# yang-z-03/scd-resnet

Measured on AMD Instinct MI355X. Metric: 512x512 images/sec training, centerOffsetRes10, at 1/2/4/8 MI355X, higher is better.
Workload: dtype bf16; 1 GPU; centerOffsetRes10 train step (fwd+focal/L1 loss+bwd+Adam, DDP over RCCL), 512x512 synthetic SCD tiles; model=centerOffsetRes10, global_batch=32, step_issue=eager launches, per_gpu_batch=32, parallelism=dp1, image_size=512

## Files before the change

include/scdhip.h:

```cpp
#ifndef SCDHIP_H
#define SCDHIP_H
#include <stddef.h>
#include <stdint.h>

#ifdef __cplusplus
extern "C" {
#endif

#define SCD_DT_F32 0
#define SCD_DT_BF16 1
#define SCD_DT_F16 2

#define SCD_ERR_ARG 9001

#define SCD_MAX_TAPS 16
#define SCD_MAX_PHASES 4
#define SCD_STAT_REPLICAS 64

typedef struct scd_gemm_phase {
    int Qh, Qw, rho_h, rho_w, ntaps;
    int dh[SCD_MAX_TAPS], dw[SCD_MAX_TAPS], wt[SCD_MAX_TAPS];
} scd_gemm_phase;

int scd_conv_gemm(int dtype, const void* x, const void* w, void* y, const float* bias, double* stats,
                  int N, int Hi, int Wi, int Ci, int Ho, int Wo, int Co, int in_stride, int out_stride,
                  int wrow, int relu, int accumulate, int nphase, const scd_gemm_phase* phases,
                  void* stream);

int scd_conv_dgrad_s2(int dtype, const void* dy, const void* w3, void* dx, int N, int Hq, int Wq, int Cg, int Cin,
                      int accumulate, void* stream);
int scd_conv_gemm_bnbwd(int dtype, const void* x, const void* w, void* y, int N, int Hi, int Wi, int Ci, int Ho,
                        int Wo, int Co, int in_stride, int out_stride, int wrow, int nphase,
                        const scd_gemm_phase* phases, const void* bn_y, const float* mean, const float* invstd,
                        const float* relu_scale, const float* relu_shift, double* bn_stats, void* stream);
int scd_conv_gemm_sel(int dtype, int kernel, const void* x, const void* w, void* y, const float* bias, double* stats,
                      int N, int Hi, int Wi, int Ci, int Ho, int Wo, int Co, int in_stride, int out_stride, int wrow,
                      int relu, int accumulate, int nphase, const scd_gemm_phase* phases, const void* bn_y,
                      const float* mean, const float* invstd, const float* relu_scale, const float* relu_shift,
                      void* stream);
int scd_conv_gemm_res(int dtype, const void* x, const void* w, void* y, const float* bias, const void* res, int N,
                      int Hi, int Wi, int Ci, int Ho, int Wo, int Co, int in_stride, int out_stride, int wrow,
                      int relu, int nphase, const scd_gemm_phase* phases, void* stream);
int scd_conv_gemm_heads(int dtype, const void* x, const void* w, void* hid, const float* bias, int N, int H,
                        int W, int Ci, int nh, const int* od, const float* const* w1, const float* const* b1,
                        float* const* outs, void* stream);
int scd_conv_gemm_heads_keep(int dtype, const void* x, const void* w, void* hid, const float* bias, int N, int H,
                             int W, int Ci, int nh, const int* od, const float* const* w1, const float* const* b1,
                             float* const* outs, const unsigned char* keep, int keep_cols, void* stream);

size_t scd_conv_wgrad_workspace(int Cg, int T, int Ci, int nsplit);
int scd_conv_wgrad_nsplit(int dtype, long M, int Cg, int T, int Ci);
int scd_conv_wgrad_nsplit2(int dtype, long M, int Ho, int Wo, int Cg, int T, int Ci);
int scd_conv_wgrad(int dtype, const void* g, const void* x, float* ws, int nsplit,
                   int N, int Ho, int Wo, int Cg, int Hi, int Wi, int Ci, int in_stride,
                   int T, const int* dh, const int* dw, void* stream);
int scd_wgrad_reduce(const float* ws, int nsplit, int Cg, int T, int Ci, int r0, int r1, int cvalid,
                     long ld_n, long ld_c, long ld_t, float* dst, int accumulate, float alpha, void* stream);
int scd_wgrad_reduce_rows(const float* ws, int nsplit, int Cg, int T, int Ci, int nslices, const int* r0,
                          const int* r1, const long* ld_n, const long* ld_c, const long* ld_t, float* const* dst,
                          int cvalid, int accumulate, float alpha, void* stream);

int scd_pack_weight(int dtype, const float* w, void* out, int A, int B, int T, int mode, int ldp,
                    int row_off, void* stream);

int scd_pad_channels(int dtype, const void* src, long rows, int C, int Cp, void* dst, void* stream);

int scd_upsample2x_add(int dtype, const void* up, const void* low, void* out, int N, int h, int w, int C, void* stream);
int scd_upsample2x_add_bwd(int dtype, const void* dout, void* dlow, int N, int h, int w, int C, void* stream);

typedef struct scd_pack_desc {
    const float* w;
    void* out;
    long start;
    int A, B, T, mode, ldp, row_off, a_off, a_tot;
} scd_pack_desc;
int scd_pack_weights_batched(int dtype, const scd_pack_desc* descs, int n, long total, void* stream);

int scd_im2col_stem(int dtype, const float* x, void* cols, int N, int H, int W, int Ho, int Wo, int kh,
                    int kw, int stride, int pad, int Kpad, void* stream);

int scd_stem_conv_fwd(int dtype, const float* x, const void* wpk, void* y, double* stats, int N, int H, int W,
                      int Ho, int Wo, void* stream);
int scd_stem_conv_wgrad_nsplit(long M);
int scd_stem_conv_wgrad(int dtype, const void* dy, const void* ybn, const float* coef, const float* x, float* ws,
                        int nsplit, int N, int H, int W, int Ho, int Wo, void* stream);
int scd_stem_bwd_nsplit(void);
int scd_stem_bwd_fused(int dtype, const void* dout, const uint8_t* argmax, const void* y, const float* scale,
                       const float* shift, const float* mean, const float* invstd, const float* x, double* stats,
                       float* ws, int nsplit, float* tg, int N, int H, int W, int Ho, int Wo, void* stream);
int scd_stem_bwd_combine(int dtype, const float* tg, const void* wpk, const float* coef, float* dst, int accumulate,
                         float alpha, void* stream);

int scd_stats_collapse(double* stats, int nrep, int C, void* stream);
int scd_stats_collapse_to(double* stats, int nrep, int C, double* out, void* stream);
int scd_bn_finalize(double* stats, int nrep, int C, double count, const float* gamma,
                    const float* beta, float* running_mean, float* running_var, int64_t* num_batches,
                    float momentum, float eps, float* mean, float* invstd, float* scale, float* shift,
                    void* stream);
#define SCD_BN_FIN_MAX 4
typedef struct scd_bn_fin_args {
    double* stats;
    int nrep, C;
    double count;
    const float* gamma;
    const float* beta;
    float* running_mean;
    float* running_var;
    int64_t* num_batches;
    float momentum, eps;
    float* mean;
    float* invstd;
    float* scale;
    float* shift;
} scd_bn_fin_args;
int scd_bn_finalize_n(const scd_bn_fin_args* layers, int n, void* stream);
int scd_bn_apply(int dtype, const void* y, void* out, int C, long total, const float* scale,
                 const float* shift, const void* res, const float* rscale, const float* rshift,
                 int relu, void* stream);
int scd_bn_bwd_reduce(int dtype, const void* dout, const void* mask, const void* y, const float* relu_scale,
                      const float* relu_shift, const float* mean, const float* invstd, int C, long total,
                      double* stats, void* stream);
int scd_bn_bwd_finalize(double* stats, int nrep, int C, double count, const float* gamma,
                        const float* mean, const float* invstd, float* dgamma, float* dbeta,
                        float gscale, float* coef, void* stream);
typedef struct scd_bn_bwd_fin_args {
    double* stats;
    int nrep, C;
    double count;
    const float* gamma;
    const float* mean;
    const float* invstd;
    float* dgamma;
    float* dbeta;
    float gscale;
    float* coef;
} scd_bn_bwd_fin_args;
int scd_bn_bwd_finalize_n(const scd_bn_bwd_fin_args* layers, int n, void* stream);
int scd_bn_bwd_apply(int dtype, const void* dout, const void* mask, const void* y, const float* relu_scale,
                     const float* relu_shift, const float* coef, int C, long total, void* dy, void* dz,
                     void* stream);

int scd_bn_bwd_reduce2(int dtype, const void* dout, const void* mask, const void* ya, const void* yb,
                       const float* mean_a, const float* invstd_a, const float* mean_b, const float* invstd_b, int C,
                       long total, double* stats_a, double* stats_b, void* stream);
int scd_bn_bwd_apply2(int dtype, const void* dout, const void* mask, const void* ya, const void* yb,
                      const float* coef_a, const float* coef_b, int C, long total, void* dya, void* dyb, void* stream);


int scd_stem_pool_bwd_bn(int dtype, const void* dout, const uint8_t* argmax, const void* y, const float* scale,
                         const float* shift, const float* mean, const float* invstd, void* dz, double* stats, int N,
                         int H, int W, int C, int Ho, int Wo, void* stream);
int scd_stem_pool_fwd(int dtype, const void* y, const float* scale, const float* shift, void* out,
                      uint8_t* argmax, int N, int H, int W, int C, int Ho, int Wo, void* stream);
int scd_stem_pool_bwd(int dtype, const void* dout, const uint8_t* argmax, const void* y,
                      const float* scale, const float* shift, void* dz, int N, int H, int W, int C,
                      int Ho, int Wo, void* stream);

int scd_heads_fwd(int dtype, const void* hid, int N, int HW, int nh, int Hd, const int* od,
                  const float* const* w1, const float* const* b1, float* const* outs, void* stream);
size_t scd_heads_bwd_accsize(int nh, int Hd, const int* od);
int scd_heads_bwd(int dtype, const void* hid, int N, int HW, int nh, int Hd, const int* od,
                  const float* const* w1, const float* const* douts, void* dhid, double* acc, void* stream);
int scd_heads_bwd_packed(int dtype, const void* hid, int N, int HW, int nh, int Hd, const int* od,
                         const float* const* w1, const float* const* douts, float dscale, float* packed, void* dhid,
                         double* acc, void* stream);
int scd_heads_bwd_weight_finalize(double* acc, int nh, int Hd, const int* od, float* const* dw1,
                                  float* const* db1, float* const* db0, int accumulate, float alpha, void* stream);
int scd_heads_bwd_packed_split(int dtype, const void* hid, int N, int HW, int nh, int Hd, const int* od, int nd,
                               const float* const* w1, const float* const* douts, float dscale, float* packed,
                               void* dhid, double* acc, void* stream);
int scd_heads_sparse_bwd(int dtype, const void* hid, const void* feat, int N, int H, int W, int Cin, int nh, int Hd,
                         const int* od, int nd, const float* const* w1, const float* const* douts, float dscale,
                         const long* inds, int K, void* dhid_s, void* xcol, double* acc, int* slotmap, int* ownermap,
                         void* stream);
int scd_heads_sparse_fixup(int dtype, void* dx, const void* cols, int N, int H, int W, int Cin, const long* inds, int K,
                           int* slotmap, int* ownermap, const void* bn_y, const float* mean, const float* invstd,
                           const float* relu_scale, const float* relu_shift, double* bn_stats, void* stream);

int scd_focal_fwd(const float* logits, const float* gt, long n, float* g, double* acc, void* stream);
int scd_l1_gather_fwd(const float* feat, int N, int C, int HW, const int64_t* inds, const uint8_t* mask,
                      const float* target, int K, int tstride, int toff, float* g, double* acc, void* stream);
int scd_centernet_loss_finalize(double* focal_acc, int nfocal, double* l1_acc, int nl1,
                                const float* l1_weights, float* out, float* factors, void* stream);
int scd_centernet_loss_fwd(const float* heat, const float* gt, long n_heat, const float* regr, int Cr, const float* off,
                           int Co, int N, int HW, const int64_t* inds, const uint8_t* mask, const float* target, int K,
                           int tstride, int toff_r, int toff_o, const float* l1_weights, float* g_heat, float* g_regr,
                           float* g_off, double* focal_acc, float* out, float* factors, void* stream);
int scd_centernet_loss_bwd_scale(float* g_heat, long n_heat, int N, int HW, const int64_t* inds, int K, float* g_regr,
                                 int Cr, float* g_off, int Co, const float* factors, const float* go, void* stream);

int scd_corner_ae_fwd(const float* tl_tag, const float* br_tag, int N, int HW, const int64_t* tl_inds,
                      const int64_t* br_inds, const uint8_t* valid, int K, float w_pull, float w_push,
                      double* focal_acc, int nfocal, double* ae_acc, float* gs_tl, float* gs_br, float* out,
                      float* factors, void* stream);
int scd_corner_ae_bwd(const float* gs_tl, const float* gs_br, int N, int HW, const int64_t* tl_inds,
                      const int64_t* br_inds, const uint8_t* valid, int K, const float* go, float* g_tl, float* g_br,
                      void* stream);

int scd_heads_keep_map(const int64_t* inds, int N, int K, int HW, int64_t* prev, int nprev, uint8_t* keep, void* stream);

int scd_scale_by_device(float* g, long n, const float* factors, int idx, const float* go, void* stream);

int scd_render_center_targets(const float* locs, const int* counts, int B, int K, int H, float threshold,
                              float* heat, uint8_t* mask, float* regr, int64_t* inds, void* stream);
#define SCD_CORNER_SPLIT_THREAD 0
#define SCD_CORNER_SPLIT_GRID 1
#define SCD_CORNER_SPLIT_DEFAULT SCD_CORNER_SPLIT_GRID
int scd_render_corner_targets(const float* locs, const int* counts, int B, int K, int H, float threshold,
                              float* heat, float* tl, float* br, uint8_t* mask, float* regr, int64_t* inds,
                              void* stream);
int scd_render_corner_targets_split(const float* locs, const int* counts, int B, int K, int H, float threshold,
                                    float* heat, float* tl, float* br, uint8_t* mask, float* regr, int64_t* inds,
                                    int split, void* stream);
int scd_corner_tag_inds(const float* locs, const int* counts, int B, int K, int size, int64_t* tl_inds,
                        int64_t* br_inds, uint8_t* valid, void* stream);
size_t scd_augment_workspace(int B);
int scd_augment_tiles(const float* in, float* out, int B, int H, int W, const uint8_t* flips, const float* jitter,
                      const float* noise, float noise_sv, unsigned long long seed, void* workspace, void* stream);
int scd_augment_tiles_indexed(const float* store, long nstore, const int* ids, float* out, int B, int H, int W,
                              const uint8_t* flips, const float* jitter, const float* noise, float noise_sv,
                              unsigned long long seed, void* workspace, void* stream);
int scd_pack_locs(const float* rows, const long* offsets, const int* ids, int B, const uint8_t* flips, const float* cs,
                  int size, int K, int trunc, float* locs, int* counts, void* stream);
#define SCD_ROTATE_MAP_ROW 0
#define SCD_ROTATE_MAP_64X4 1
#define SCD_ROTATE_MAP_32X8 2
#define SCD_ROTATE_MAP_16X16 3
#define SCD_ROTATE_MAP_DEFAULT SCD_ROTATE_MAP_32X8
int scd_rotate_tiles(const float* in, float* out, int B, int H, int W, const double* cs, void* stream);
int scd_rotate_tiles_mapped(const float* in, float* out, int B, int H, int W, const double* cs, int mapping,
                            void* stream);
size_t scd_slide_workspace(int ntiles);
int scd_slide_tiles(const uint8_t* rgb, int H, int W, int C, int tile, int stride, int clipH, int clipV, int padLR,
                    int padTB, int fix, float* out, void* workspace, void* stream);
int scd_slide_detections(const float* decoded, int T, int K, int stride, int padLR, int padTB, int clipV, float thr,
                         int* xy, double* ratio, int* count, void* stream);
#define SCD_SLIDE_SAMPLES_MAX 16384
#define SCD_SLIDE_RADIUS_MAX 1048576
size_t scd_slide_samples_workspace(int T, int K);
int scd_slide_samples(const float* decoded, int T, int K, int stride, int padLR, int padTB, int clipV, float thr,
                      int x0, int y0, int x1, int y1, int radius, double lo, double scale, int nbins, int* xy,
                      double* ratio, float* score, int* index, int* count, int64_t* hist, int64_t* counters,
                      void* workspace, void* stream);
size_t scd_slide_rotate_workspace(int H, int W);
int scd_slide_rotate_clips(const uint8_t* rgb, int H, int W, int C, int left, int top, int right, int bottom,
                           int tile, const double* angles, int R, float* out, void* workspace, void* stream);
size_t scd_decode_workspace(int N, int HW);
int scd_decode_topk(const float* heat, int N, int H, int W, int K, const float* offset, int od_off,
                    const float* regr, int od_regr, float* scores, int64_t* inds, int64_t* ys, int64_t* xs,
                    float* off_out, float* regr_out, void* workspace, void* stream);
int scd_corner_pairs(const float* tl_scores, const int64_t* tl_inds, const int64_t* tl_ys, const int64_t* tl_xs,
                     const float* br_scores, const int64_t* br_inds, const int64_t* br_ys, const int64_t* br_xs,
                     const float* tl_tag, const float* br_tag, int N, int K, int HW, float threshold, int D, float* det,
                     int* nvalid, void* stream);

int scd_ceval_count(const float* scores, const int64_t* cty, const int64_t* ctx, const float* offset, const float* regr,
                    const float* gt_regr, const void* gt_loc, int loc_mode, int loc_w, int N, int K, int L, int H,
                    float thr, int* counts, void* stream);
int scd_ceval_emit(const float* scores, const int64_t* cty, const int64_t* ctx, const float* offset, const float* regr,
                   const float* gt_regr, const void* gt_loc, int loc_mode, int loc_w, int N, int K, int L, int H,
                   float thr, const int* counts, float* const* streams, void* stream);
size_t scd_ceval_summary_workspace(long n);
int scd_ceval_summary(const float* const* streams, const long* lens, long objnum, const float* thr, int nthr,
                      double* out, void* workspace, void* stream);

int scd_adam_step(float* p, const float* g, float* m, float* v, long n, float lr, float beta1, float beta2,
                  float eps, float bc1, float bc2, float gscale, void* stream);
int scd_adam_step_dev(float* p, const float* g, float* m, float* v, long n, double* hyper, float beta1, float beta2,
                      float eps, float gscale, const unsigned long long* skip, void* stream);
int scd_sgd_step_dev(float* p, const float* g, float* buf, long n, double* hyper, float momentum, float dampening,
                     float weight_decay, int nesterov, float gscale,
                     const unsigned long long* skip, void* stream);

int scd_cpool_fwd(int dtype, int dir, const void* x, const void* addend, void* y, int N, int H, int W, int C,
                  void* stream);
int scd_cpool_bwd(int dtype, int dir, const void* x, const void* dy, void* dx, int N, int H, int W, int C,
                  void* stream);

int scd_nms(const float* x, long planes, int H, int W, int k, float* out, void* stream);
int scd_topk(const float* scores, int B, long n, int K, int HW, int W, float* out_scores, int64_t* inds, int* cats,
             float* ys, float* xs, void* stream);
int scd_focal_prob_fwd(const float* p, const float* gt, long n, float* g, double* acc, void* stream);
int scd_masked_l1_fwd(const float* r, const float* t, const uint8_t* mask, long rows, int C, int smooth, float* g,
                      double* acc, void* stream);

size_t scd_peer_mailbox_bytes(int R, int cap);
int scd_peer_alloc(size_t bytes, void** ptr);
int scd_peer_free(void* ptr);
int scd_peer_ipc_handle(void* ptr, void* handle64);
int scd_peer_ipc_open(const void* handle64, void** ptr);
int scd_peer_ipc_close(void* ptr);
int scd_peer_allreduce_f64(double* data, int n, int rank, int R, void* const* boxes, int cap, unsigned long long epoch,
                           unsigned long long* err, unsigned timeout_ms, void* stream);


int scd_event_create(void** ev);
int scd_event_destroy(void* ev);
int scd_event_record(void* ev, void* stream);
int scd_event_elapsed_ms(void* start, void* end, float* ms);

int scd_calib_mfma_peak(const void* src, int grid, int iters, float* out, unsigned long long* stamps, void* stream);
int scd_calib_set_stamps(unsigned long long* stamps);
int scd_calib_stamped_build(void);

const char* scd_version(void);

#ifdef __cplusplus
}
#endif
#endif
```

scd-resnet_amd/csrc/layers.hip:

```cpp
#include <algorithm>

#include "gemm_common.h"
#include "scd_common.h"

namespace {
SCD_KERNEL_NS_BEGIN

__device__ __forceinline__ float s2_phase_weight(const float* w, unsigned A, unsigned B, unsigned r, unsigned k) {
    const unsigned ph = r / B, b = r - ph * B, t = k / A, a = k - t * A;
    const int kr = (int)(ph >> 1) + 1 - 2 * (int)(t >> 1), ks = (int)(ph & 1) + 1 - 2 * (int)(t & 1);
    return (kr >= 0 && kr < 3 && ks >= 0 && ks < 3) ? w[(a * B + b) * 9 + kr * 3 + ks] : 0.f;
}

template <typename T>
__global__ void pack_weight_kernel(const float* w, T* out, int A, int B, int Tt, int mode, int ldp, int row_off) {
    if (mode == 3) {
        const unsigned total = 4u * B * ldp;
        for (unsigned i = blockIdx.x * blockDim.x + threadIdx.x; i < total; i += gridDim.x * blockDim.x) {
            const unsigned r = i / (unsigned)ldp, k = i - r * (unsigned)ldp;
            out[(long)(row_off + r) * ldp + k] = from_f<T>(k < 4u * A ? s2_phase_weight(w, A, B, r, k) : 0.f);
        }
        return;
    }
    const int rows = mode == 0 ? A : mode == 1 ? B : Tt * B;
    const unsigned total = (unsigned)rows * ldp;
    for (unsigned i = blockIdx.x * blockDim.x + threadIdx.x; i < total; i += gridDim.x * blockDim.x) {
        const int r = (int)(i / (unsigned)ldp);
        const int k = (int)(i - (unsigned)r * ldp);
        float v = 0.f;
        if (mode == 0) {
            const int t = k / B, b = k - (k / B) * B;
            if (t < Tt) v = w[((long)r * B + b) * Tt + t];
        } else if (mode == 1) {
            const int t = k / A, a = k - (k / A) * A;
            if (t < Tt) v = w[((long)a * B + r) * Tt + t];
        } else {
            if (k >= A) continue;
            const int t = r / B, b = r - (r / B) * B;
            out[(long)r * ldp + row_off + k] = from_f<T>(w[((long)k * B + b) * Tt + t]);
            continue;
        }
        out[(long)(row_off + r) * ldp + k] = from_f<T>(v);
    }
}

constexpr int PACK_UNIT = 4096;

__global__ __launch_bounds__(256) void pack_weights_batched_kernel(const scd_pack_desc* __restrict__ d, int n, int bf16) {
    const long e0 = (long)blockIdx.x * PACK_UNIT;
    int lo = 0, hi = n - 1;
    while (lo < hi) {
        const int mid = (lo + hi + 1) >> 1;
        if (d[mid].start <= e0) lo = mid; else hi = mid - 1;
    }
    const scd_pack_desc q = d[lo];
    if (q.mode == 1) {
        __shared__ float tile[64 * 65];
        const int T = q.T, BB = max(1, 64 / T);
        const int nbb = (q.B + BB - 1) / BB;
        const int u = (int)((e0 - q.start) / PACK_UNIT);
        const int ta = u / nbb, tb = u - (u / nbb) * nbb;
        const int a0 = ta * 64, b0 = tb * BB;
        if (a0 >= q.A) return;
        const int na = min(64, q.A - a0), nb = min(BB, q.B - b0);
        const int rowl = nb * T, pitch = rowl | 1;
        for (int i = threadIdx.x; i < na * rowl; i += 256) {
            const int a = i / rowl, k = i - a * rowl;
            tile[a * pitch + k] = q.w[((unsigned)(a0 + a) * q.B + b0) * T + k];
        }
        __syncthreads();
        if (bf16 && na % 8 == 0 && q.ldp % 8 == 0 && q.a_tot % 8 == 0 && q.a_off % 8 == 0) {
            const int na8 = na / 8;
            for (int i = threadIdx.x; i < na8 * rowl; i += 256) {
                const int bt = i / na8, a = (i - bt * na8) * 8;
                const int b = bt / T, t = bt - b * T;
                typedef __attribute__((ext_vector_type(8))) h16 bf8;
                bf8 v;
#pragma unroll
                for (int e = 0; e < 8; ++e) v[e] = (h16)tile[(a + e) * pitch + b * T + t];
                const unsigned o = (unsigned)(b0 + b) * q.ldp + t * q.a_tot + q.a_off + a0 + a;
                *(bf8*)((h16*)q.out + o) = v;
            }
            return;
        }
        for (int i = threadIdx.x; i < na * rowl; i += 256) {
            const int bt = i / na, a = i - bt * na;
            const int b = bt / T, t = bt - b * T;
            const float v = tile[a * pitch + b * T + t];
            const unsigned o = (unsigned)(b0 + b) * q.ldp + t * q.a_tot + q.a_off + a0 + a;
            if (bf16) ((h16*)q.out)[o] = (h16)v;
            else ((float*)q.out)[o] = v;
        }
        return;
    }
    if (q.mode == 3) {
        const unsigned count3 = 4u * q.B * q.ldp, base3 = (unsigned)(e0 - q.start);
#pragma unroll 4
        for (int j = 0; j < PACK_UNIT / 256; ++j) {
            const unsigned i = base3 + threadIdx.x + 256 * j;
            if (i >= count3) break;
            const unsigned r = i / (unsigned)q.ldp, k = i - r * (unsigned)q.ldp;
            const float v = s2_phase_weight(q.w, q.A, q.B, r, k);
            const unsigned o = (q.row_off + r) * (unsigned)q.ldp + k;
            if (bf16) ((h16*)q.out)[o] = (h16)v;
            else ((float*)q.out)[o] = v;
        }
        return;
    }
    const unsigned count = q.mode == 0 ? (unsigned)q.A * q.ldp : (unsigned)q.B * q.T * q.A;
    const unsigned base = (unsigned)(e0 - q.start);
    const unsigned ldp = q.ldp, B = q.B, Tt = q.T, A = q.A, TA = Tt * A;
    if (q.mode == 0 && bf16 && ldp % 8 == 0 && B % 8 == 0 && q.row_off >= 0) {
        typedef __attribute__((ext_vector_type(8))) h16 bf8;
#pragma unroll
        for (int j = 0; j < PACK_UNIT / 256 / 8; ++j) {
            const unsigned i = base + 8 * (threadIdx.x + 256 * j);
            if (i >= count) break;
            const unsigned r = i / ldp, k = i - r * ldp;
            const unsigned t = k / B, b = k - t * B;
            bf8 v;
            const float* src = q.w + (r * B + b) * Tt + min(t, Tt - 1);
#pragma unroll
            for (int e = 0; e < 8; ++e) {
                const float x = src[e * Tt];
                v[e] = (h16)(t < Tt ? x : 0.f);
            }
            *(bf8*)((h16*)q.out + (q.row_off + r) * ldp + k) = v;
        }
        return;
    }
#pragma unroll 4
    for (int j = 0; j < PACK_UNIT / 256; ++j) {
        const unsigned i = base + threadIdx.x + 256 * j;
        if (i >= count) break;
        float v;
        unsigned o;
        if (q.mode == 0) {
            const unsigned r = i / ldp, k = i - r * ldp;
            const unsigned t = k / B, b = k - t * B;
            v = t < Tt ? q.w[(r * B + b) * Tt + t] : 0.f;
            o = (q.row_off + r) * ldp + k;
        } else if (q.mode == 1) {
            const unsigned r = i / TA, rem = i - r * TA;
            const unsigned t = rem / A, a = rem - t * A;
            v = q.w[(a * B + r) * Tt + t];
            o = r * ldp + t * q.a_tot + q.a_off + a;
        } else {
            const unsigned BA = B * A;
            const unsigned t = i / BA, rem = i - t * BA;
            const unsigned b = rem / A, a = rem - b * A;
            v = q.w[(a * B + b) * Tt + t];
            o = (t * B + b) * ldp + q.a_off + a;
        }
        if (bf16) ((h16*)q.out)[o] = (h16)v;
        else ((float*)q.out)[o] = v;
    }
}

struct HeadsDesc {
    int nh, Hd, od[4], orow[4], nout;
    int nd;
    int hstride, dstride;
    const float* w1[4];
    const float* b1[4];
    const float* dout[4];
    float* out[4];
    const float* pk;
};

__global__ void heads_pack_kernel(int N, int HW, HeadsDesc d, float scale, float* pk) {
    const long P = (long)N * HW;
    for (long px = blockIdx.x * (long)blockDim.x + threadIdx.x; px < P; px += (long)gridDim.x * blockDim.x) {
        const long n = px / HW, q = px - n * HW;
        for (int h = 0; h < d.nd; ++h) {
            float v[4];
#pragma unroll
            for (int o = 0; o < 4; ++o) v[o] = o < d.od[h] ? d.dout[h][(n * d.od[h] + o) * HW + q] * scale : 0.f;
            *(float4*)(pk + (px * d.nd + h) * 4) = make_float4(v[0], v[1], v[2], v[3]);
        }
    }
}

template <typename T>
__global__ void heads_fwd_kernel(const T* hid, int N, int HW, HeadsDesc d) {
    constexpr int E = Vec16<T>::N;
    const int cph = d.Hd / E;
    const unsigned cpp = (unsigned)(d.nh * cph);
    const unsigned total = (unsigned)N * HW * cpp;
    for (unsigned base = blockIdx.x * blockDim.x; base < total; base += gridDim.x * blockDim.x) {
        const unsigned i = base + threadIdx.x;
        const bool ok = i < total;
        const unsigned px = ok ? i / cpp : 0;
        const int ch = ok ? (int)(i - px * cpp) : 0;
        const int h = ch / cph;
        const int cl = (ch - h * cph) * E;
        float v[E];
        if (ok) Vec16<T>::load(hid + (size_t)i * E, v);
        else
#pragma unroll
            for (int e = 0; e < E; ++e) v[e] = 0.f;
        float acc[4];
#pragma unroll
        for (int o = 0; o < 4; ++o) {
            float a = 0.f;
            if (ok && o < d.od[h]) {
                const float* w = d.w1[h] + o * d.Hd + cl;
#pragma unroll
                for (int e = 0; e < E; ++e) a += v[e] * w[e];
            }
            for (int m = cph >> 1; m > 0; m >>= 1) a += __shfl_xor(a, m, 64);
            acc[o] = a;
        }
        if (ok && (ch - h * cph) == 0) {
            const int n = (int)(px / (unsigned)HW);
            const int q = (int)(px - (unsigned)n * HW);
            for (int o = 0; o < d.od[h]; ++o)
                d.out[h][((size_t)n * d.od[h] + o) * HW + q] = acc[o] + d.b1[h][o];
        }
    }
}

template <typename T, int U, bool PK = false>
__global__ __launch_bounds__(512) void heads_bwd_kernel(const T* hid, int N, int HW, HeadsDesc d, T* dhid,
                                                        double* acc, int accsz, int PXB) {
    constexpr int E = Vec16<T>::N;
    constexpr int NA = 4 * E + E + 4;
    const int cph = d.Hd / E;
    const int cpp = d.nd * cph;
    const int G = blockDim.x / cpp;
    const int tid = threadIdx.x;
    const int c = tid % cpp;
    const int g = tid / cpp;
    const int h = c / cph;
    const int cl = (c - h * cph) * E;
    const int ct = h * d.Hd + cl;
    const int od = d.od[h];
    const float* dout = d.dout[h];
    float w[4][E];
#pragma unroll
    for (int o = 0; o < 4; ++o)
#pragma unroll
        for (int e = 0; e < E; ++e) w[o][e] = o < od ? d.w1[h][o * d.Hd + cl + e] : 0.f;
    float a[NA];
#pragma unroll
    for (int k = 0; k < NA; ++k) a[k] = 0.f;
    const unsigned P = (unsigned)N * HW;
    const unsigned p0 = blockIdx.x * (unsigned)PXB;
    const unsigned p1 = min(P, p0 + PXB);
    const unsigned Ctot = d.hstride, Dtot = d.dstride;
    auto body = [&](unsigned px, const float* gd, float* v) {
        float r[E];
#pragma unroll
        for (int e = 0; e < E; ++e) {
            const float s = gd[0] * w[0][e] + gd[1] * w[1][e] + gd[2] * w[2][e] + gd[3] * w[3][e];
            r[e] = v[e] > 0.f ? s : 0.f;
#pragma unroll
            for (int o = 0; o < 4; ++o) a[o * E + e] += gd[o] * v[e];
            a[4 * E + e] += r[e];
        }
#pragma unroll
        for (int o = 0; o < 4; ++o) a[5 * E + o] += gd[o];
        Vec16<T>::store(dhid + px * Dtot + ct, r);
    };
    auto load_gd = [&](unsigned px, float* gd) {
        if constexpr (PK) {
            const float4 v = *(const float4*)(d.pk + ((size_t)px * d.nd + h) * 4);
            gd[0] = v.x; gd[1] = v.y; gd[2] = v.z; gd[3] = v.w;
        } else {
            const unsigned n = px / (unsigned)HW;
            const unsigned q = px - n * HW;
#pragma unroll
            for (int o = 0; o < 4; ++o) gd[o] = o < od ? dout[(n * od + o) * (unsigned)HW + q] : 0.f;
        }
    };
    if (g < G) {
        unsigned px = p0 + g;
        for (; px + (U - 1) * G < p1; px += U * G) {
            float gd[U][4], v[U][E];
#pragma unroll
            for (int u = 0; u < U; ++u) {
                load_gd(px + u * G, gd[u]);
                Vec16<T>::load(hid + (px + u * G) * Ctot + ct, v[u]);
            }
#pragma unroll
            for (int u = 0; u < U; ++u) body(px + u * G, gd[u], v[u]);
        }
        for (; px < p1; px += G) {
            float gd[4], v[E];
            load_gd(px, gd);
            Vec16<T>::load(hid + px * Ctot + ct, v);
            body(px, gd, v);
        }
    }
    constexpr int KR = (NA + 3) / 4;
    __shared__ float red[KR * 512];
    double* dst = acc + (size_t)(blockIdx.x % SCD_STAT_REPLICAS) * accsz;
#pragma unroll
    for (int k0 = 0; k0 < NA; k0 += KR) {
        if (k0) __syncthreads();
        if (g < G)
#pragma unroll
            for (int k = 0; k < KR; ++k)
                if (k0 + k < NA) red[(k * G + g) * cpp + c] = a[k0 + k];
        __syncthreads();
        for (int i = tid; i < KR * cpp; i += blockDim.x) {
            const int kk = i / cpp, cc = i - (i / cpp) * cpp;
            const int k = k0 + kk;
            if (k >= NA) continue;
            float s = 0.f;
            for (int j = 0; j < G; ++j) s += red[(kk * G + j) * cpp + cc];
            const int hh = cc / cph;
            const int cll = (cc - hh * cph) * E;
            const int odh = d.od[hh];
            if (k < 4 * E) {
                const int o = k / E, e = k - (k / E) * E;
                if (o < odh) atomic_add_f64(dst + (d.orow[hh] + o) * d.Hd + cll + e, (double)s);
            } else if (k < 5 * E) {
                atomic_add_f64(dst + d.nout * d.Hd + d.nout + hh * d.Hd + cll + (k - 4 * E), (double)s);
            } else {
                const int o = k - 5 * E;
                if (o < odh && cll == 0) atomic_add_f64(dst + d.nout * d.Hd + d.orow[hh] + o, (double)s);
            }
        }
    }
}

bool make_desc(HeadsDesc& d, int nh, int Hd, const int* od) {
    if (nh < 1 || nh > 4 || Hd % 8 != 0) return false;
    d.nh = nh; d.Hd = Hd; d.nout = 0;
    d.nd = nh; d.hstride = d.dstride = nh * Hd;
    for (int h = 0; h < 4; ++h) {
        d.od[h] = h < nh ? od[h] : 0;
        if (d.od[h] > 4) return false;
        d.orow[h] = d.nout;
        d.nout += d.od[h];
        d.w1[h] = nullptr; d.b1[h] = nullptr; d.dout[h] = nullptr; d.out[h] = nullptr;
        d.pk = nullptr;
    }
    return d.nout * Hd <= 8 * 512;
}

inline int ew_blocks(long n) { return (int)std::min<long>(8192, std::max<long>(1, (n + 255) / 256)); }

SCD_KERNEL_NS_END
}

extern "C" int scd_pack_weights_batched(int dtype, const scd_pack_desc* descs, int n, long total, void* stream) {
    SCD_F16_FWD(scd_pack_weights_batched, descs, n, total, stream);
    if (n < 1 || total < 1 || total >= (1L << 31) || total % PACK_UNIT || (dtype != SCD_DT_BF16 && dtype != SCD_DT_F32)) return SCD_ERR_ARG;
    hipLaunchKernelGGL(pack_weights_batched_kernel, dim3((unsigned)(total / PACK_UNIT)), dim3(256), 0, (hipStream_t)stream,
                       descs, n, dtype == SCD_DT_BF16 ? 1 : 0);
    SCD_RETURN_LAUNCH();
}

extern "C" int scd_pack_weight(int dtype, const float* w, void* out, int A, int B, int T, int mode, int ldp, int row_off,
                               void* stream) {
    SCD_F16_FWD(scd_pack_weight, w, out, A, B, T, mode, ldp, row_off, stream);
    if (mode == 3 && (T != 9 || ldp < 4 * A)) return SCD_ERR_ARG;
    const long total = (long)(mode == 0 ? A : mode == 3 ? 4 * B : B) * ldp;
    return scd_dispatch_dtype(dtype, [&](auto tag) {
        using E = typename decltype(tag)::type;
        hipLaunchKernelGGL((pack_weight_kernel<E>), dim3(ew_blocks(total)), dim3(256), 0, (hipStream_t)stream, w,
                           (E*)out, A, B, T, mode, ldp, row_off);
        SCD_RETURN_LAUNCH();
    });
}

extern "C" int scd_heads_fwd(int dtype, const void* hid, int N, int HW, int nh, int Hd, const int* od,
                             const float* const* w1, const float* const* b1, float* const* outs, void* stream) {
    SCD_F16_FWD(scd_heads_fwd, hid, N, HW, nh, Hd, od, w1, b1, outs, stream);
    HeadsDesc d;
    if (!make_desc(d, nh, Hd, od)) return SCD_ERR_ARG;
    return scd_dispatch_dtype(dtype, [&](auto tag) {
        using T = typename decltype(tag)::type;
        constexpr int E = 16 / sizeof(T);
        const int cph = Hd / E;
        if (cph > 64 || (cph & (cph - 1))) return SCD_ERR_ARG;
        for (int h = 0; h < nh; ++h) { d.w1[h] = w1[h]; d.b1[h] = b1[h]; d.out[h] = outs[h]; }
        const long total = (long)N * HW * nh * cph;
        const int blocks = (int)std::min<long>(16384, (total + 255) / 256);
        hipLaunchKernelGGL((heads_fwd_kernel<T>), dim3(blocks), dim3(256), 0, (hipStream_t)stream, (const T*)hid, N,
                           HW, d);
        SCD_RETURN_LAUNCH();
    });
}

template <bool PK>
static int launch_heads_bwd(int dtype, const void* hid, int N, int HW, int nh, int Hd, const int* od, int nd,
                            const float* const* w1, const float* const* douts, float dscale, float* packed, void* dhid,
                            double* acc, void* stream) {
    HeadsDesc d;
    if (!make_desc(d, nh, Hd, od) || (PK && !packed) || nd < 1 || nd > nh) return SCD_ERR_ARG;
    d.nd = nd;
    d.dstride = nd * Hd;
    return scd_dispatch_dtype(dtype, [&](auto tag) {
        using T = typename decltype(tag)::type;
        constexpr int E = 16 / sizeof(T);
        const int cpp = nd * Hd / E;
        if (cpp > 256 || (Hd % E)) return SCD_ERR_ARG;
        for (int h = 0; h < nh; ++h) { d.w1[h] = w1[h]; d.dout[h] = douts[h]; }
        const int accsz = d.nout * Hd + d.nout + nh * Hd;
        const long P = (long)N * HW;
        if (P * nh * Hd >= (1L << 31)) return SCD_ERR_ARG;
        hipStream_t st = (hipStream_t)stream;
        if constexpr (PK) {
            hipLaunchKernelGGL(heads_pack_kernel, dim3(ew_blocks(P)), dim3(256), 0, st, N, HW, d, dscale, packed);
            hipError_t e = hipGetLastError();
            if (e != hipSuccess) return (int)e;
            d.pk = packed;
        }
        const int G = 512 / cpp;
        const int threads = G * cpp;
        const int PXB = 2048;
        const int blocks = cdiv(P, PXB);
        hipLaunchKernelGGL((heads_bwd_kernel<T, E, PK>), dim3(blocks), dim3(threads), 0, st, (const T*)hid, N, HW, d,
                           (T*)dhid, acc, accsz, PXB);
        SCD_RETURN_LAUNCH();
    });
}

extern "C" int scd_heads_bwd(int dtype, const void* hid, int N, int HW, int nh, int Hd, const int* od,
                             const float* const* w1, const float* const* douts, void* dhid, double* acc,
                             void* stream) {
    SCD_F16_FWD(scd_heads_bwd, hid, N, HW, nh, Hd, od, w1, douts, dhid, acc, stream);
    return launch_heads_bwd<false>(dtype, hid, N, HW, nh, Hd, od, nh, w1, douts, 1.f, nullptr, dhid, acc, stream);
}

extern "C" int scd_heads_bwd_packed(int dtype, const void* hid, int N, int HW, int nh, int Hd, const int* od,
                                    const float* const* w1, const float* const* douts, float dscale, float* packed,
                                    void* dhid, double* acc, void* stream) {
    SCD_F16_FWD(scd_heads_bwd_packed, hid, N, HW, nh, Hd, od, w1, douts, dscale, packed, dhid, acc, stream);
    return scd_heads_bwd_packed_split(dtype, hid, N, HW, nh, Hd, od, nh, w1, douts, dscale, packed, dhid, acc, stream);
}

extern "C" int scd_heads_bwd_packed_split(int dtype, const void* hid, int N, int HW, int nh, int Hd, const int* od,
                                          int nd, const float* const* w1, const float* const* douts, float dscale,
                                          float* packed, void* dhid, double* acc, void* stream) {
    SCD_F16_FWD(scd_heads_bwd_packed_split, hid, N, HW, nh, Hd, od, nd, w1, douts, dscale, packed, dhid, acc, stream);
    return launch_heads_bwd<true>(dtype, hid, N, HW, nh, Hd, od, nd, w1, douts, dscale, packed, dhid, acc, stream);
}

namespace {
SCD_KERNEL_NS_BEGIN
constexpr int SP_SPB = 2;

template <typename T>
__global__ __launch_bounds__(256) void heads_sparse_bwd_kernel(const T* hid, const T* feat, int N, int H, int W, int Cin,
                                                               HeadsDesc d, float dscale, const long* inds, int K,
                                                               T* dhid_s, T* xcol, double* acc, int accsz,
                                                               int* slotmap, int* ownermap) {
    const int HW = H * W;
    const int Cs = (d.nh - d.nd) * d.Hd;
    const int tid = threadIdx.x;
    const int c = tid;
    const bool cok = c < Cs;
    const int h = cok ? d.nd + c / d.Hd : d.nd;
    const int j = cok ? c - (h - d.nd) * d.Hd : 0;
    const int od = d.od[h];
    float w[4];
#pragma unroll
    for (int o = 0; o < 4; ++o) w[o] = (cok && o < od) ? d.w1[h][o * d.Hd + j] : 0.f;
    float a_dw1[4] = {0.f, 0.f, 0.f, 0.f}, a_db1[4] = {0.f, 0.f, 0.f, 0.f}, a_db0 = 0.f;
    const int S = N * K;
    const int s0 = blockIdx.x * SP_SPB;
    const int ns = min(S, s0 + SP_SPB) - s0;
    __shared__ int dup[SP_SPB];
    if (tid < SP_SPB) dup[tid] = 0;
    __syncthreads();
    for (int i = tid; i < ns * K; i += blockDim.x) {
        const int jj = i / K, k2 = i - (i / K) * K;
        const int s = s0 + jj, k = s - (s / K) * K;
        if (k2 < k && inds[s - k + k2] == inds[s]) dup[jj] = 1;
    }
    __syncthreads();
    for (int jj = 0; jj < ns; ++jj) {
        const int s = s0 + jj;
        const int b = s / K;
        const long ind = inds[s];
        const bool active = ind >= 0 && ind < HW && !dup[jj];
        const int q0 = active ? (int)ind : 0;
        const int y = q0 / W, x = q0 - (q0 / W) * W;
        const long p = (long)b * HW + q0;
        float r = 0.f;
        if (active && cok) {
            const float hv = to_f<T>(hid[p * d.hstride + d.nd * d.Hd + c]);
            float g[4];
#pragma unroll
            for (int o = 0; o < 4; ++o) g[o] = o < od ? d.dout[h][((long)b * od + o) * HW + q0] * dscale : 0.f;
            const float sacc = g[0] * w[0] + g[1] * w[1] + g[2] * w[2] + g[3] * w[3];
            r = hv > 0.f ? sacc : 0.f;
#pragma unroll
            for (int o = 0; o < 4; ++o) { a_dw1[o] += g[o] * hv; a_db1[o] += g[o]; }
            a_db0 += r;
        }
        if (cok) dhid_s[(long)s * Cs + c] = from_f<T>(r);
        if (active && tid < 9) {
            if (tid == 0) slotmap[p] = s;
            const int qy = y + tid / 3 - 1, qx = x + tid % 3 - 1;
            if ((unsigned)qy < (unsigned)H && (unsigned)qx < (unsigned)W)
                atomicMin(ownermap + (long)b * HW + qy * W + qx, s * 9 + tid);
        }
        for (int ci = tid; ci < Cin; ci += blockDim.x) {
            T v[9];
#pragma unroll
            for (int t = 0; t < 9; ++t) {
                const int iy = y + t / 3 - 1, ix = x + t % 3 - 1;
                const bool in = (unsigned)iy < (unsigned)H && (unsigned)ix < (unsigned)W;
                v[t] = in ? feat[(((long)b * H + iy) * W + ix) * Cin + ci] : from_f<T>(0.f);
            }
#pragma unroll
            for (int t = 0; t < 9; ++t) xcol[(long)s * 9 * Cin + t * Cin + ci] = v[t];
        }
    }
    if (cok) {
        double* dst = acc + (size_t)(blockIdx.x % SCD_STAT_REPLICAS) * accsz;
#pragma unroll
        for (int o = 0; o < 4; ++o)
            if (o < od) atomic_add_f64(dst + (d.orow[h] + o) * d.Hd + j, (double)a_dw1[o]);
        atomic_add_f64(dst + d.nout * d.Hd + d.nout + h * d.Hd + j, (double)a_db0);
        if (j == 0)
#pragma unroll
            for (int o = 0; o < 4; ++o)
                if (o < od) atomic_add_f64(dst + d.nout * d.Hd + d.orow[h] + o, (double)a_db1[o]);
    }
}

template <typename T>
__global__ __launch_bounds__(256) void heads_sparse_fixup_kernel(T* dx, const T* cols, int N, int H, int W, int Cin,
                                                                 const long* inds, int K, const int* slotmap,
                                                                 int* ownermap, const T* bny, const float* mean,
                                                                 const float* invstd, const float* rsc,
                                                                 const float* rsh, double* stats) {
    const int HW = H * W;
    const int s = blockIdx.x;
    const int b = s / K;
    const long ind = inds[s];
    if (ind < 0 || ind >= HW) return;
    const long p = (long)b * HW + ind;
    if (slotmap[p] != s) return;
    const int y = (int)ind / W, x = (int)ind - ((int)ind / W) * W;
    const int tid = threadIdx.x;
    __shared__ int nb[25], own[9];
    if (tid < 25) {
        const int py = y + tid / 5 - 2, px = x + tid % 5 - 2;
        nb[tid] = ((unsigned)py < (unsigned)H && (unsigned)px < (unsigned)W) ? slotmap[(long)b * HW + py * W + px] : -1;
    } else if (tid >= 32 && tid < 41) {
        const int t = tid - 32;
        const int qy = y + t / 3 - 1, qx = x + t % 3 - 1;
        own[t] = ((unsigned)qy < (unsigned)H && (unsigned)qx < (unsigned)W) ? ownermap[(long)b * HW + qy * W + qx] : -1;
    }
    __syncthreads();
    if (tid < 9 && own[tid] == s * 9 + tid)
        ownermap[(long)b * HW + (y + tid / 3 - 1) * W + x + tid % 3 - 1] = 0x7fffffff;
    const long KC = 9L * Cin;
    for (int ci = tid; ci < Cin; ci += blockDim.x) {
        float bm = 0.f, bi = 0.f, bs = 0.f, bh = 0.f;
        if (bny) { bm = mean[ci]; bi = invstd[ci]; bs = rsc[ci]; bh = rsh[ci]; }
        float dsum = 0.f, dsq = 0.f;
        for (int t = 0; t < 9; ++t) {
            if (own[t] != s * 9 + t) continue;
            const int oy = t / 3 - 1, ox = t % 3 - 1;
            float corr = 0.f;
#pragma unroll
            for (int t2 = 0; t2 < 9; ++t2) {
                const int s2 = nb[(oy - (t2 / 3 - 1) + 2) * 5 + ox - (t2 % 3 - 1) + 2];
                if (s2 >= 0) corr += to_f<T>(cols[(long)s2 * KC + t2 * Cin + ci]);
            }
            const long qi = p + oy * W + ox;
            T* dp = dx + qi * Cin + ci;
            const T old = *dp;
            const T nv = from_f<T>(to_f<T>(old) + corr);
            *dp = nv;
            if (bny) {
                const float yv = to_f<T>(bny[qi * Cin + ci]);
                const float dd = yv * bs + bh > 0.f ? to_f<T>(nv) - to_f<T>(old) : 0.f;
                dsum += dd;
                dsq += dd * (yv - bm) * bi;
            }
        }
        if (bny) {
            const int rep = stat_replica(s);
            atomic_add_f64(stat_slot(stats, rep, 0, Cin, ci), (double)dsum);
            atomic_add_f64(stat_slot(stats, rep, 1, Cin, ci), (double)dsq);
        }
    }
}

__global__ void heads_sparse_reset_kernel(const long* inds, int S, int K, int HW, int* slotmap) {
    const int s = blockIdx.x * blockDim.x + threadIdx.x;
    if (s >= S) return;
    const long ind = inds[s];
    if (ind < 0 || ind >= HW) return;
    const long p = (long)(s / K) * HW + ind;
    if (slotmap[p] == s) slotmap[p] = -1;
}

SCD_KERNEL_NS_END
}

extern "C" int scd_heads_sparse_bwd(int dtype, const void* hid, const void* feat, int N, int H, int W, int Cin, int nh,
                                    int Hd, const int* od, int nd, const float* const* w1, const float* const* douts,
                                    float dscale, const long* inds, int K, void* dhid_s, void* xcol, double* acc,
                                    int* slotmap, int* ownermap, void* stream) {
    SCD_F16_FWD(scd_heads_sparse_bwd, hid, feat, N, H, W, Cin, nh, Hd, od, nd, w1, douts, dscale, inds, K, dhid_s, xcol,
                acc, slotmap, ownermap, stream);
    HeadsDesc d;
    if (!make_desc(d, nh, Hd, od) || nd < 0 || nd >= nh || K < 1 || (nh - nd) * Hd > 256) return SCD_ERR_ARG;
    if ((long)N * K * 9 * 9 >= (1L << 31) || (long)N * H * W * nh * Hd >= (1L << 31)) return SCD_ERR_ARG;
    d.nd = nd;
    for (int h = 0; h < nh; ++h) { d.w1[h] = w1[h]; d.dout[h] = douts[h]; }
    const int accsz = d.nout * Hd + d.nout + nh * Hd;
    const int blocks = cdiv((long)N * K, SP_SPB);
    return scd_dispatch_dtype(dtype, [&](auto tag) {
        using T = typename decltype(tag)::type;
        hipLaunchKernelGGL(heads_sparse_bwd_kernel<T>, dim3(blocks), dim3(256), 0, (hipStream_t)stream, (const T*)hid,
                           (const T*)feat, N, H, W, Cin, d, dscale, inds, K, (T*)dhid_s, (T*)xcol, acc, accsz, slotmap,
                           ownermap);
        SCD_RETURN_LAUNCH();
    });
}

extern "C" int scd_heads_sparse_fixup(int dtype, void* dx, const void* cols, int N, int H, int W, int Cin,
                                      const long* inds, int K, int* slotmap, int* ownermap, const void* bn_y,
                                      const float* mean, const float* invstd, const float* relu_scale,
                                      const float* relu_shift, double* bn_stats, void* stream) {
    SCD_F16_FWD(scd_heads_sparse_fixup, dx, cols, N, H, W, Cin, inds, K, slotmap, ownermap, bn_y, mean, invstd,
                relu_scale, relu_shift, bn_stats, stream);
    if (Cin < 1 || K < 1) return SCD_ERR_ARG;
    if (bn_y && !(mean && invstd && relu_scale && relu_shift && bn_stats)) return SCD_ERR_ARG;
    const int S = N * K;
    hipStream_t st = (hipStream_t)stream;
    return scd_dispatch_dtype(dtype, [&](auto tag) {
        using T = typename decltype(tag)::type;
        hipLaunchKernelGGL(heads_sparse_fixup_kernel<T>, dim3(S), dim3(256), 0, st, (T*)dx, (const T*)cols, N, H, W,
                           Cin, inds, K, slotmap, ownermap, (const T*)bn_y, mean, invstd, relu_scale, relu_shift,
                           bn_stats);
        hipError_t e = hipGetLastError();
        if (e != hipSuccess) return (int)e;
        hipLaunchKernelGGL(heads_sparse_reset_kernel, dim3(cdiv(S, 256)), dim3(256), 0, st, inds, S, K, H * W, slotmap);
        SCD_RETURN_LAUNCH();
    });
}

#ifndef SCD_F16_BUILD
namespace {

struct HeadsGrad {
    float* dw1[4];
    float* db1[4];
    float* db0[4];
};

__global__ void heads_bwd_weight_finalize_kernel(double* acc, int accsz, HeadsDesc d, HeadsGrad g, int accumulate,
                                                 double alpha) {
    for (int i = blockIdx.x * blockDim.x + threadIdx.x; i < accsz; i += gridDim.x * blockDim.x) {
        double s = 0.0;
        for (int r = 0; r < SCD_STAT_REPLICAS; ++r) {
            s += acc[(long)r * accsz + i];
            acc[(long)r * accsz + i] = 0.0;
        }
        float* dst;
        if (i < d.nout * d.Hd) {
            const int row = i / d.Hd, cl = i - (i / d.Hd) * d.Hd;
            int h = 0;
            while (h + 1 < d.nh && row >= d.orow[h + 1]) ++h;
            dst = g.dw1[h] + (row - d.orow[h]) * d.Hd + cl;
        } else if (i < d.nout * d.Hd + d.nout) {
            const int row = i - d.nout * d.Hd;
            int h = 0;
            while (h + 1 < d.nh && row >= d.orow[h + 1]) ++h;
            dst = g.db1[h] + (row - d.orow[h]);
        } else {
            const int c = i - d.nout * d.Hd - d.nout;
            const int h = c / d.Hd;
            dst = g.db0[h] + (c - h * d.Hd);
        }
        s *= alpha;
        *dst = accumulate ? (*dst + (float)s) : (float)s;
    }
}

__global__ void adam_kernel(float* p, const float* g, float* m, float* v, long n, float lr, float b1, float b2,
                            float eps, float bc1, float bc2_sqrt, float gscale) {
    const float step = lr / bc1;
    for (long i = blockIdx.x * (long)blockDim.x + threadIdx.x; i < n; i += (long)gridDim.x * blockDim.x) {
        const float gi = g[i] * gscale;
        float mi = m[i];
        mi = mi + (1.f - b1) * (gi - mi);
        float vi = v[i] * b2 + (1.f - b2) * gi * gi;
        const float denom = sqrtf(vi) / bc2_sqrt + eps;
        p[i] = p[i] - step * (mi / denom);
        m[i] = mi;
        v[i] = vi;
    }
}

__global__ void adam_tick_kernel(double* hyper, const unsigned long long* skip) {
    if (skip && *skip) return;
    if (threadIdx.x == 0) hyper[1] = hyper[1] + 1.0;
}

__global__ void adam_dev_kernel(float* p, const float* g, float* m, float* v, long n, const double* hyper, float b1,
                                float b2, float eps, float gscale, const unsigned long long* skip) {
    if (skip && *skip) return;
    const double s = hyper[1];
    const float lr = (float)hyper[0];
    const float bc1 = (float)(1.0 - pow((double)b1, s));
    const float bc2 = (float)(1.0 - pow((double)b2, s));
    const float step = lr / bc1;
    const float bc2_sqrt = sqrtf(bc2);
    for (long i = blockIdx.x * (long)blockDim.x + threadIdx.x; i < n; i += (long)gridDim.x * blockDim.x) {
        const float gi = g[i] * gscale;
        float mi = m[i];
        mi = mi + (1.f - b1) * (gi - mi);
        float vi = v[i] * b2 + (1.f - b2) * gi * gi;
        const float denom = sqrtf(vi) / bc2_sqrt + eps;
        p[i] = p[i] - step * (mi / denom);
        m[i] = mi;
        v[i] = vi;
    }
}

__global__ void sgd_tick_kernel(double* hyper, const unsigned long long* skip) {
    if (skip && *skip) return;
    if (threadIdx.x == 0) {
        hyper[1] = hyper[1] + 1.0;
        hyper[3] = hyper[2];
        hyper[2] = 1.0;
    }
}

__global__ void sgd_dev_kernel(float* p, const float* g, float* buf, long n, const double* hyper, float mom, float damp,
                               float wd, int nesterov, float gscale, const unsigned long long* skip) {
    if (skip && *skip) return;
    const float lr = (float)hyper[0];
    const bool first = hyper[3] == 0.0;
    for (long i = blockIdx.x * (long)blockDim.x + threadIdx.x; i < n; i += (long)gridDim.x * blockDim.x) {
        const float pi = p[i];
        float d = g[i] * gscale;
        if (wd != 0.f) d = d + wd * pi;
        if (mom != 0.f) {
            const float b = first ? d : buf[i] * mom + (1.f - damp) * d;
            buf[i] = b;
            d = nesterov ? d + mom * b : b;
        }
        p[i] = pi - lr * d;
    }
}
}

extern "C" size_t scd_heads_bwd_accsize(int nh, int Hd, const int* od) {
    int nout = 0;
    for (int h = 0; h < nh; ++h) nout += od[h];
    return (size_t)SCD_STAT_REPLICAS * (nout * Hd + nout + nh * Hd) * sizeof(double);
}

extern "C" int scd_heads_bwd_weight_finalize(double* acc, int nh, int Hd, const int* od, float* const* dw1,
                                             float* const* db1, float* const* db0, int accumulate, float alpha, void* stream) {
    HeadsDesc d;
    if (!make_desc(d, nh, Hd, od)) return SCD_ERR_ARG;
    HeadsGrad g;
    for (int h = 0; h < 4; ++h) {
        g.dw1[h] = h < nh ? dw1[h] : nullptr;
        g.db1[h] = h < nh ? db1[h] : nullptr;
        g.db0[h] = h < nh ? db0[h] : nullptr;
    }
    const int accsz = d.nout * Hd + d.nout + nh * Hd;
    hipLaunchKernelGGL(heads_bwd_weight_finalize_kernel, dim3(cdiv(accsz, 256)), dim3(256), 0, (hipStream_t)stream, acc,
                       accsz, d, g, accumulate, (double)alpha);
    SCD_RETURN_LAUNCH();
}

extern "C" int scd_adam_step(float* p, const float* g, float* m, float* v, long n, float lr, float beta1, float beta2,
                             float eps, float bc1, float bc2, float gscale, void* stream) {
    hipLaunchKernelGGL(adam_kernel, dim3(ew_blocks(n)), dim3(256), 0, (hipStream_t)stream, p, g, m, v, n, lr, beta1,
                       beta2, eps, bc1, sqrtf(bc2), gscale);
    SCD_RETURN_LAUNCH();
}

extern "C" int scd_adam_step_dev(float* p, const float* g, float* m, float* v, long n, double* hyper, float beta1,
                                 float beta2, float eps, float gscale, const unsigned long long* skip, void* stream) {
    if (!hyper) return SCD_ERR_ARG;
    hipLaunchKernelGGL(adam_tick_kernel, dim3(1), dim3(64), 0, (hipStream_t)stream, hyper, skip);
    hipLaunchKernelGGL(adam_dev_kernel, dim3(ew_blocks(n)), dim3(256), 0, (hipStream_t)stream, p, g, m, v, n,
                       (const double*)hyper, beta1, beta2, eps, gscale, skip);
    SCD_RETURN_LAUNCH();
}

extern "C" int scd_sgd_step_dev(float* p, const float* g, float* buf, long n, double* hyper, float momentum,
                                float dampening, float weight_decay, int nesterov, float gscale,
                                const unsigned long long* skip, void* stream) {
    if (!hyper || (momentum != 0.f && !buf)) return SCD_ERR_ARG;
    hipLaunchKernelGGL(sgd_tick_kernel, dim3(1), dim3(64), 0, (hipStream_t)stream, hyper, skip);
    hipLaunchKernelGGL(sgd_dev_kernel, dim3(ew_blocks(n)), dim3(256), 0, (hipStream_t)stream, p, g, buf, n,
                       (const double*)hyper, momentum, dampening, weight_decay, nesterov, gscale, skip);
    SCD_RETURN_LAUNCH();
}
#endif
```

scd-resnet_amd/csrc/loss_decode.hip:

```cpp
#define BLOCK_OPS_FP
#include "block_ops.h"

namespace {

__global__ void focal_fwd_kernel(const float* x, const float* gt, long n, float* g, double* acc) {
    float posl = 0.f, negl = 0.f, npos = 0.f;
    for (long i = blockIdx.x * (long)blockDim.x + threadIdx.x; i < n; i += (long)gridDim.x * blockDim.x)
        g[i] = focal_logit_term(x[i], gt[i], posl, negl, npos);
    focal_accumulate(posl, negl, npos, acc);
}

__global__ void l1_gather_kernel(const float* feat, int N, int C, int HW, const int64_t* inds, const uint8_t* mask,
                                 const float* target, int K, int tstride, int toff, float* g, double* acc) {
    float s = 0.f, cnt = 0.f;
    for (int i = blockIdx.x * blockDim.x + threadIdx.x; i < N * K; i += gridDim.x * blockDim.x) {
        const int n = i / K;
        if (!mask[i]) continue;
        cnt += 1.f;
        const long ind = inds[i];
        for (int c = 0; c < C; ++c) {
            const long fi = ((long)n * C + c) * HW + ind;
            const float d = feat[fi] - target[(long)i * tstride + toff + c];
            s += fabsf(d);
            const float sg = d > 0.f ? 1.f : (d < 0.f ? -1.f : 0.f);
            if (sg != 0.f) atomic_add_f32(g + fi, sg);
        }
    }
    double a = (double)s, b = (double)cnt;
    if (block_sums_d<4>(a, b, blockDim.x / 64)) {
        atomic_add_f64(acc + 0, a);
        atomic_add_f64(acc + 1, b);
    }
}

struct LossFin {
    float l1w[8];
};

__device__ __forceinline__ float focal_finalize(const double* facc, int f, float* factor) {
    double pl = 0, nl = 0, np = 0;
    for (int r = 0; r < SCD_STAT_REPLICAS; ++r) {
        const double* a = facc + ((long)f * SCD_STAT_REPLICAS + r) * FOCAL_ACC;
        pl += a[0]; nl += a[1]; np += a[2];
    }
    const float posl = (float)pl, negl = (float)nl, npos = (float)np;
    *factor = np == 0.0 ? -1.f : -1.f / npos;
    return np == 0.0 ? -negl : -(posl + negl) / npos;
}

__global__ void loss_finalize_kernel(double* facc, int nfocal, double* lacc, int nl1, LossFin w, float* out,
                                     float* factors) {
    if (blockIdx.x != 0) return;
    if (threadIdx.x == 0) {
        double total = 0.0;
        for (int f = 0; f < nfocal; ++f) {
            const float v = focal_finalize(facc, f, factors + f);
            out[1 + f] = v;
            total += v;
        }
        for (int l = 0; l < nl1; ++l) {
            const double s = lacc[2 * l], cnt = lacc[2 * l + 1];
            const float v = w.l1w[l] * ((float)s / ((float)cnt + 1e-4f));
            out[1 + nfocal + l] = v;
            factors[nfocal + l] = w.l1w[l] / ((float)cnt + 1e-4f);
            total += v;
        }
        out[0] = (float)total;
    }
    __syncthreads();
    for (int i = threadIdx.x; i < nfocal * SCD_STAT_REPLICAS * FOCAL_ACC; i += blockDim.x) facc[i] = 0.0;
    if (lacc)
        for (int i = threadIdx.x; i < 2 * nl1; i += blockDim.x) lacc[i] = 0.0;
}

__global__ void scale_by_device_kernel(float* g, long n, const float* factors, int idx, const float* go) {
    const float f = factors[idx] * (go ? go[0] : 1.f);
    for (long i = blockIdx.x * (long)blockDim.x + threadIdx.x; i < n; i += (long)gridDim.x * blockDim.x) g[i] *= f;
}

__global__ void centernet_loss_a_kernel(const float* x, const float* gt, long n, float* g, double* acc, float* gz,
                                        long nz) {
    float posl = 0.f, negl = 0.f, npos = 0.f;
    const long stride = (long)gridDim.x * blockDim.x;
    for (long i = blockIdx.x * (long)blockDim.x + threadIdx.x; i < n; i += stride)
        g[i] = focal_logit_term(x[i], gt[i], posl, negl, npos);
    for (long i = blockIdx.x * (long)blockDim.x + threadIdx.x; i < nz; i += stride) gz[i] = 0.f;
    focal_accumulate(posl, negl, npos, acc);
}

static_assert(SCD_STAT_REPLICAS == 64, "centernet_loss_b_kernel sums the focal replicas with one wave");

struct L1Term {
    const float* feat;
    float* g;
    int C, toff;
};

__global__ __launch_bounds__(1024) void centernet_loss_b_kernel(int N, int HW, const int64_t* inds, const uint8_t* mask,
                                                               const float* target, int K, int tstride, L1Term t0,
                                                               L1Term t1, double* facc, LossFin w, float* out,
                                                               float* factors) {
    float s[2] = {0.f, 0.f}, cnt = 0.f;
    for (int i = threadIdx.x; i < N * K; i += blockDim.x) {
        if (!mask[i]) continue;
        cnt += 1.f;
        const int n = i / K;
        const long ind = inds[i];
#pragma unroll
        for (int l = 0; l < 2; ++l) {
            const L1Term& t = l ? t1 : t0;
            for (int c = 0; c < t.C; ++c) {
                const long fi = ((long)n * t.C + c) * HW + ind;
                const float d = t.feat[fi] - target[(long)i * tstride + t.toff + c];
                s[l] += fabsf(d);
                const float sg = d > 0.f ? 1.f : (d < 0.f ? -1.f : 0.f);
                if (sg != 0.f) atomic_add_f32(t.g + fi, sg);
            }
        }
    }
    __shared__ double red[3][16], frd[3];
    const double a = wave_sum_d((double)s[0]), b = wave_sum_d((double)s[1]), c = wave_sum_d((double)cnt);
    const int lane = threadIdx.x & 63, wv = threadIdx.x >> 6;
    if (lane == 0) { red[0][wv] = a; red[1][wv] = b; red[2][wv] = c; }
    if (wv == 0) {
        const double* q = facc + (long)lane * FOCAL_ACC;
        const double pl = wave_sum_d(q[0]), nl = wave_sum_d(q[1]), np = wave_sum_d(q[2]);
        if (lane == 0) { frd[0] = pl; frd[1] = nl; frd[2] = np; }
    }
    __syncthreads();
    if (threadIdx.x == 0) {
        double ls[2] = {0.0, 0.0}, lc = 0.0;
        for (int k = 0; k < (int)(blockDim.x / 64); ++k) { ls[0] += red[0][k]; ls[1] += red[1][k]; lc += red[2][k]; }
        const double pl = frd[0], nl = frd[1], np = frd[2];
        const float posl = (float)pl, negl = (float)nl, npos = (float)np;
        const float v = np == 0.0 ? -negl : -(posl + negl) / npos;
        out[1] = v;
        factors[0] = np == 0.0 ? -1.f : -1.f / npos;
        double total = v;
        for (int l = 0; l < 2; ++l) {
            const float vl = w.l1w[l] * ((float)ls[l] / ((float)lc + 1e-4f));
            out[2 + l] = vl;
            factors[1 + l] = w.l1w[l] / ((float)lc + 1e-4f);
            total += vl;
        }
        out[0] = (float)total;
    }
    __syncthreads();
    for (int i = threadIdx.x; i < SCD_STAT_REPLICAS * FOCAL_ACC; i += blockDim.x) facc[i] = 0.0;
}

__global__ void centernet_loss_scale_kernel(float* gh, long nh, int N, int HW, const int64_t* inds, int K, float* g0,
                                            int C0, float* g1, int C1, const float* factors, const float* go) {
    const float gs = go ? go[0] : 1.f;
    const float f0 = factors[0] * gs;
    const long stride = (long)gridDim.x * blockDim.x;
    const long t0 = blockIdx.x * (long)blockDim.x + threadIdx.x;
    for (long i = t0; i < nh; i += stride) gh[i] *= f0;
    const float f1 = factors[1] * gs, f2 = factors[2] * gs;
    for (long s = t0; s < (long)N * K; s += stride) {
        const int n = (int)(s / K), k = (int)(s - (long)n * K);
        const int64_t ind = inds[s];
        if (ind < 0 || ind >= HW) continue;
        bool first = true;
        for (int k2 = 0; k2 < k; ++k2) first &= inds[(long)n * K + k2] != ind;
        if (!first) continue;
        for (int c = 0; c < C0; ++c) g0[((long)n * C0 + c) * HW + ind] *= f1;
        for (int c = 0; c < C1; ++c) g1[((long)n * C1 + c) * HW + ind] *= f2;
    }
}

template <typename Cand>
__device__ __forceinline__ void select_sorted_keys(Cand cand, int n, int K, unsigned long long* keys) {
    __shared__ unsigned hist[256];
    __shared__ unsigned s_prefix, s_krem, s_count, s_eqtaken;
    const int tid = threadIdx.x;
    unsigned prefix = 0, pmask = 0, krem = (unsigned)K;
    for (int pass = 0; pass < 4; ++pass) {
        const int shift = 24 - 8 * pass;
        for (int i = tid; i < 256; i += blockDim.x) hist[i] = 0;
        __syncthreads();
        for (int i = tid; i < n; i += blockDim.x) {
            unsigned b;
            if (cand(i, b) && (b & pmask) == prefix) atomicAdd(&hist[(b >> shift) & 255], 1u);
        }
        __syncthreads();
        if (tid == 0) {
            unsigned cum = 0, d = 0;
            for (int b = 255; b >= 0; --b) {
                if (cum + hist[b] >= krem) { d = (unsigned)b; break; }
                cum += hist[b];
            }
            s_prefix = prefix | (d << shift);
            s_krem = krem - cum;
        }
        __syncthreads();
        prefix = s_prefix;
        krem = s_krem;
        pmask |= 255u << shift;
        __syncthreads();
    }
    if (tid == 0) { s_count = 0; s_eqtaken = 0; }
    for (int i = tid; i < 1024; i += blockDim.x) keys[i] = 0ull;
    __syncthreads();
    const unsigned thr = prefix;
    for (int i = tid; i < n; i += blockDim.x) {
        unsigned b;
        if (cand(i, b) && b > thr) {
            const unsigned slot = atomicAdd(&s_count, 1u);
            keys[slot] = ((unsigned long long)b << 32) | (unsigned)(0xFFFFFFFFu - (unsigned)i);
        }
    }
    __syncthreads();
    for (int base = 0; base < n; base += blockDim.x) {
        __syncthreads();
        const unsigned taken = s_eqtaken;
        if (taken >= krem) break;
        const int i = base + tid;
        unsigned b = 0;
        const bool eq = i < n && cand(i, b) && b == thr;
        const unsigned long long bal = __ballot(eq);
        const int lane = tid & 63, wv = tid >> 6;
        __shared__ unsigned wcount[16];
        if (lane == 0) wcount[wv] = __popcll(bal);
        __syncthreads();
        unsigned before = 0;
        for (int k = 0; k < wv; ++k) before += wcount[k];
        before += __popcll(bal & ((1ull << lane) - 1ull));
        if (eq && taken + before < krem) {
            const unsigned slot = (unsigned)K - krem + taken + before;
            keys[slot] = ((unsigned long long)thr << 32) | (unsigned)(0xFFFFFFFFu - (unsigned)i);
        }
        __syncthreads();
        if (tid == 0) {
            unsigned tot = 0;
            for (int k = 0; k < (int)(blockDim.x / 64); ++k) tot += wcount[k];
            s_eqtaken = taken + tot;
        }
    }
    __syncthreads();
    int P = 1;
    while (P < K) P <<= 1;
    for (int size = 2; size <= P; size <<= 1) {
        for (int stride = size >> 1; stride > 0; stride >>= 1) {
            for (int i = tid; i < P; i += blockDim.x) {
                const int j = i ^ stride;
                if (j > i) {
                    const bool desc = (i & size) == 0;
                    const unsigned long long a = keys[i], b = keys[j];
                    if (desc ? (a < b) : (a > b)) { keys[i] = b; keys[j] = a; }
                }
            }
            __syncthreads();
        }
    }
}

// ... 74 lines not shown
        }
        *(float4*)(out + r * 8) = make_float4(row[0], row[1], row[2], row[3]);
        *(float4*)(out + r * 8 + 4) = make_float4(row[4], row[5], row[6], row[7]);
    }
    if (tid == 0) nvalid[n] = nsel;
}

constexpr int AE_MAXK = 64;
constexpr int AE_THREADS = 256;

__global__ __launch_bounds__(AE_THREADS) void corner_ae_fwd_kernel(const float* tl_tag, const float* br_tag, int HW,
                                                                   const int64_t* tl_inds, const int64_t* br_inds,
                                                                   const uint8_t* valid, int K, float w_pull,
                                                                   float w_push, double* acc, float* gs_tl,
                                                                   float* gs_br) {
    __shared__ double et[AE_MAXK], eb[AE_MAXK], mm[AE_MAXK];
    __shared__ int vd[AE_MAXK];
    const int b = blockIdx.x, tid = threadIdx.x;
    if (tid < K) {
        const long o = (long)b * K + tid;
        const int64_t it = tl_inds[o], ib = br_inds[o];
        const int v = valid[o] && it >= 0 && it < HW && ib >= 0 && ib < HW;
        vd[tid] = v;
        et[tid] = v ? (double)tl_tag[(long)b * HW + it] : 0.0;
        eb[tid] = v ? (double)br_tag[(long)b * HW + ib] : 0.0;
        mm[tid] = (et[tid] + eb[tid]) / 2;
    }
    __syncthreads();
    int n = 0;
    for (int k = 0; k < K; ++k) n += vd[k];
    const float fn = (float)n;
    const float dpull_f = fn + 1e-4f, dpush_f = (fn - 1.f) * fn + 1e-4f;
    const double dpull = (double)dpull_f, dpush = (double)dpush_f, inv = (double)(1.f / dpull_f);
    double pull = 0.0, push = 0.0;
    if (tid < K && vd[tid]) {
        const double a = et[tid] - mm[tid], c = eb[tid] - mm[tid];
        pull = a * a / dpull + c * c / dpull;
    }
    for (int f = tid; f < K * K; f += blockDim.x) {
        const int i = f / K, j = f - i * K;
        if (!(vd[i] && vd[j])) continue;
        push += (fmax(1.0 - fabs(mm[j] - mm[i]), 0.0) - inv) / dpush;
    }
    if (block_sums_d<AE_THREADS / 64>(pull, push, AE_THREADS / 64)) {
        acc[2 * b] = pull;
        acc[2 * b + 1] = push;
    }
    if (tid < K) {
        double gt = 0.0, gb = 0.0;
        if (vd[tid]) {
            const double gp = ((et[tid] - mm[tid]) - (eb[tid] - mm[tid])) / dpull;
            double cnt = 0.0;
            for (int j = 0; j < K; ++j) {
                if (!vd[j]) continue;
                const double d = mm[tid] - mm[j];
                if (1.0 - fabs(d) > 0.0) cnt += d > 0.0 ? -1.0 : (d < 0.0 ? 1.0 : 0.0);
            }
            const double gm = 2.0 * cnt / dpush * 0.5;
            gt = (double)w_pull * gp + (double)w_push * gm;
            gb = -(double)w_pull * gp + (double)w_push * gm;
        }
        gs_tl[(long)b * K + tid] = (float)gt;
        gs_br[(long)b * K + tid] = (float)gb;
    }
}

__global__ void corner_ae_finalize_kernel(double* facc, int nfocal, const double* acc, int N, float w_pull, float w_push,
                                          float* out, float* factors) {
    if (threadIdx.x == 0) {
        double total = 0.0;
        for (int f = 0; f < nfocal; ++f) {
            const float v = focal_finalize(facc, f, factors + f);
            out[1 + f] = v;
            total += v;
        }
        double pull = 0.0, push = 0.0;
        for (int b = 0; b < N; ++b) { pull += acc[2 * b]; push += acc[2 * b + 1]; }
        const float vp = w_pull * (float)pull, vq = w_push * (float)push;
        out[1 + nfocal] = vp;
        out[2 + nfocal] = vq;
        out[0] = (float)(total + vp + vq);
    }
    __syncthreads();
    for (int i = threadIdx.x; i < nfocal * SCD_STAT_REPLICAS * FOCAL_ACC; i += blockDim.x) facc[i] = 0.0;
}

__global__ __launch_bounds__(256) void corner_ae_bwd_kernel(const float* gs_tl, const float* gs_br,
                                                            const int64_t* tl_inds, const int64_t* br_inds,
                                                            const uint8_t* valid, int K, int HW, const float* go,
                                                            float* g_tl, float* g_br) {
    __shared__ float gs[2][AE_MAXK];
    __shared__ int ix[2][AE_MAXK];
    const int b = blockIdx.y, tid = threadIdx.x;
    if (tid < 2 * K) {
        const int c = tid >= K, k = tid - c * K;
        const long o = (long)b * K + k;
        gs[c][k] = (c ? gs_br : gs_tl)[o];
        const int64_t ind = (c ? br_inds : tl_inds)[o];
        ix[c][k] = (valid[o] && ind >= 0 && ind < HW) ? (int)ind : -1;
    }
    __syncthreads();
    const float s = go ? go[0] : 1.f;
    for (int p = blockIdx.x * blockDim.x + tid; p < HW; p += gridDim.x * blockDim.x) {
        float a = 0.f, c = 0.f;
        for (int k = 0; k < K; ++k) {
            if (ix[0][k] == p) a += gs[0][k];
            if (ix[1][k] == p) c += gs[1][k];
        }
        g_tl[(long)b * HW + p] = a * s;
        g_br[(long)b * HW + p] = c * s;
    }
}

}

extern "C" int scd_focal_fwd(const float* logits, const float* gt, long n, float* g, double* acc, void* stream) {
    hipLaunchKernelGGL(focal_fwd_kernel, dim3(ew_blocks(n)), dim3(256), 0, (hipStream_t)stream, logits, gt, n, g, acc);
    SCD_RETURN_LAUNCH();
}

extern "C" int scd_l1_gather_fwd(const float* feat, int N, int C, int HW, const int64_t* inds, const uint8_t* mask,
                                 const float* target, int K, int tstride, int toff, float* g, double* acc, void* stream) {
    const int blocks = std::max(1, std::min(64, cdiv((long)N * K, 256)));
    hipLaunchKernelGGL(l1_gather_kernel, dim3(blocks), dim3(256), 0, (hipStream_t)stream, feat, N, C, HW, inds, mask,
                       target, K, tstride, toff, g, acc);
    SCD_RETURN_LAUNCH();
}

extern "C" int scd_centernet_loss_finalize(double* focal_acc, int nfocal, double* l1_acc, int nl1,
                                           const float* l1_weights, float* out, float* factors, void* stream) {
    if (nl1 > 8) return SCD_ERR_ARG;
    LossFin w;
    for (int i = 0; i < 8; ++i) w.l1w[i] = i < nl1 ? l1_weights[i] : 0.f;
    hipLaunchKernelGGL(loss_finalize_kernel, dim3(1), dim3(64), 0, (hipStream_t)stream, focal_acc, nfocal, l1_acc, nl1, w,
                       out, factors);
    SCD_RETURN_LAUNCH();
}

extern "C" int scd_centernet_loss_fwd(const float* heat, const float* gt, long n_heat, const float* regr, int Cr,
                                      const float* off, int Co, int N, int HW, const int64_t* inds, const uint8_t* mask,
                                      const float* target, int K, int tstride, int toff_r, int toff_o,
                                      const float* l1_weights, float* g_heat, float* g_regr, float* g_off,
                                      double* focal_acc, float* out, float* factors, void* stream) {
    if (n_heat < 1 || K < 1 || N < 1 || g_off != g_regr + (long)N * Cr * HW) return SCD_ERR_ARG;
    hipStream_t st = (hipStream_t)stream;
    const long nz = (long)N * (Cr + Co) * HW;
    hipLaunchKernelGGL(centernet_loss_a_kernel, dim3(ew_blocks(std::max(n_heat, nz))), dim3(256), 0, st, heat, gt, n_heat,
                       g_heat, focal_acc, g_regr, nz);
    hipError_t e = hipGetLastError();
    if (e != hipSuccess) return (int)e;
    LossFin w;
    for (int i = 0; i < 8; ++i) w.l1w[i] = i < 2 ? l1_weights[i] : 0.f;
    L1Term t0{regr, g_regr, Cr, toff_r}, t1{off, g_off, Co, toff_o};
    hipLaunchKernelGGL(centernet_loss_b_kernel, dim3(1), dim3(1024), 0, st, N, HW, inds, mask, target, K, tstride, t0, t1,
                       focal_acc, w, out, factors);
    SCD_RETURN_LAUNCH();
}

extern "C" int scd_centernet_loss_bwd_scale(float* g_heat, long n_heat, int N, int HW, const int64_t* inds, int K,
                                            float* g_regr, int Cr, float* g_off, int Co, const float* factors,
                                            const float* go, void* stream) {
    hipLaunchKernelGGL(centernet_loss_scale_kernel, dim3(ew_blocks(n_heat)), dim3(256), 0, (hipStream_t)stream, g_heat,
                       n_heat, N, HW, inds, K, g_regr, Cr, g_off, Co, factors, go);
    SCD_RETURN_LAUNCH();
}

__global__ __launch_bounds__(1024) void heads_keep_map_kernel(const int64_t* inds, int N, int K, int HW, int64_t* prev,
                                                              int nprev, uint8_t* keep) {
    for (int i = threadIdx.x; i < nprev; i += blockDim.x) {
        const int64_t q = prev[i];
        if (q >= 0) keep[q] = 0;
    }
    __syncthreads();
    for (int i = threadIdx.x; i < N * K; i += blockDim.x) {
        const int n = i / K;
        const int64_t v = inds[i];
        const int64_t q = (v >= 0 && v < HW) ? (int64_t)n * HW + v : -1;
        if (q >= 0) keep[q] = 1;
        prev[i] = q;
    }
    for (int i = N * K + threadIdx.x; i < nprev; i += blockDim.x) prev[i] = -1;
}

extern "C" int scd_heads_keep_map(const int64_t* inds, int N, int K, int HW, int64_t* prev, int nprev, uint8_t* keep,
                                  void* stream) {
    if (N < 1 || K < 1 || HW < 1 || nprev < N * K) return SCD_ERR_ARG;
    hipLaunchKernelGGL(heads_keep_map_kernel, dim3(1), dim3(1024), 0, (hipStream_t)stream, inds, N, K, HW, prev, nprev,
                       keep);
    SCD_RETURN_LAUNCH();
}

extern "C" int scd_scale_by_device(float* g, long n, const float* factors, int idx, const float* go, void* stream) {
    hipLaunchKernelGGL(scale_by_device_kernel, dim3(ew_blocks(n)), dim3(256), 0, (hipStream_t)stream, g, n, factors, idx,
                       go);
    SCD_RETURN_LAUNCH();
}

extern "C" size_t scd_decode_workspace(int N, int HW) { return (size_t)N * HW * sizeof(float); }

extern "C" int scd_decode_topk(const float* heat, int N, int H, int W, int K, const float* offset, int od_off,
                               const float* regr, int od_regr, float* scores, int64_t* inds, int64_t* ys, int64_t* xs,
                               float* off_out, float* regr_out, void* workspace, void* stream) {
    if (K < 1 || K > 1024 || K > H * W) return SCD_ERR_ARG;
    hipStream_t st = (hipStream_t)stream;
    float* t = (float*)workspace;
    hipLaunchKernelGGL(nms_kernel<NmsSigmoid>, dim3(ew_blocks((long)N * H * W)), dim3(256), 0, st, heat, (long)N, H, W, 3,
                       t);
    hipError_t e = hipGetLastError();
    if (e != hipSuccess) return (int)e;
    hipLaunchKernelGGL(decode_select_kernel, dim3(N), dim3(1024), 0, st, t, H * W, W, K, offset, od_off, regr, od_regr,
                       scores, inds, ys, xs, off_out, regr_out);
    SCD_RETURN_LAUNCH();
}

extern "C" int scd_corner_pairs(const float* tl_scores, const int64_t* tl_inds, const int64_t* tl_ys,
                                const int64_t* tl_xs, const float* br_scores, const int64_t* br_inds,
                                const int64_t* br_ys, const int64_t* br_xs, const float* tl_tag, const float* br_tag,
                                int N, int K, int HW, float threshold, int D, float* det, int* nvalid, void* stream) {
    if (!tl_scores || !tl_inds || !tl_ys || !tl_xs || !br_scores || !br_inds || !br_ys || !br_xs || !tl_tag || !br_tag ||
        !det || !nvalid)
        return SCD_ERR_ARG;
    if (N < 1 || K < 1 || K > PAIR_MAXK || HW < 1 || D < 1 || D > 1024 || D > K * K) return SCD_ERR_ARG;
    hipLaunchKernelGGL(corner_pairs_kernel, dim3(N), dim3(1024), 0, (hipStream_t)stream, tl_scores, tl_inds, tl_ys, tl_xs,
                       br_scores, br_inds, br_ys, br_xs, tl_tag, br_tag, K, HW, threshold, D, det, nvalid);
    SCD_RETURN_LAUNCH();
}

extern "C" int scd_corner_ae_fwd(const float* tl_tag, const float* br_tag, int N, int HW, const int64_t* tl_inds,
                                 const int64_t* br_inds, const uint8_t* valid, int K, float w_pull, float w_push,
                                 double* focal_acc, int nfocal, double* ae_acc, float* gs_tl, float* gs_br, float* out,
                                 float* factors, void* stream) {
    if (!tl_tag || !br_tag || !tl_inds || !br_inds || !valid || !focal_acc || !ae_acc || !gs_tl || !gs_br || !out ||
        !factors)
        return SCD_ERR_ARG;
    if (N < 1 || HW < 1 || (long)N * HW >= (1L << 31) || K < 1 || K > AE_MAXK || nfocal < 0) return SCD_ERR_ARG;
    hipStream_t st = (hipStream_t)stream;
    hipLaunchKernelGGL(corner_ae_fwd_kernel, dim3(N), dim3(AE_THREADS), 0, st, tl_tag, br_tag, HW, tl_inds, br_inds,
                       valid, K, w_pull, w_push, ae_acc, gs_tl, gs_br);
    hipError_t e = hipGetLastError();
    if (e != hipSuccess) return (int)e;
    hipLaunchKernelGGL(corner_ae_finalize_kernel, dim3(1), dim3(64), 0, st, focal_acc, nfocal, ae_acc, N, w_pull, w_push,
                       out, factors);
    SCD_RETURN_LAUNCH();
}

extern "C" int scd_corner_ae_bwd(const float* gs_tl, const float* gs_br, int N, int HW, const int64_t* tl_inds,
                                 const int64_t* br_inds, const uint8_t* valid, int K, const float* go, float* g_tl,
                                 float* g_br, void* stream) {
    if (!gs_tl || !gs_br || !tl_inds || !br_inds || !valid || !g_tl || !g_br) return SCD_ERR_ARG;
    if (N < 1 || N > 65535 || HW < 1 || (long)N * HW >= (1L << 31) || K < 1 || K > AE_MAXK) return SCD_ERR_ARG;
    const int slices = std::max(1, std::min(64, cdiv(HW, 256)));
    hipLaunchKernelGGL(corner_ae_bwd_kernel, dim3(slices, N), dim3(256), 0, (hipStream_t)stream, gs_tl, gs_br, tl_inds,
                       br_inds, valid, K, HW, go, g_tl, g_br);
    SCD_RETURN_LAUNCH();
}
```

scd-resnet_amd/csrc/scd_common.h:

```cpp
#pragma once
#include <hip/hip_runtime.h>
#include <stdint.h>
#include <string.h>

#include "../../include/scdhip.h"

#define SCD_F16_ENTRY_POINTS(X) \
    X(scd_conv_gemm) \
    X(scd_conv_gemm_sel) \
    X(scd_conv_gemm_bnbwd) \
    X(scd_conv_gemm_res) \
    X(scd_conv_gemm_heads) \
    X(scd_conv_gemm_heads_keep) \
    X(scd_conv_wgrad_nsplit2) \
    X(scd_conv_wgrad_nsplit) \
    X(scd_conv_wgrad) \
    X(scd_bn_apply) \
    X(scd_bn_bwd_reduce) \
    X(scd_bn_bwd_apply) \
    X(scd_bn_bwd_reduce2) \
    X(scd_bn_bwd_apply2) \
    X(scd_pack_weights_batched) \
    X(scd_pack_weight) \
    X(scd_im2col_stem) \
    X(scd_stem_pool_fwd) \
    X(scd_stem_pool_bwd) \
    X(scd_stem_pool_bwd_bn) \
    X(scd_heads_fwd) \
    X(scd_heads_bwd) \
    X(scd_heads_bwd_packed) \
    X(scd_heads_bwd_packed_split) \
    X(scd_heads_sparse_bwd) \
    X(scd_heads_sparse_fixup) \
    X(scd_stem_conv_fwd) \
    X(scd_stem_conv_wgrad) \
    X(scd_stem_bwd_fused) \
    X(scd_conv_dgrad_s2) \
    X(scd_stem_bwd_combine) \
    X(scd_pad_channels) \
    X(scd_upsample2x_add) \
    X(scd_upsample2x_add_bwd)
#ifdef SCD_F16_BUILD
#define SCD_F16_RENAME(fn) extern "C" decltype(fn) fn __asm__(#fn "__f16");
SCD_F16_ENTRY_POINTS(SCD_F16_RENAME)
#define SCD_F16_FWD(fn, ...) ((void)0)
#else
#define SCD_F16_DECL(fn) extern "C" decltype(fn) fn##__f16;
SCD_F16_ENTRY_POINTS(SCD_F16_DECL)
#define SCD_F16_FWD(fn, ...) \
    do { if (dtype == SCD_DT_F16) return fn##__f16(SCD_DT_BF16, __VA_ARGS__); } while (0)
#endif

#ifdef SCD_F16_BUILD
#define SCD_KERNEL_NS_BEGIN inline namespace f16 {
#define SCD_KERNEL_NS_END }
#else
#define SCD_KERNEL_NS_BEGIN
#define SCD_KERNEL_NS_END
#endif

__device__ __forceinline__ float h16_word_half(unsigned w, int hi) {
#ifdef SCD_F16_BUILD
    return (float)__builtin_bit_cast(_Float16, (unsigned short)(hi ? w >> 16 : w & 0xffffu));
#else
    return __uint_as_float(hi ? (w & 0xffff0000u) : (w << 16));
#endif
}

typedef __attribute__((ext_vector_type(4))) float f32x4;
typedef __attribute__((ext_vector_type(8))) __bf16 bf16x8;
#ifdef SCD_F16_BUILD
typedef _Float16 h16;
#else
typedef __bf16 h16;
#endif
typedef __attribute__((ext_vector_type(8))) h16 h16x8;
typedef __attribute__((ext_vector_type(4))) h16 h16x4;
__device__ __forceinline__ f32x4 mfma_16x16x32_h16(h16x8 a, h16x8 b, f32x4 c) {
#ifdef SCD_F16_BUILD
    return __builtin_amdgcn_mfma_f32_16x16x32_f16(a, b, c, 0, 0, 0);
#else
    return __builtin_amdgcn_mfma_f32_16x16x32_bf16(a, b, c, 0, 0, 0);
#endif
}
typedef __attribute__((ext_vector_type(4))) short s16x4;
typedef __attribute__((address_space(3))) s16x4 lds_s16x4;

template <typename T> struct scd_type { using type = T; };
template <typename F>
static inline int scd_dispatch_dtype(int dtype, F&& f) {
    if (dtype == SCD_DT_BF16) return f(scd_type<h16>{});
#ifndef SCD_F16_BUILD
    if (dtype == SCD_DT_F32) return f(scd_type<float>{});
#endif
    return SCD_ERR_ARG;
}

#define SCD_RETURN_LAUNCH() return (int)hipGetLastError()

template <typename T> __device__ __forceinline__ float to_f(T v);
template <> __device__ __forceinline__ float to_f<float>(float v) { return v; }
template <> __device__ __forceinline__ float to_f<h16>(h16 v) { return (float)v; }

template <typename T> __device__ __forceinline__ T from_f(float v);
template <> __device__ __forceinline__ float from_f<float>(float v) { return v; }
template <> __device__ __forceinline__ h16 from_f<h16>(float v) { return (h16)v; }

template <typename T> struct Vec16;
template <> struct Vec16<float> {
    static constexpr int N = 4;
    __device__ static void load(const void* p, float* f) {
        float4 v = *(const float4*)p;
        f[0] = v.x; f[1] = v.y; f[2] = v.z; f[3] = v.w;
    }
    __device__ static void store(void* p, const float* f) {
        *(float4*)p = make_float4(f[0], f[1], f[2], f[3]);
    }
};
template <> struct Vec16<h16> {
    static constexpr int N = 8;
    __device__ static void load(const void* p, float* f) {
        h16x8 v = *(const h16x8*)p;
#pragma unroll
        for (int i = 0; i < 8; ++i) f[i] = (float)v[i];
    }
    __device__ static void store(void* p, const float* f) {
        h16x8 v;
#pragma unroll
        for (int i = 0; i < 8; ++i) v[i] = (h16)f[i];
        *(h16x8*)p = v;
    }
};

__device__ __forceinline__ float wave_sum(float v) {
#pragma unroll
    for (int o = 32; o > 0; o >>= 1) v += __shfl_xor(v, o, 64);
    return v;
}
__device__ __forceinline__ double wave_sum_d(double v) {
#pragma unroll
    for (int o = 32; o > 0; o >>= 1) v += __shfl_xor(v, o, 64);
    return v;
}

__device__ __forceinline__ void atomic_add_f64(double* p, double v) { unsafeAtomicAdd(p, v); }
__device__ __forceinline__ void atomic_add_f32(float* p, float v) { unsafeAtomicAdd(p, v); }

static inline int cdiv(long a, long b) { return (int)((a + b - 1) / b); }

static inline int num_cus() {
    static int n = 0;
    if (n == 0) {
        int dev = 0;
        if (hipGetDevice(&dev) != hipSuccess ||
            hipDeviceGetAttribute(&n, hipDeviceAttributeMultiprocessorCount, dev) != hipSuccess || n <= 0)
            n = 256;
    }
    return n;
}

static inline int resident_grid(const void* kernel, int threads, size_t dyn_lds = 0) {
    int per = 1;
    if (hipOccupancyMaxActiveBlocksPerMultiprocessor(&per, kernel, threads, dyn_lds) != hipSuccess || per < 1) per = 1;
    return per * num_cus();
}
```

scd-resnet_amd/scdhip/blocks.py:

```python
import os

import torch

from . import ops
from .flat import grads_ready


def _c(t):
    return t if t is None or t.is_contiguous() else t.contiguous()


_STEM_FUSED_BWD = os.environ.get("SCD_STEM_FUSED_BWD", "1") != "0"


def _conv_ld(w):
    T = w.shape[2] * w.shape[3]
    return (w.shape[1] * T, T, 1)


def _conv_stats(x, conv, bn, stride, pad, training, timer=None):
    C = conv.weight.shape[0]
    kh, kw = conv.weight.shape[2], conv.weight.shape[3]
    wp = ops.pack_weight(conv.weight, x.dtype, 0)
    stats = ops.bn_stats(bn, "fwd") if training else None
# ... 97 lines not shown
    def forward(ctx, up, low):
        return ops.upsample_add(up, low)

    @staticmethod
    def backward(ctx, dout):
        dout = _c(dout)
        return dout, ops.upsample_add_bwd(dout)


def _block_layers(blk):
    mods = [(blk.conv1, blk.bn1), (blk.conv2, blk.bn2)]
    if "conv3" in blk._modules:
        mods.append((blk.conv3, blk.bn3))
    return [(c, bn, c.weight, (c.kernel_size[0], c.kernel_size[1], c.stride[0], c.padding[0])) for c, bn in mods]


class ResidualFn(torch.autograd.Function):

    @staticmethod
    def forward(ctx, x, w1, blk):
        tr = blk.training
        layers = _block_layers(blk)
        dconv, dbn = blk.downsample if blk.downsample is not None else (None, None)
        yd = std = None
        saved, sts, a = [], [], x
        for i, (conv, bn, _, (_, _, s, p)) in enumerate(layers):
            if i == 0 and tr and dconv is not None:
                y, st, yd, std = _conv1_and_downsample(x, dconv, dbn, conv, bn, s, p, dconv.stride[0])
            else:
                y, st = _train_bn_conv(a, conv, bn, s, p, tr)
            saved += [a, y]
            sts.append(st)
            if i + 1 < len(layers):
                a = ops.bn_apply(y, st, True)
        if dconv is not None:
            if yd is None:
                yd, std = _train_bn_conv(x, dconv, dbn, dconv.stride[0], 0, tr)
            out = ops.bn_apply(y, st, True, res=yd, rst=std)
        else:
            out = ops.bn_apply(y, st, True, res=x)
        ctx.save_for_backward(*saved, yd, out)
        ctx.sts = (sts, std)
        ctx.blk, ctx.layers, ctx.down = blk, layers, (dconv, dbn)
        return out

    @staticmethod
    def backward(ctx, dout):
        *saved, yd, out = ctx.saved_tensors
        sts, std = ctx.sts
        layers, (dconv, dbn) = ctx.layers, ctx.down
        ins, ys = saved[0::2], saved[1::2]
        x = ins[0]
        _, H, W, Cin = x.shape
        dx = dyd = None

        def wgrad(i, dy, dst):
            ops.conv_wgrad(dy, ins[i], *layers[i][3], dst, _conv_ld(layers[i][2]))

        n = len(layers) - 1
        _, bnn, wn, _ = layers[n]
        if dconv is not None:
            dy, dyd = ops.bn_backward_pair(bnn, sts[n], ys[n], dbn, std, yd, _c(dout), out)
            wd = dconv.weight
            gd, gn = ops.grad_of(wd), ops.grad_of(wn)
            with ops.side_batch():
                ops.conv_wgrad(dyd, x, 1, 1, dconv.stride[0], 0, gd, _conv_ld(wd))
                wgrad(n, dy, gn)
        else:
            dx = torch.empty_like(x)
            dy = ops.bn_backward(bnn, sts[n], _c(dout), ys[n], mask=out, dz_out=dx)
            wgrad(n, dy, ops.grad_of(wn))
        for i in range(n, 0, -1):
            _, _, w, geom = layers[i]
            dy = _dgrad_bn_relu_bwd(dy, ops.pack_weight(w, x.dtype, 1), w.shape[1], ins[i].shape[1], ins[i].shape[2],
                                    *geom, layers[i - 1][1], sts[i - 1], ys[i - 1])
            wgrad(i - 1, dy, ops.grad_of(layers[i - 1][2]))
        _, _, w1, (_, _, s1, p1) = layers[0]
        dx = ops.conv_dgrad_w(dy, w1, H, W, s1, p1, out=dx, accumulate=dx is not None)
        if dyd is not None:
            ops.conv_dgrad(dyd, ops.pack_weight(wd, x.dtype, 1), Cin, H, W, 1, 1, dconv.stride[0], 0, out=dx,
                           accumulate=True)
        grads_ready(ctx.blk)
        return dx, None, None


class DeconvBNFn(torch.autograd.Function):

    @staticmethod
    def forward(ctx, x, w, deconv, bn):
        k = w.shape[2]
        s, p = deconv.stride[0], deconv.padding[0]
        Cout = w.shape[1]
        stats = ops.bn_stats(bn, "fwd") if bn.training else None
        y = ops.deconv_fwd(x, ops.pack_weight(w, x.dtype, 1), Cout, k, s, p, stats=stats)
        st = ops.bn_finalize(bn, stats, Cout, y.numel() // Cout, bn.training)
        out = ops.bn_apply(y, st, True)
        ctx.save_for_backward(x, y, out)
        ctx.st, ctx.deconv, ctx.bn = st, deconv, bn
        ctx.prod = ops.bn_producer(x)
        ops.set_bn_producer(out, bn, st, y)
        return out

    @staticmethod
    def backward(ctx, dout):
        x, y, out = ctx.saved_tensors
        deconv, bn, st = ctx.deconv, ctx.bn, ctx.st
        w = deconv.weight
        k = w.shape[2]
        s, p = deconv.stride[0], deconv.padding[0]
        dout = _c(dout)
        dy = ops.bn_backward(bn, st, dout, y, relu=True, stats=ops.take_bn_bwd_fused(bn, dout))
        T = k * k
        ops.conv_wgrad(x, dy, k, k, s, p, ops.grad_of(w), (w.shape[1] * T, T, 1))
        fuse = ctx.prod is not None and x.dtype in ops.HALF
        dx = ops.deconv_dgrad(dy, ops.pack_weight(w, x.dtype, 0), w.shape[0], k, s, p,
                              bn_bwd=ops.fused_bn_bwd_args(ctx.prod) if fuse else None)
        if fuse:
            ops.mark_bn_bwd_fused(ctx.prod[0], dx)
        grads_ready(deconv, bn)
        return dx, None, None, None


class ConvBNFn(torch.autograd.Function):

    @staticmethod
    def forward(ctx, x, w, conv, bn, relu):
        s, p = conv.stride[0], conv.padding[0]
        y, st = _train_bn_conv(x, conv, bn, s, p, bn.training)
        out = ops.bn_apply(y, st, relu)
        ctx.save_for_backward(x, y, out)
        ctx.st, ctx.conv, ctx.bn, ctx.relu = st, conv, bn, relu
        return out

    @staticmethod
    def backward(ctx, dout):
        x, y, out = ctx.saved_tensors
        conv, bn, st = ctx.conv, ctx.bn, ctx.st
        w = conv.weight
        kh, kw = w.shape[2], w.shape[3]
        s, p = conv.stride[0], conv.padding[0]
        dy = ops.bn_backward(bn, st, _c(dout), y, relu=ctx.relu)
        ops.conv_wgrad(dy, x, kh, kw, s, p, ops.grad_of(w), _conv_ld(w))
        dx = ops.conv_dgrad(dy, ops.pack_weight(w, x.dtype, 1), x.shape[3], x.shape[1], x.shape[2], kh, kw, s, p)
        grads_ready(conv, bn)
        return dx, None, None, None, None


class HeadsFn(torch.autograd.Function):

    @staticmethod
    def forward(ctx, feat, w0_first, heads):
        N, H, W, Cin = feat.shape
        w0s = [h[0].weight for h in heads]
        b0 = torch.cat([h[0].bias for h in heads], 0)
        hd = ops.HeadsDesc([h[2].weight for h in heads], [h[2].bias for h in heads])
        wp = ops.pack_concat(w0s, feat.dtype, 0)
        hint = ops.take_sparse_hint()
        keep = ctx.keep = ctx.refill = None
        if (hd.fused and hint is not None and hd.nh >= 2 and Cin <= 256 and (hd.nh - 1) * hd.Hd <= 256
                and hint.dim() == 2 and hint.shape[0] == N):
            keep = ops.heads_keep_map(hint, N, H * W)
            ctx.keep = (hint, hint._version)
            ctx.refill = (wp, b0)
        hid, outs = ops.heads_fwd(feat, wp, b0, hd, keep)
        ctx.save_for_backward(feat, hid)
        ctx.w0s = w0s
        ctx.heads, ctx.hd = heads, hd
        ctx.prod = ops.bn_producer(feat)
        return tuple(outs)

    @staticmethod
    def backward(ctx, *douts):
        feat, hid = ctx.saved_tensors
        w0s = ctx.w0s
        heads, hd = ctx.heads, ctx.hd
        Hd, nh = hd.Hd, hd.nh
        N, H, W, Cin = feat.shape
        douts = [(_c(d) if d is not None else torch.zeros(N, o, H, W, device=feat.device))
                 for d, o in zip(douts, hd.od)]
        S = ops.begin_loss_scale(feat.dtype)
        dptrs = ops.tensor_ptrs(douts)
        nd = HeadsFn._dense_prefix(douts, Hd, Cin)
        if ctx.keep is not None:
            inds = ops.sparse_grad_inds(douts[-1]) if nd == 1 else None
            if inds is None or inds is not ctx.keep[0] or inds._version != ctx.keep[1]:
                ops.heads_refill(feat, *ctx.refill, hd, hid)
            ctx.refill = None
        if nd < nh:
            return HeadsFn._backward_sparse(ctx, douts, dptrs, hd.odarr, nd, S)
        dhid = ops.heads_bwd_packed(hid, hd, dptrs, S)
        ops.heads_bwd_weight_finalize(hd, [h[0].bias for h in heads], S)
        ld = (Cin * 9, 9, 1)
        rows = [(i * Hd, (i + 1) * Hd, ops.grad_of(h[0].weight), ld) for i, h in enumerate(heads)]
        ops.conv_wgrad(dhid, feat, 3, 3, 1, 1, None, None, rows=rows)
        slot = ops.shared_grad_slot(feat)
        prev = slot[1] if slot is not None else None
        fuse = slot is None and ctx.prod is not None and feat.dtype in ops.HALF
        dfeat = ops.conv_dgrad(dhid, ops.pack_concat(w0s, feat.dtype, 1), Cin, H, W, 3, 3, 1, 1, out=prev,
                               accumulate=prev is not None, bn_bwd=ops.fused_bn_bwd_args(ctx.prod) if fuse else None)
        if fuse:
            ops.mark_bn_bwd_fused(ctx.prod[0], dfeat)
        grads_ready(*[m for h in heads for m in h if isinstance(m, torch.nn.Module)])
        if slot is not None:
            return ops.shared_grad_out(feat, slot, dfeat if prev is None else None), None, None
        return dfeat, None, None

    @staticmethod
    def _dense_prefix(douts, Hd, Cin):
        nh = len(douts)
        if nh < 2 or Cin > 256:
            return nh
        certs = [ops.sparse_grad_inds(d) for d in douts]
        nd = nh
        while nd > 1 and certs[nd - 1] is not None and certs[nd - 1] is certs[-1]:
            nd -= 1
        return nd if (nh - nd) * Hd <= 256 else nh

    @staticmethod
    def _backward_sparse(ctx, douts, dptrs, odarr, nd, S):
        feat, hid = ctx.saved_tensors
        w0s, heads, hd = ctx.w0s, ctx.heads, ctx.hd
        Hd, nh = hd.Hd, hd.nh
        N, H, W, Cin = feat.shape
        dt = feat.dtype
        inds = ops.sparse_grad_inds(douts[-1])
        Sl = N * inds.shape[1]
        Cs = (nh - nd) * Hd
        dh_dense = ops.heads_bwd_packed(hid, hd, dptrs, S, nd)
        dhid_s, xcol, slotmap, ownermap = ops.heads_sparse_bwd(hid, feat, hd, nd, dptrs, S, inds)
        ops.heads_bwd_weight_finalize(hd, [h[0].bias for h in heads], S)
        ld = (Cin * 9, 9, 1)

        def wgrads():
            rd = [(i * Hd, (i + 1) * Hd, ops.grad_of(heads[i][0].weight), ld) for i in range(nd)]
            rs = [((i - nd) * Hd, (i - nd + 1) * Hd, ops.grad_of(heads[i][0].weight), ld) for i in range(nd, nh)]
            with ops.side_batch():
                ops.conv_wgrad(dh_dense, feat, 3, 3, 1, 1, None, None, rows=rd)
                ops.conv_wgrad(dhid_s.view(1, 1, Sl, Cs), xcol.view(1, 1, Sl, 9 * Cin), 1, 1, 1, 0, None, None,
                               rows=rs, red_taps=9)
        fuse = ctx.prod is not None and dt in ops.HALF
        bn_args = ops.fused_bn_bwd_args(ctx.prod) if fuse else None
        dfeat = ops.conv_dgrad(dh_dense, ops.pack_concat(w0s[:nd], dt, 1), Cin, H, W, 3, 3, 1, 1, bn_bwd=bn_args)
        wt_s = ops.pack_concat(w0s[nd:], dt, 2)
        cols = ops.conv_fwd(dhid_s.view(1, 1, Sl, Cs), wt_s, 9 * Cin, 1, 1, 1, 0)
        ops.heads_sparse_fixup(dfeat, cols, inds, slotmap, ownermap, bn_args)
        mods = [m for h in heads for m in h if isinstance(m, torch.nn.Module)]
        if fuse:
            ops.mark_bn_bwd_fused(ctx.prod[0], dfeat)
        wgrads()
        grads_ready(*mods)
        return dfeat, None, None


class CornerPoolFn(torch.autograd.Function):

    @staticmethod
    def forward(ctx, x, w_anchor, mod, dirs):
        tr = mod.branchMergeBn.training
        b1, b2, lc = mod.branch1, mod.branch2, mod.lastConv
        if tr:
            y1, s1 = _conv_stats(x, b1.conv, b1.bn, 1, 1, tr)
            y2, s2 = _conv_stats(x, b2.conv, b2.bn, 1, 1, tr)
            C1, C2 = b1.conv.weight.shape[0], b2.conv.weight.shape[0]
            st1, st2 = ops.bn_finalize_pair(b1.bn, s1, C1, y1.numel() // C1, b2.bn, s2, C2, y2.numel() // C2)
        else:
            y1, st1 = _train_bn_conv(x, b1.conv, b1.bn, 1, 1, tr)
            y2, st2 = _train_bn_conv(x, b2.conv, b2.bn, 1, 1, tr)
        a1 = ops.bn_apply(y1, st1, True)
        a2 = ops.bn_apply(y2, st2, True)
        p1 = ops.cpool_fwd(a1, dirs[0])
        t0 = ops.LaunchTimer.record("cpool_fwd_add")
        s = ops.cpool_fwd(a2, dirs[1], addend=p1)
        ops.LaunchTimer.close("cpool_fwd_add", t0)
        del p1
        if tr:
            ym, sm = _conv_stats(s, mod.branchMerge, mod.branchMergeBn, 1, 1, tr)
            ysc, ss = _conv_stats(x, mod.shortcutConv, mod.shortcutBn, 1, 0, tr)
            Cm, Cs = mod.branchMerge.weight.shape[0], mod.shortcutConv.weight.shape[0]
            stm, sts = ops.bn_finalize_pair(mod.branchMergeBn, sm, Cm, ym.numel() // Cm, mod.shortcutBn, ss, Cs,
                                            ysc.numel() // Cs)
        else:
            ym, stm = _train_bn_conv(s, mod.branchMerge, mod.branchMergeBn, 1, 1, tr)
            ysc, sts = _train_bn_conv(x, mod.shortcutConv, mod.shortcutBn, 1, 0, tr)
        r = ops.bn_apply(ym, stm, True, res=ysc, rst=sts)
        yl, stl = _train_bn_conv(r, lc.conv, lc.bn, 1, 1, tr, timer="cpool_lastconv")
        out = ops.bn_apply(yl, stl, True)
        ctx.save_for_backward(x, y1, a1, y2, a2, s, ym, ysc, r, yl, out)
        ctx.sts = (st1, st2, stm, sts, stl)
        ctx.mod, ctx.dirs = mod, dirs
        return out

    @staticmethod
    def backward(ctx, dout):
        x, y1, a1, y2, a2, s, ym, ysc, r, yl, out = ctx.saved_tensors
        st1, st2, stm, sts, stl = ctx.sts
        mod, dirs = ctx.mod, ctx.dirs
        N, H, W, C = x.shape
        lc = mod.lastConv
        dyl = ops.bn_backward(lc.bn, stl, _c(dout), yl, relu=True)
        ops.conv_wgrad(dyl, r, 3, 3, 1, 1, ops.grad_of(lc.conv.weight), _conv_ld(lc.conv.weight))
        dr = ops.conv_dgrad(dyl, ops.pack_weight(lc.conv.weight, x.dtype, 1), C, H, W, 3, 3, 1, 1)
        dym, dys = ops.bn_backward_pair(mod.branchMergeBn, stm, ym, mod.shortcutBn, sts, ysc, dr, r)
        wsc = mod.shortcutConv.weight
        ops.conv_wgrad(dys, x, 1, 1, 1, 0, ops.grad_of(wsc), _conv_ld(wsc))
        slot = ops.shared_grad_slot(x)
        prev = slot[1] if slot is not None else None
        dx = ops.conv_dgrad(dys, ops.pack_weight(wsc, x.dtype, 1), C, H, W, 1, 1, 1, 0, out=prev,
                            accumulate=prev is not None)
        wm = mod.branchMerge.weight
        ops.conv_wgrad(dym, s, 3, 3, 1, 1, ops.grad_of(wm), _conv_ld(wm))
        Cb = wm.shape[1]
        ds = ops.conv_dgrad(dym, ops.pack_weight(wm, x.dtype, 1), Cb, H, W, 3, 3, 1, 1)
        for (a, y, st, br), d in zip(((a1, y1, st1, mod.branch1), (a2, y2, st2, mod.branch2)), dirs):
            da = ops.cpool_bwd(a, ds, d)
            dy = ops.bn_backward(br.bn, st, da, y, relu=True)
            ops.conv_wgrad(dy, x, 3, 3, 1, 1, ops.grad_of(br.conv.weight), _conv_ld(br.conv.weight))
            ops.conv_dgrad(dy, ops.pack_weight(br.conv.weight, x.dtype, 1), C, H, W, 3, 3, 1, 1, out=dx,
                           accumulate=True)
        grads_ready(mod)
        if slot is not None:
            return ops.shared_grad_out(x, slot, dx if prev is None else None), None, None, None
        return dx, None, None, None


class CPoolFn(torch.autograd.Function):

    @staticmethod
    def forward(ctx, x, direction):
        ctx.save_for_backward(x)
        ctx.direction = direction
        return ops.cpool_fwd(x, direction)


    @staticmethod
    def backward(ctx, dy):
        (x,) = ctx.saved_tensors
        return ops.cpool_bwd(x, _c(dy), ctx.direction), None


class NCHWToNHWC(torch.autograd.Function):

    @staticmethod
    def forward(ctx, x, dtype):
        ctx.dtype_in = x.dtype
        return x.permute(0, 2, 3, 1).to(dtype).contiguous()

    @staticmethod
    def backward(ctx, g):
        return g.permute(0, 3, 1, 2).to(ctx.dtype_in).contiguous(), None
```

scd-resnet_amd/scdhip/lib.py:

```python
import ctypes
import os

import torch

HERE = os.path.dirname(os.path.abspath(__file__))
LIB_PATH = os.environ.get("SCDHIP_LIB", os.path.join(HERE, "libscdhip.so"))

DT_F32 = 0
DT_BF16 = 1
DT_F16 = 2
MAX_TAPS = 16
MAX_PHASES = 4
STAT_REPLICAS = 64

c_int, c_long, c_float, c_double, c_size_t, c_void_p = (ctypes.c_int, ctypes.c_long, ctypes.c_float,
                                                        ctypes.c_double, ctypes.c_size_t, ctypes.c_void_p)


class GemmPhase(ctypes.Structure):
    _fields_ = [("Qh", c_int), ("Qw", c_int), ("rho_h", c_int), ("rho_w", c_int), ("ntaps", c_int),
                ("dh", c_int * MAX_TAPS), ("dw", c_int * MAX_TAPS), ("wt", c_int * MAX_TAPS)]


class BnFinArgs(ctypes.Structure):
    _fields_ = [("stats", c_void_p), ("nrep", c_int), ("C", c_int), ("count", c_double), ("gamma", c_void_p),
                ("beta", c_void_p), ("running_mean", c_void_p), ("running_var", c_void_p), ("num_batches", c_void_p),
                ("momentum", c_float), ("eps", c_float), ("mean", c_void_p), ("invstd", c_void_p), ("scale", c_void_p),
                ("shift", c_void_p)]


class BnBwdFinArgs(ctypes.Structure):
    _fields_ = [("stats", c_void_p), ("nrep", c_int), ("C", c_int), ("count", c_double), ("gamma", c_void_p),
                ("mean", c_void_p), ("invstd", c_void_p), ("dgamma", c_void_p), ("dbeta", c_void_p),
                ("gscale", c_float), ("coef", c_void_p)]


class PackDesc(ctypes.Structure):
    _fields_ = [("w", c_void_p), ("out", c_void_p), ("start", c_long), ("A", c_int), ("B", c_int), ("T", c_int),
                ("mode", c_int), ("ldp", c_int), ("row_off", c_int), ("a_off", c_int), ("a_tot", c_int)]


P = c_void_p
I = c_int
L = c_long
F = c_float
D = c_double
PP = ctypes.POINTER(c_void_p)
IP = ctypes.POINTER(c_int)
LP = ctypes.POINTER(c_long)

SIGNATURES = {
    "scd_conv_gemm": (I, [I, P, P, P, P, P, I, I, I, I, I, I, I, I, I, I, I, I, I, ctypes.POINTER(GemmPhase), P]),
    "scd_conv_gemm_sel": (I, [I, I, P, P, P, P, P, I, I, I, I, I, I, I, I, I, I, I, I, I, ctypes.POINTER(GemmPhase), P, P,
                              P, P, P, P]),
    "scd_conv_gemm_res": (I, [I, P, P, P, P, P, I, I, I, I, I, I, I, I, I, I, I, I, ctypes.POINTER(GemmPhase), P]),
    "scd_conv_gemm_heads": (I, [I, P, P, P, P, I, I, I, I, I, IP, PP, PP, PP, P]),
    "scd_conv_gemm_heads_keep": (I, [I, P, P, P, P, I, I, I, I, I, IP, PP, PP, PP, P, I, P]),
    "scd_conv_gemm_bnbwd": (I, [I, P, P, P, I, I, I, I, I, I, I, I, I, I, I, ctypes.POINTER(GemmPhase), P, P, P, P,
                                P, P, P]),
    "scd_conv_wgrad_workspace": (c_size_t, [I, I, I, I]),
    "scd_conv_wgrad_nsplit": (I, [I, L, I, I, I]),
    "scd_conv_wgrad_nsplit2": (I, [I, L, I, I, I, I, I]),
    "scd_conv_wgrad": (I, [I, P, P, P, I, I, I, I, I, I, I, I, I, I, IP, IP, P]),
    "scd_wgrad_reduce": (I, [P, I, I, I, I, I, I, I, L, L, L, P, I, F, P]),
    "scd_wgrad_reduce_rows": (I, [P, I, I, I, I, I, IP, IP, LP, LP, LP, PP, I, I, F, P]),
    "scd_pack_weight": (I, [I, P, P, I, I, I, I, I, I, P]),
    "scd_pack_weights_batched": (I, [I, P, I, L, P]),
    "scd_pad_channels": (I, [I, P, L, I, I, P, P]),
    "scd_upsample2x_add": (I, [I, P, P, P, I, I, I, I, P]),
    "scd_upsample2x_add_bwd": (I, [I, P, P, I, I, I, I, P]),
    "scd_im2col_stem": (I, [I, P, P, I, I, I, I, I, I, I, I, I, I, P]),
    "scd_stem_conv_fwd": (I, [I, P, P, P, P, I, I, I, I, I, P]),
    "scd_stem_conv_wgrad_nsplit": (I, [L]),
    "scd_stem_conv_wgrad": (I, [I, P, P, P, P, P, I, I, I, I, I, I, P]),
    "scd_stem_bwd_nsplit": (I, []),
    "scd_conv_dgrad_s2": (I, [I, P, P, P, I, I, I, I, I, I, P]),
    "scd_stem_bwd_fused": (I, [I, P, P, P, P, P, P, P, P, P, P, I, P, I, I, I, I, I, P]),
    "scd_stem_bwd_combine": (I, [I, P, P, P, P, I, F, P]),
    "scd_stem_pool_bwd_bn": (I, [I, P, P, P, P, P, P, P, P, P, I, I, I, I, I, I, P]),
    "scd_stats_collapse": (I, [P, I, I, P]),
    "scd_stats_collapse_to": (I, [P, I, I, P, P]),
    "scd_bn_finalize": (I, [P, I, I, D, P, P, P, P, P, F, F, P, P, P, P, P]),
    "scd_bn_apply": (I, [I, P, P, I, L, P, P, P, P, P, I, P]),
    "scd_bn_bwd_reduce": (I, [I, P, P, P, P, P, P, P, I, L, P, P]),
    "scd_bn_bwd_finalize": (I, [P, I, I, D, P, P, P, P, P, F, P, P]),
    "scd_bn_finalize_n": (I, [ctypes.POINTER(BnFinArgs), I, P]),
    "scd_bn_bwd_finalize_n": (I, [ctypes.POINTER(BnBwdFinArgs), I, P]),
    "scd_bn_bwd_apply": (I, [I, P, P, P, P, P, P, I, L, P, P, P]),
    "scd_bn_bwd_reduce2": (I, [I, P, P, P, P, P, P, P, P, I, L, P, P, P]),
    "scd_bn_bwd_apply2": (I, [I, P, P, P, P, P, P, I, L, P, P, P]),
    "scd_stem_pool_fwd": (I, [I, P, P, P, P, P, I, I, I, I, I, I, P]),
    "scd_stem_pool_bwd": (I, [I, P, P, P, P, P, P, I, I, I, I, I, I, P]),
    "scd_heads_fwd": (I, [I, P, I, I, I, I, IP, PP, PP, PP, P]),
    "scd_heads_bwd_accsize": (c_size_t, [I, I, IP]),
    "scd_heads_bwd": (I, [I, P, I, I, I, I, IP, PP, PP, P, P, P]),
    "scd_heads_bwd_packed": (I, [I, P, I, I, I, I, IP, PP, PP, F, P, P, P, P]),
    "scd_heads_bwd_weight_finalize": (I, [P, I, I, IP, PP, PP, PP, I, F, P]),
    "scd_heads_bwd_packed_split": (I, [I, P, I, I, I, I, IP, I, PP, PP, F, P, P, P, P]),
    "scd_heads_sparse_bwd": (I, [I, P, P, I, I, I, I, I, I, IP, I, PP, PP, F, P, I, P, P, P, P, P, P]),
    "scd_heads_sparse_fixup": (I, [I, P, P, I, I, I, I, P, I, P, P, P, P, P, P, P, P, P]),
    "scd_focal_fwd": (I, [P, P, L, P, P, P]),
    "scd_l1_gather_fwd": (I, [P, I, I, I, P, P, P, I, I, I, P, P, P]),
    "scd_centernet_loss_finalize": (I, [P, I, P, I, P, P, P, P]),
    "scd_scale_by_device": (I, [P, L, P, I, P, P]),
    "scd_heads_keep_map": (I, [P, I, I, I, P, I, P, P]),
    "scd_centernet_loss_fwd": (I, [P, P, L, P, I, P, I, I, I, P, P, P, I, I, I, I, P, P, P, P, P, P, P, P]),
    "scd_centernet_loss_bwd_scale": (I, [P, L, I, I, P, I, P, I, P, I, P, P, P]),
    "scd_corner_ae_fwd": (I, [P, P, I, I, P, P, P, I, F, F, P, I, P, P, P, P, P, P]),
    "scd_corner_ae_bwd": (I, [P, P, I, I, P, P, P, I, P, P, P, P]),
    "scd_corner_pairs": (I, [P, P, P, P, P, P, P, P, P, P, I, I, I, F, I, P, P, P]),
    "scd_decode_workspace": (c_size_t, [I, I]),
    "scd_decode_topk": (I, [P, I, I, I, I, P, I, P, I, P, P, P, P, P, P, P, P]),
    "scd_augment_workspace": (c_size_t, [I]),
    "scd_augment_tiles": (I, [P, P, I, I, I, P, P, P, F, ctypes.c_ulonglong, P, P]),
    "scd_augment_tiles_indexed": (I, [P, L, P, P, I, I, I, P, P, P, F, ctypes.c_ulonglong, P, P]),
    "scd_pack_locs": (I, [P, P, P, I, P, P, I, I, I, P, P, P]),
    "scd_rotate_tiles": (I, [P, P, I, I, I, P, P]),
    "scd_rotate_tiles_mapped": (I, [P, P, I, I, I, P, I, P]),
    "scd_slide_workspace": (c_size_t, [I]),
    "scd_slide_tiles": (I, [P, I, I, I, I, I, I, I, I, I, I, P, P, P]),
    "scd_slide_detections": (I, [P, I, I, I, I, I, I, F, P, P, P, P]),
    "scd_slide_samples_workspace": (c_size_t, [I, I]),
    "scd_slide_samples": (I, [P, I, I, I, I, I, I, F, I, I, I, I, I, D, D, I, P, P, P, P, P, P, P, P, P]),
    "scd_slide_rotate_workspace": (c_size_t, [I, I]),
    "scd_slide_rotate_clips": (I, [P, I, I, I, I, I, I, I, I, ctypes.POINTER(c_double), I, P, P, P]),
    "scd_ceval_count": (I, [P, P, P, P, P, P, P, I, I, I, I, I, I, F, P, P]),
    "scd_ceval_emit": (I, [P, P, P, P, P, P, P, I, I, I, I, I, I, F, P, PP, P]),
    "scd_ceval_summary_workspace": (c_size_t, [L]),
    "scd_ceval_summary": (I, [PP, ctypes.POINTER(c_long), L, P, I, P, P, P]),
    "scd_adam_step": (I, [P, P, P, P, L, F, F, F, F, F, F, F, P]),
    "scd_adam_step_dev": (I, [P, P, P, P, L, P, F, F, F, F, P, P]),
    "scd_sgd_step_dev": (I, [P, P, P, L, P, F, F, F, I, F, P, P]),
    "scd_render_center_targets": (I, [P, P, I, I, I, F, P, P, P, P, P]),
    "scd_render_corner_targets": (I, [P, P, I, I, I, F, P, P, P, P, P, P, P]),
    "scd_render_corner_targets_split": (I, [P, P, I, I, I, F, P, P, P, P, P, P, I, P]),
    "scd_corner_tag_inds": (I, [P, P, I, I, I, P, P, P, P]),
    "scd_cpool_fwd": (I, [I, I, P, P, P, I, I, I, I, P]),
    "scd_cpool_bwd": (I, [I, I, P, P, P, I, I, I, I, P]),
    "scd_nms": (I, [P, L, I, I, I, P, P]),
    "scd_topk": (I, [P, I, L, I, I, I, P, P, P, P, P, P]),
    "scd_focal_prob_fwd": (I, [P, P, L, P, P, P]),
    "scd_masked_l1_fwd": (I, [P, P, P, L, I, I, P, P, P]),
    "scd_peer_mailbox_bytes": (c_size_t, [I, I]),
    "scd_peer_alloc": (I, [c_size_t, PP]),
    "scd_peer_free": (I, [P]),
    "scd_peer_ipc_handle": (I, [P, P]),
    "scd_peer_ipc_open": (I, [P, PP]),
    "scd_peer_ipc_close": (I, [P]),
    "scd_peer_allreduce_f64": (I, [P, I, I, I, PP, I, ctypes.c_ulonglong, P, ctypes.c_uint, P]),
    "scd_event_create": (I, [PP]),
    "scd_event_destroy": (I, [P]),
    "scd_event_record": (I, [P, P]),
    "scd_event_elapsed_ms": (I, [P, P, ctypes.POINTER(c_float)]),
    "scd_calib_mfma_peak": (I, [P, I, I, P, P, P]),
    "scd_calib_set_stamps": (I, [P]),
    "scd_calib_stamped_build": (I, []),
    "scd_version": (ctypes.c_char_p, []),
}


class _Lib:
    def __init__(self, path):
        if not os.path.exists(path):
            raise RuntimeError("libscdhip.so not found at %s -- build it with `python -c 'import __graft_entry__ as g; "
                               "g.build()'` (make -C scd-resnet_amd/csrc).  There is no CPU fallback." % path)
        self.path = path
        self.dll = ctypes.CDLL(path)
        for name, (res, args) in SIGNATURES.items():
            fn = getattr(self.dll, name)
            fn.restype = res
            fn.argtypes = args
            setattr(self, name, fn)


_LIB = None


def lib():
    global _LIB
    if _LIB is None:
        _LIB = _Lib(LIB_PATH)
    return _LIB


def check(rc, name):
    if rc != 0:
        raise RuntimeError("libscdhip: %s failed with status %d%s" % (
            name, rc, " (invalid argument / unsupported shape)" if rc == 9001 else " (hipError)"))


def call(name, *args):
    rc = getattr(_LIB or lib(), name)(*args)
    if rc:
        check(rc, name)


def ptr_array(ptrs):
    arr = (c_void_p * max(1, len(ptrs)))()
    for i, p in enumerate(ptrs):
        arr[i] = p
    return arr


def int_array(vals):
    arr = (c_int * max(1, len(vals)))()
    for i, v in enumerate(vals):
        arr[i] = int(v)
    return arr


def long_array(vals):
    arr = (c_long * max(1, len(vals)))()
    for i, v in enumerate(vals):
        arr[i] = int(v)
    return arr


def exported_symbols():
    return list(SIGNATURES)
```

scd-resnet_amd/scdhip/ops.py:

```python
import contextlib
import ctypes
import math
import os

import torch
import torch.distributed as dist

from . import lib as L

_DT = {torch.float32: L.DT_F32, torch.bfloat16: L.DT_BF16, torch.float16: L.DT_F16}
HALF = (torch.bfloat16, torch.float16)


class LossScale:
    f16 = float(os.environ.get("SCD_F16_LOSS_SCALE", "1024"))
    scaled_task = None


def loss_scale(dtype):
    return LossScale.f16 if dtype == torch.float16 else 1.0


def begin_loss_scale(dtype):
    S = loss_scale(dtype)
# ... 166 lines not shown
def new_bn_group():
    return dist.new_group(ranks=list(range(dist.get_world_size())))


def syncbn_group():
    if os.environ.get("SCD_SYNCBN_OWN_GROUP", "0") == "1":
        return new_bn_group()
    return dist.group.WORLD


def bn_sync_shares_group(group):
    g = _BNSync.group
    if g is None or _BNSync.peer is not None:
        return False
    world = dist.group.WORLD
    return (g or world) is (group or world)


def set_bn_sync(group, peer=None):
    if _BNSync.peer is not None:
        _BNSync.peer.close()
        _BNSync.peer = None
    _BNSync.group = group
    _BNSync.world = dist.get_world_size(group) if group is not None else 1
    if peer is None:
        peer = os.environ.get("SCD_SYNCBN_PEER", "0") == "1"
    if group is not None and peer and _BNSync.world > 1:
        from .peer import PeerAllReduce
        _BNSync.peer = PeerAllReduce(group)


def setup_syncbn(log=None):
    want = os.environ.get("SCD_SYNCBN_PEER", "0").lower()
    if _BNSync.peer is not None:
        _BNSync.peer.close()
        _BNSync.peer = None
    _BNSync.why = None
    if want in ("1", "auto", "on") and torch.cuda.is_available() and dist.get_world_size() > 1:
        from .peer import PeerAllReduce
        peer, why = PeerAllReduce.try_create(dist.group.WORLD)
        if peer is None and want == "1":
            raise RuntimeError("SCD_SYNCBN_PEER=1: the peer-memory SyncBN path could not be set up: %s" % why)
        if peer is not None:
            _BNSync.group, _BNSync.world, _BNSync.peer = dist.group.WORLD, dist.get_world_size(), peer
        else:
            _BNSync.why = why
    elif want not in ("1", "auto", "on"):
        _BNSync.why = "opt-in (SCD_SYNCBN_PEER=auto)"
    else:
        _BNSync.why = "no GPU" if not torch.cuda.is_available() else "world 1"
    if _BNSync.peer is None:
        set_bn_sync(syncbn_group(), peer=False)
        _BNSync.why = _BNSync.why or "fallback"
    mode = bn_sync_mode()
    if log is not None:
        log("SyncBN statistics: %s%s; gradient buckets %s" % (
            mode, "" if _BNSync.peer is not None else " (peer memory not used: %s)" % _BNSync.why,
            "all-reduced on WORLD from inside the backward" if mode != "rccl-world" else
            "all-reduced at the end of the backward (SyncBN shares their RCCL communicator)"))
    return mode


def bn_sync_mode():
    if _BNSync.group is None:
        return "off"
    if _BNSync.peer is not None:
        return "peer"
    return "rccl-world" if _BNSync.group is dist.group.WORLD else "rccl-own"


def bn_sync_peer():
    return _BNSync.peer


@contextlib.contextmanager
def bn_sync_suspended():
    saved = (_BNSync.group, _BNSync.world, _BNSync.peer)
    _BNSync.group, _BNSync.world, _BNSync.peer = None, 1, None
    try:
        yield
    finally:
        _BNSync.group, _BNSync.world, _BNSync.peer = saved


def bn_sync_group():
    return _BNSync.group


def bn_sync_poll():
    if _BNSync.peer is not None:
        _BNSync.peer.poll()


def bn_sync_world():
    return _BNSync.world if _BNSync.group is not None else 1


class SyncCounter:
    calls = 0
    per_step = None


def _allreduce_stats(stats, C):
    if _BNSync.group is None:
        return L.STAT_REPLICAS
    SyncCounter.calls += 1
    L.call("scd_stats_collapse", ptr(stats), L.STAT_REPLICAS, C, stream())
    if _BNSync.peer is not None:
        _BNSync.peer.all_reduce(stats[:2 * C])
    else:
        dist.all_reduce(stats[:2 * C], group=_BNSync.group)
    return 1


def _allreduce_stats_pair(sa, Ca, sb, Cb):
    if _BNSync.group is None:
        return sa, sb, L.STAT_REPLICAS
    n = 2 * (Ca + Cb)
    if _BNSync.peer is not None and n > _BNSync.peer.cap:
        _allreduce_stats(sa, Ca)
        _allreduce_stats(sb, Cb)
        return sa, sb, 1
    SyncCounter.calls += 1
    stage = torch.empty(n, dtype=torch.float64, device=sa.device)
    L.call("scd_stats_collapse_to", ptr(sa), L.STAT_REPLICAS, Ca, ptr(stage), stream())
    L.call("scd_stats_collapse_to", ptr(sb), L.STAT_REPLICAS, Cb, ptr(stage[2 * Ca:]), stream())
    if _BNSync.peer is not None:
        _BNSync.peer.all_reduce(stage)
    else:
        dist.all_reduce(stage, group=_BNSync.group)
    return stage[:2 * Ca], stage[2 * Ca:], 1


def new_stats(C, device):
    return torch.zeros(L.STAT_REPLICAS * 2 * C, dtype=torch.float64, device=device)


def persistent_zeros(owner, attr, numel, dtype):
    buf = getattr(owner, attr, None)
    dev = owner.device if torch.is_tensor(owner) else owner.weight.device
    if buf is None or buf.numel() != numel or buf.device != dev or buf.dtype != dtype:
        buf = torch.zeros(numel, dtype=dtype, device=dev)
        setattr(owner, attr, buf)
    return buf


def bn_stats(bn, which):
    return persistent_zeros(bn, "_scd_stats_" + which, L.STAT_REPLICAS * 2 * bn.num_features, torch.float64)



class PackPlan:

    def __init__(self):
        self.entries = {}
        self._sig = None
        self._dev = {}
        self.frozen = False
        self._retired = []

    def lookup(self, key):
        e = self.entries.get(key)
        if e is None:
            return None
        e[3] = True
        return e[0]

    def add(self, key, out, parts, dtype):
        self.entries[key] = [out, parts, dtype, True]

    def refresh(self):
        if capturing():
            self.frozen = True
        if not self.frozen:
            self.entries = {k: e for k, e in self.entries.items() if e[3]}
        if not self.entries:
            return
        sig = tuple((k, e[0].data_ptr(), tuple(p[0].data_ptr() for p in e[1])) for k, e in self.entries.items())
        if sig != self._sig:
            if capturing():
                raise RuntimeError("PackPlan: the operand set changed inside a step-graph capture (run an eager "
                                   "step first)")
            self._sig = sig
            if self.frozen:
                self._retired.append(self._dev)
            self._dev = {}
            per = {}
            for e in self.entries.values():
                per.setdefault(e[2], []).append(e)
            for dtype, es in per.items():
                descs, start = [], 0
                for out, parts, _, _ in es:
                    for (w, mode, ldp, row_off, a_off, a_tot) in parts:
                        A, B, T = w.shape[0], w.shape[1], w.shape[2] * w.shape[3]
                        d = L.PackDesc(w.data_ptr(), out.data_ptr(), start, A, B, T, mode, ldp, row_off, a_off, a_tot)
                        descs.append(d)
                        if mode == 0:
                            start += (A * ldp + 4095) // 4096 * 4096
                        elif mode == 3:
                            start += (4 * B * ldp + 4095) // 4096 * 4096
                        elif mode == 2:
                            start += (A * B * T + 4095) // 4096 * 4096
                        else:
                            bb = max(1, 64 // T)
                            start += ((A + 63) // 64) * ((B + bb - 1) // bb) * 4096
                arr = (L.PackDesc * len(descs))(*descs)
                host = torch.frombuffer(bytearray(bytes(arr)), dtype=torch.uint8)
                self._dev[dtype] = (host.to(es[0][0].device), len(descs), start)
        for dtype, (dev, n, total) in self._dev.items():
            L.call("scd_pack_weights_batched", _DT[dtype], dev.data_ptr(), n, total, stream())
        for e in self.entries.values():
            e[3] = False


_ACTIVE_PLAN = None


def pack_begin(plan):
    global _ACTIVE_PLAN
    clear_bn_fusion()
    _ACTIVE_PLAN = None
    plan.refresh()
    _ACTIVE_PLAN = plan


def pack_end():
    global _ACTIVE_PLAN
    _ACTIVE_PLAN = None


def pack_concat(ws, dtype, mode):
    A_tot = sum(w.shape[0] for w in ws)
    B, T = ws[0].shape[1], ws[0].shape[2] * ws[0].shape[3]
    plan = _ACTIVE_PLAN
    key = (tuple(id(w) for w in ws), dtype, mode)
    if plan is not None and all(isinstance(w, torch.nn.Parameter) for w in ws):
        hit = plan.lookup(key)
        if hit is not None:
            return hit
    if mode == 0:
        out = torch.empty(A_tot, T * B, dtype=dtype, device=ws[0].device)
        parts, off = [], 0
        for w in ws:
            parts.append((w, 0, T * B, off, 0, 0))
            pack_weight(w, dtype, 0, out=out, row_off=off, _cache=False)
            off += w.shape[0]
    elif mode == 2:
        out = torch.empty(T * B, A_tot, dtype=dtype, device=ws[0].device)
        parts, off = [], 0
        for w in ws:
            parts.append((w, 2, A_tot, 0, off, A_tot))
            L.call("scd_pack_weight", _DT[dtype], ptr(w), ptr(out), w.shape[0], B, T, 2, A_tot, off, stream())
            off += w.shape[0]
    else:
        cat = torch.cat(list(ws), 0)
        out = pack_weight(cat, dtype, 1, _cache=False)
        parts, off = [], 0
        for w in ws:
            parts.append((w, 1, T * A_tot, 0, off, A_tot))
            off += w.shape[0]
    if plan is not None and all(isinstance(w, torch.nn.Parameter) for w in ws):
        plan.add(key, out, parts, dtype)
    return out


def pack_weight(w, dtype, mode, ldp=None, out=None, row_off=0, _cache=True):
    plan = _ACTIVE_PLAN
    if _cache and out is None and row_off == 0 and plan is not None and isinstance(w, torch.nn.Parameter):
        key = (id(w), dtype, mode, ldp)
        hit = plan.lookup(key)
        if hit is not None:
            return hit
        res = pack_weight(w, dtype, mode, ldp, _cache=False)
        T = w.shape[2] * w.shape[3]
        plan.add(key, res, [(w, mode, res.shape[1], 0, 0, w.shape[0])], dtype)
        return res
    A, B = w.shape[0], w.shape[1]
    T = w.shape[2] * w.shape[3]
    if mode == 3:
        rows, ldp = 4 * B, ldp or 4 * A
    else:
        rows = A if mode == 0 else B
        ldp = ldp or T * (B if mode == 0 else A)
    if out is None:
        out = torch.empty(rows, ldp, dtype=dtype, device=w.device)
    L.call("scd_pack_weight", _DT[dtype], ptr(w), ptr(out), A, B, T, mode, ldp, row_off, stream())
    return out



class _Phases:
    __slots__ = ("arr", "n", "list")

    def __init__(self, phases):
        self.list = phases
        self.n = len(phases)
        self.arr = (L.GemmPhase * max(1, self.n))(*phases)

    def __len__(self):
        return self.n

    def __iter__(self):
        return iter(self.list)


_PHASES = {}


def _fwd_phase(kh, kw, pad, Ho, Wo):
    key = ("f", kh, kw, pad, Ho, Wo)
    ps = _PHASES.get(key)
    if ps is None:
        ph = L.GemmPhase()
        ph.Qh, ph.Qw, ph.rho_h, ph.rho_w = Ho, Wo, 0, 0
        ph.ntaps = kh * kw
        for r in range(kh):
            for s in range(kw):
                t = r * kw + s
                ph.dh[t], ph.dw[t], ph.wt[t] = r - pad, s - pad, t
        ps = _PHASES[key] = _Phases([ph])
    return ps


def _dgrad_phases(kh, kw, stride, pad, Hc, Wc, nonempty=False):
    key = ("d", kh, kw, stride, pad, Hc, Wc, nonempty)
    ps = _PHASES.get(key)
    if ps is not None:
        return ps
    phases = []
    for rh in range(stride):
        for rw in range(stride):
            Qh = -(-(Hc - rh) // stride)
            Qw = -(-(Wc - rw) // stride)
            if Qh <= 0 or Qw <= 0:
                continue
            ph = L.GemmPhase()
            ph.Qh, ph.Qw, ph.rho_h, ph.rho_w = Qh, Qw, rh, rw
            taps = [(r, s) for r in range(kh) if (r - rh - pad) % stride == 0
                    for s in range(kw) if (s - rw - pad) % stride == 0]
            ph.ntaps = len(taps)
            for t, (r, s) in enumerate(taps):
                ph.dh[t] = (rh + pad - r) // stride
                ph.dw[t] = (rw + pad - s) // stride
                ph.wt[t] = r * kw + s
            if ph.ntaps > 0 or not nonempty:
                phases.append(ph)
    ps = _PHASES[key] = _Phases(phases)
    return ps


def _c(t):
    return t if t.is_contiguous() else t.contiguous()


def pad_channels(t, C, Cp, rows):
    out = torch.empty(rows, Cp, dtype=t.dtype, device=t.device)
    L.call("scd_pad_channels", dt(t), ptr(t), rows, C, Cp, ptr(out), stream())
    return out


def _gemm(x, wpack, y, Co, Ho, Wo, in_stride, out_stride, phases, bias=None, stats=None, relu=False,
          accumulate=False, bn_bwd=None):
    N, Hi, Wi, Ci = x.shape
    bk = 64 if x.dtype in HALF else 32
    if Ci % bk:
        Cp = -(-Ci // bk) * bk
        T = wpack.shape[1] // Ci
        if T * Ci != wpack.shape[1]:
            raise RuntimeError("narrow-layer padding needs an unpadded [rows][taps*Ci] operand")
        x = pad_channels(_c(x), Ci, Cp, N * Hi * Wi).view(N, Hi, Wi, Cp)
        wpack = pad_channels(wpack, Ci, Cp, wpack.shape[0] * T).view(wpack.shape[0], T * Cp)
        Ci = Cp
    arr, nph = phases.arr, phases.n
    t0 = ClassTimer.begin()
    if bn_bwd is not None:
        st, ybn, bstats = bn_bwd
        assert bias is None and stats is None and not relu and not accumulate
        L.call("scd_conv_gemm_bnbwd", dt(x), ptr(x), ptr(wpack), ptr(y), N, Hi, Wi, Ci, Ho, Wo, Co, in_stride,
               out_stride, wpack.shape[1], nph, arr, ptr(ybn), ptr(st.mean), ptr(st.invstd), ptr(st.scale),
               ptr(st.shift), ptr(bstats), stream())
    else:
        L.call("scd_conv_gemm", dt(x), ptr(x), ptr(wpack), ptr(y), ptr(bias), ptr(stats), N, Hi, Wi, Ci, Ho, Wo, Co,
               in_stride, out_stride, wpack.shape[1], int(relu), int(accumulate), nph, arr, stream())
    if t0 is not None:
        ClassTimer.end("gemm", t0, _gemm_flops(Ci, Co, N, phases))
    return y


def conv_fwd(x, wpack, Co, kh, kw, stride, pad, bias=None, stats=None, relu=False, out=None):
    _need_gpu(x)
    N, H, W, _ = x.shape
    Ho = (H + 2 * pad - kh) // stride + 1
    Wo = (W + 2 * pad - kw) // stride + 1
    if out is None:
        out = torch.empty(N, Ho, Wo, Co, dtype=x.dtype, device=x.device)
    return _gemm(x, wpack, out, Co, Ho, Wo, stride, 1, _fwd_phase(kh, kw, pad, Ho, Wo), bias, stats, relu)


def gemm_res(x, wpack, y, Co, Ho, Wo, in_stride, out_stride, phases, bias=None, res=None, relu=False):
    _need_gpu(x)
    N, Hi, Wi, Ci = x.shape
    if Ci % (64 if x.dtype in HALF else 32):
        raise RuntimeError("scd_conv_gemm_res: %d input channels (a multiple of the K stage is required)" % Ci)
    if res is not None and (res.shape != y.shape or res.dtype != y.dtype or not res.is_contiguous()):
        raise RuntimeError("scd_conv_gemm_res: the residual must be a contiguous NHWC tensor of the output's shape "
                           "and dtype")
    t0 = ClassTimer.begin()
    L.call("scd_conv_gemm_res", dt(x), ptr(x), ptr(wpack), ptr(y), ptr(bias), ptr(res), N, Hi, Wi, Ci, Ho, Wo, Co,
           in_stride, out_stride, wpack.shape[1], int(relu), phases.n, phases.arr, stream())
    if t0 is not None:
        ClassTimer.end("gemm", t0, _gemm_flops(Ci, Co, N, phases))
    return y


def conv_fwd_res(x, wpack, Co, kh, kw, stride, pad, bias=None, res=None, relu=False, out=None):
    N, H, W, _ = x.shape
    Ho = (H + 2 * pad - kh) // stride + 1
    Wo = (W + 2 * pad - kw) // stride + 1
# ... 87 lines not shown
    return (st, y, bn_stats(bn, "bwdf"))



class SharedGrad:
    enabled = os.environ.get("SCD_SHARED_GRAD", "1") != "0"


_SHARED_GRAD = {}


def share_grad(t, n):
    if SharedGrad.enabled and n > 1 and torch.is_grad_enabled() and t.requires_grad:
        _SHARED_GRAD.clear()
        _SHARED_GRAD[_tkey(t)] = [n, None]


def shared_grad_slot(t):
    return _SHARED_GRAD.get(_tkey(t)) if _SHARED_GRAD else None


def _shared_grad_check(key, slot):
    if slot[0] > 0 and _SHARED_GRAD.get(key) is slot:
        _SHARED_GRAD.pop(key, None)
        raise RuntimeError("scdhip: %d consumer(s) of a shared feature gradient never ran backward; the partial sum "
                           "was not handed to autograd (ops.share_grad)" % slot[0])


def shared_grad_out(t, slot, grad):
    key = _tkey(t)
    if slot[1] is None:
        slot[1] = grad
        torch.autograd.Variable._execution_engine.queue_callback(lambda: _shared_grad_check(key, slot))
    slot[0] -= 1
    if slot[0] <= 0:
        _SHARED_GRAD.pop(key, None)
        return slot[1]
    return None


def mark_bn_bwd_fused(bn, grad):
    _BN_FUSED[id(bn)] = _tkey(grad)


def take_bn_bwd_fused(bn, dout):
    k = _BN_FUSED.pop(id(bn), None)
    if k is None:
        return None
    buf = bn_stats(bn, "bwdf")
    if k != _tkey(dout):
        buf.zero_()
        return None
    return buf


def clear_bn_fusion():
    _BN_PRODUCER.clear()



class SparseHeads:
    enabled = os.environ.get("SCD_SPARSE_HEADS", "1") != "0"


_SPARSE_GRAD = {}


def certify_sparse_grad(buf, inds):
    if SparseHeads.enabled:
        _SPARSE_GRAD[buf.untyped_storage().data_ptr()] = (buf, buf._version, inds)


def clear_sparse_grads():
    _SPARSE_GRAD.clear()


def sparse_grad_inds(g):
    if g is None or not _SPARSE_GRAD:
        return None
    e = _SPARSE_GRAD.get(g.untyped_storage().data_ptr())
    if e is None:
        return None
    buf, ver, inds = e
    if buf._version != ver or g._version != ver:
        return None
    return inds


_HEADS_HINT = [None]
_KEEP_MAPS = {}


def hint_sparse_support(inds):
    if SparseHeads.enabled and inds is not None:
        conv = inds.to(torch.int64).contiguous()
        _HEADS_HINT[0] = (inds, inds._version, conv)


def take_sparse_hint():
    h = _HEADS_HINT[0]
    _HEADS_HINT[0] = None
    _LAST_HINT[0] = h
    return h[2] if h is not None else None


def hinted_inds(inds):
    h = _HEADS_HINT[0] if _HEADS_HINT[0] is not None else _LAST_HINT[0]
    if h is not None and h[0] is inds and h[1] == inds._version:
        return h[2]
    return inds.to(torch.int64).contiguous()


_LAST_HINT = [None]


def heads_keep_map(inds, N, HW):
    K = inds.shape[1]
    key = (str(inds.device), N * HW, K)
    e = _KEEP_MAPS.get(key)
    if e is None:
        e = (torch.zeros(N * HW, dtype=torch.uint8, device=inds.device),
             torch.full((N * K,), -1, dtype=torch.int64, device=inds.device))
        _KEEP_MAPS[key] = e
    keep, prev = e
    L.call("scd_heads_keep_map", ptr(inds), N, K, HW, ptr(prev), prev.numel(), ptr(keep), stream())
    return keep


_SPARSE_MAPS = {}


def sparse_maps(dev, npix):
    key = (str(dev), npix)
    m = _SPARSE_MAPS.get(key)
    if m is None:
        m = (torch.full((npix,), -1, dtype=torch.int32, device=dev),
             torch.full((npix,), 0x7fffffff, dtype=torch.int32, device=dev))
        _SPARSE_MAPS[key] = m
    return m


def tensor_ptrs(ts):
    return L.ptr_array([t.data_ptr() for t in ts])


class HeadsDesc:

    def __init__(self, w1, b1):
        self.w1, self.b1, self.nh, self.od, self.Hd = w1, b1, len(w1), [w.shape[0] for w in w1], w1[0].shape[1]
        self.odarr, self.w1s, self.b1s = L.int_array(self.od), tensor_ptrs(w1), tensor_ptrs(b1)
        self.fused = self.Hd == 128 and self.nh <= 4 and max(self.od) <= 4
        self._acc = None

    def acc(self):
        if self._acc is None:
            n = L.lib().scd_heads_bwd_accsize(self.nh, self.Hd, self.odarr) // 8
            self._acc = persistent_zeros(self.w1[0], "_scd_heads_acc", n, torch.float64)
        return self._acc


def _heads_gemm(feat, wp, b0, hd, hid, outs, keep, keep_cols):
    N, H, W, Cin = feat.shape
    L.call("scd_conv_gemm_heads_keep", dt(feat), ptr(feat), ptr(wp), ptr(hid), ptr(b0), N, H, W, Cin, hd.nh, hd.odarr,
           hd.w1s, hd.b1s, tensor_ptrs(outs), ptr(keep) if keep is not None else None, keep_cols, stream())


def heads_fwd(feat, wp, b0, hd, keep=None):
    N, H, W, _ = feat.shape
    Ct = hd.nh * hd.Hd
    outs = [torch.empty(N, o, H, W, device=feat.device, dtype=torch.float32) for o in hd.od]
    if hd.fused:
        hid = torch.empty(N, H, W, Ct, device=feat.device, dtype=feat.dtype)
        t0 = LaunchTimer.record("heads_gemm")
        _heads_gemm(feat, wp, b0, hd, hid, outs, keep, hd.Hd)
        LaunchTimer.close("heads_gemm", t0)
    else:
        hid = conv_fwd(feat, wp, Ct, 3, 3, 1, 1, bias=b0, relu=True)
        L.call("scd_heads_fwd", dt(hid), ptr(hid), N, H * W, hd.nh, hd.Hd, hd.odarr, hd.w1s, hd.b1s, tensor_ptrs(outs),
               stream())
    return hid, outs


def heads_refill(feat, wp, b0, hd, hid):
    N, H, W, _ = feat.shape
    _heads_gemm(feat, wp, b0, hd, hid, [torch.empty(N, o, H, W, device=feat.device) for o in hd.od], None, 0)


def heads_bwd_packed(hid, hd, dptrs, S, nd=None):
    N, H, W, _ = hid.shape
    n = hd.nh if nd is None else nd
    dhid = torch.empty(N, H, W, n * hd.Hd, device=hid.device, dtype=hid.dtype)
    packed = torch.empty(N * H * W * n * 4, device=hid.device)
    name, split = ("scd_heads_bwd_packed", ()) if nd is None else ("scd_heads_bwd_packed_split", (nd,))
    L.call(name, dt(hid), ptr(hid), N, H * W, hd.nh, hd.Hd, hd.odarr, *split, hd.w1s, dptrs, float(S), ptr(packed),
           ptr(dhid), ptr(hd.acc()), stream())
    return dhid


def heads_sparse_bwd(hid, feat, hd, nd, dptrs, S, inds):
    N, H, W, Cin = feat.shape
    K = inds.shape[1]
    dhid_s = torch.empty(N * K, (hd.nh - nd) * hd.Hd, device=feat.device, dtype=feat.dtype)
    xcol = torch.empty(N * K, Cin * 9, device=feat.device, dtype=feat.dtype)
    slotmap, ownermap = sparse_maps(feat.device, N * H * W)
    L.call("scd_heads_sparse_bwd", dt(hid), ptr(hid), ptr(feat), N, H, W, Cin, hd.nh, hd.Hd, hd.odarr, nd, hd.w1s,
           dptrs, float(S), ptr(inds), K, ptr(dhid_s), ptr(xcol), ptr(hd.acc()), ptr(slotmap), ptr(ownermap), stream())
    return dhid_s, xcol, slotmap, ownermap


def heads_sparse_fixup(dfeat, cols, inds, slotmap, ownermap, bn_bwd=None):
    N, H, W, Cin = dfeat.shape
    bn_ptrs = (None,) * 6
    if bn_bwd is not None:
        st, ybn, bstats = bn_bwd
        bn_ptrs = (ptr(ybn), ptr(st.mean), ptr(st.invstd), ptr(st.scale), ptr(st.shift), ptr(bstats))
    L.call("scd_heads_sparse_fixup", dt(dfeat), ptr(dfeat), ptr(cols), N, H, W, Cin, ptr(inds), inds.shape[1],
           ptr(slotmap), ptr(ownermap), *bn_ptrs, stream())


def heads_bwd_weight_finalize(hd, b0s, S):
    L.call("scd_heads_bwd_weight_finalize", ptr(hd.acc()), hd.nh, hd.Hd, hd.odarr,
           tensor_ptrs([grad_of(w) for w in hd.w1]), tensor_ptrs([grad_of(b) for b in hd.b1]),
           tensor_ptrs([grad_of(b) for b in b0s]), 1, 1.0 / S, stream())



class _Side:
    enabled = os.environ.get("SCD_WGRAD_STREAM", "1") != "0"
    batch = None
    priority = 10
    streams = {}
    joined_task = {}


def _graph_task():
    try:
        return torch._C._current_graph_task_id()
    except Exception:
        return -1


def side_stream(dev):
    task = _graph_task()
    if not _Side.enabled or task == -1:
        return None
    idx = dev.index if dev.index is not None else torch.cuda.current_device()
    s = _Side.streams.get(idx)
    if s is None:
        s = _new_side_stream(idx)
        _Side.streams[idx] = s
    if _Side.batch is None or idx not in _Side.batch:
        s.wait_stream(torch.cuda.current_stream(idx))
        if _Side.batch is not None:
            _Side.batch.add(idx)
    if _Side.joined_task.get(idx) != task:
        _Side.joined_task[idx] = task
        torch.autograd.Variable._execution_engine.queue_callback(join_side_streams)
    return s


def _new_side_stream(idx):
    return torch.cuda.Stream(device=idx, priority=_Side.priority)


@contextlib.contextmanager
def side_batch():
    outer = _Side.batch
    _Side.batch = set() if outer is None else outer
    try:
        yield
    finally:
        _Side.batch = outer


def join_side_streams():
    for idx, s in _Side.streams.items():
        torch.cuda.current_stream(idx).wait_stream(s)
    _Side.joined_task.clear()


def side_stream_for_comm(dev):
    idx = dev.index if dev.index is not None else torch.cuda.current_device()
    s = _Side.streams.get(idx)
    if s is None or _graph_task() == -1:
        return None
    s.wait_stream(torch.cuda.current_stream(idx))
    return s


def conv_wgrad(g, x, kh, kw, stride, pad, dst, ld, cvalid=None, accumulate=True, rows=None, red_taps=1):
    side = side_stream(g.device) if g.is_cuda else None
    if side is None:
        return _conv_wgrad(g, x, kh, kw, stride, pad, dst, ld, cvalid, accumulate, rows, red_taps)
    with torch.cuda.stream(side):
        _conv_wgrad(g, x, kh, kw, stride, pad, dst, ld, cvalid, accumulate, rows, red_taps)
    g.record_stream(side)
    x.record_stream(side)


def _conv_wgrad(g, x, kh, kw, stride, pad, dst, ld, cvalid=None, accumulate=True, rows=None, red_taps=1):
    N, Ho, Wo, Cg = g.shape
    _, Hi, Wi, Ci = x.shape
    T = kh * kw
    d = dt(g)
    key = (d, N, Ho, Wo, Cg, Ci, kh, kw, pad)
    plan = _WGRAD_PLANS.get(key)
    if plan is None:
        dh = L.int_array([r - pad for r in range(kh) for s in range(kw)])
        dw = L.int_array([s - pad for r in range(kh) for s in range(kw)])
        ns = L.lib().scd_conv_wgrad_nsplit2(d, N * Ho * Wo, Ho, Wo, Cg, T, Ci)
        plan = _WGRAD_PLANS[key] = (dh, dw, ns, L.lib().scd_conv_wgrad_workspace(Cg, T, Ci, ns) // 4)
    dh, dw, ns, wsn = plan
    ws = torch.empty(wsn, dtype=torch.float32, device=g.device)
    t0 = ClassTimer.begin()
    L.call("scd_conv_wgrad", d, ptr(g), ptr(x), ptr(ws), ns, N, Ho, Wo, Cg, Hi, Wi, Ci, stride, T, dh, dw, stream())
    if rows is None:
        rows = [(0, Cg, dst, ld)]
    Tr, Cr = T * red_taps, Ci // red_taps
    cv = Cr if cvalid is None else cvalid
    for i in range(0, len(rows), 4):
        part = rows[i:i + 4]
        rkey = tuple((r[0], r[1], ptr(r[2]), tuple(r[3])) for r in part)
        arrs = _WGRAD_ROWS.get(rkey)
        if arrs is None:
            if len(_WGRAD_ROWS) > 4096:
                _WGRAD_ROWS.clear()
            arrs = _WGRAD_ROWS[rkey] = (
                L.int_array([r[0] for r in part]), L.int_array([r[1] for r in part]),
                L.long_array([r[3][0] for r in part]), L.long_array([r[3][1] for r in part]),
                L.long_array([r[3][2] for r in part]), L.ptr_array([ptr(r[2]) for r in part]))
        L.call("scd_wgrad_reduce_rows", ptr(ws), ns, Cg, Tr, Cr, len(part), *arrs, cv, int(accumulate), grad_alpha(g),
               stream())
    if t0 is not None:
        ClassTimer.end("wgrad", t0, 2.0 * N * Ho * Wo * Cg * T * Ci)


_WGRAD_PLANS = {}
_WGRAD_ROWS = {}



class BNState:
    __slots__ = ("mean", "invstd", "scale", "shift", "count")


def bn_finalize(bn, stats, C, count, training=True):
    st = _bn_state(C, bn.weight.device)
    if training:
        return _bn_finalize_launch(bn, st, stats, _allreduce_stats(stats, C), C, count)
    st.count = count
    L.call("scd_bn_finalize", *_bn_fin_args(bn, st, None, 0, C), stream())
    return st


def _bn_fin_args(bn, st, stats, nrep, C):
    ev = stats is None
    return (ptr(stats), nrep, C, 1.0 if ev else float(st.count), ptr(bn.weight), ptr(bn.bias), ptr(bn.running_mean),
            ptr(bn.running_var), 0 if ev else ptr(bn.num_batches_tracked), 0.0 if ev else float(bn.momentum),
            float(bn.eps), ptr(st.mean), ptr(st.invstd), ptr(st.scale), ptr(st.shift))


def _bn_finalize_launch(bn, st, stats, nrep, C, count):
    st.count = count * bn_sync_world()
    L.call("scd_bn_finalize", *_bn_fin_args(bn, st, stats, nrep, C), stream())
    return st


def _bn_state(C, dev):
    st = BNState()
    st.mean, st.invstd, st.scale, st.shift = torch.empty(4, C, device=dev).unbind(0)
# ... 613 lines not shown
```

Measured before the change: 6162 images/s.

## Fuse dense and sparse head backward kernels and cache concatenated biases

Merges the dense heads backward and the sparse heads backward into one launch, with block ranges split between the two paths. Single-output heads now read dout directly, which skips the pack kernel. The slotmap reset moves to a side stream with event synchronisation, and bias concatenation goes through the batched pack plan cache. The aim is fewer launches and less packing traffic in the heads backward, at the cost of added cross-stream ordering complexity and a fused kernel whose two halves may be unevenly balanced.

```diff
diff --git a/include/scdhip.h b/include/scdhip.h
--- a/include/scdhip.h
+++ b/include/scdhip.h
@@ -176,6 +176,18 @@
 int scd_heads_sparse_fixup(int dtype, void* dx, const void* cols, int N, int H, int W, int Cin, const long* inds, int K,
                            int* slotmap, int* ownermap, const void* bn_y, const float* mean, const float* invstd,
                            const float* relu_scale, const float* relu_shift, double* bn_stats, void* stream);
+int scd_heads_bwd_split(int dtype, const void* hid, int N, int HW, int nh, int Hd, const int* od, int nd,
+                        const float* const* w1, const float* const* douts, float dscale, void* dhid, double* acc,
+                        void* stream);
+int scd_heads_bwd_dense_sparse(int dtype, const void* hid, const void* feat, int N, int H, int W, int Cin, int nh,
+                               int Hd, const int* od, int nd, const float* const* w1, const float* const* douts,
+                               float dscale, float* packed, const long* inds, int K, void* dhid, void* dhid_s,
+                               void* xcol, double* acc, int* slotmap, int* ownermap, void* stream);
+int scd_heads_sparse_fixup_keep(int dtype, void* dx, const void* cols, int N, int H, int W, int Cin, const long* inds,
+                                int K, int* slotmap, int* ownermap, const void* bn_y, const float* mean,
+                                const float* invstd, const float* relu_scale, const float* relu_shift, double* bn_stats,
+                                void* stream);
+int scd_heads_sparse_reset(const long* inds, int N, int K, int HW, int* slotmap, void* stream);
 
 int scd_focal_fwd(const float* logits, const float* gt, long n, float* g, double* acc, void* stream);
 int scd_l1_gather_fwd(const float* feat, int N, int C, int HW, const int64_t* inds, const uint8_t* mask,
diff --git a/scd-resnet_amd/csrc/layers.hip b/scd-resnet_amd/csrc/layers.hip
--- a/scd-resnet_amd/csrc/layers.hip
+++ b/scd-resnet_amd/csrc/layers.hip
@@ -54,6 +54,15 @@
         if (d[mid].start <= e0) lo = mid; else hi = mid - 1;
     }
     const scd_pack_desc q = d[lo];
+    if (q.mode == 4) {
+        const unsigned base4 = (unsigned)(e0 - q.start);
+        for (int j = 0; j < PACK_UNIT / 256; ++j) {
+            const unsigned i = base4 + threadIdx.x + 256 * j;
+            if (i >= (unsigned)q.A) break;
+            ((float*)q.out)[q.a_off + i] = q.w[i];
+        }
+        return;
+    }
     if (q.mode == 1) {
         __shared__ float tile[64 * 65];
         const int T = q.T, BB = max(1, 64 / T);
@@ -166,6 +175,7 @@
     const float* dout[4];
     float* out[4];
     const float* pk;
+    float dscale;
 };
 
 __global__ void heads_pack_kernel(int N, int HW, HeadsDesc d, float scale, float* pk) {
@@ -220,9 +230,12 @@
     }
 }
 
-template <typename T, int U, bool PK = false>
-__global__ __launch_bounds__(512) void heads_bwd_kernel(const T* hid, int N, int HW, HeadsDesc d, T* dhid,
-                                                        double* acc, int accsz, int PXB) {
+constexpr int GD_NCHW = 0;
+constexpr int GD_PACKED = 1;
+constexpr int GD_ONE = 2;
+template <typename T, int U, int GD>
+__device__ __forceinline__ void heads_bwd_block(const T* hid, int N, int HW, const HeadsDesc& d, T* dhid, double* acc,
+                                                int accsz, int PXB, unsigned bid) {
     constexpr int E = Vec16<T>::N;
     constexpr int NA = 4 * E + E + 4;
     const int cph = d.Hd / E;
@@ -245,7 +258,7 @@
 #pragma unroll
     for (int k = 0; k < NA; ++k) a[k] = 0.f;
     const unsigned P = (unsigned)N * HW;
-    const unsigned p0 = blockIdx.x * (unsigned)PXB;
+    const unsigned p0 = bid * (unsigned)PXB;
     const unsigned p1 = min(P, p0 + PXB);
     const unsigned Ctot = d.hstride, Dtot = d.dstride;
     auto body = [&](unsigned px, const float* gd, float* v) {
@@ -255,7 +268,7 @@
             const float s = gd[0] * w[0][e] + gd[1] * w[1][e] + gd[2] * w[2][e] + gd[3] * w[3][e];
             r[e] = v[e] > 0.f ? s : 0.f;
 #pragma unroll
-            for (int o = 0; o < 4; ++o) a[o * E + e] += gd[o] * v[e];
+            for (int o = 0; o < 4; ++o) a[o * E + e] = __builtin_fmaf(gd[o], v[e], a[o * E + e]);
             a[4 * E + e] += r[e];
         }
 #pragma unroll
@@ -263,14 +276,17 @@
         Vec16<T>::store(dhid + px * Dtot + ct, r);
     };
     auto load_gd = [&](unsigned px, float* gd) {
-        if constexpr (PK) {
+        if constexpr (GD == GD_PACKED) {
             const float4 v = *(const float4*)(d.pk + ((size_t)px * d.nd + h) * 4);
             gd[0] = v.x; gd[1] = v.y; gd[2] = v.z; gd[3] = v.w;
+        } else if constexpr (GD == GD_ONE) {
+            gd[0] = dout[px] * d.dscale;
+            gd[1] = gd[2] = gd[3] = 0.f;
         } else {
             const unsigned n = px / (unsigned)HW;
             const unsigned q = px - n * HW;
 #pragma unroll
-            for (int o = 0; o < 4; ++o) gd[o] = o < od ? dout[(n * od + o) * (unsigned)HW + q] : 0.f;
+            for (int o = 0; o < 4; ++o) gd[o] = o < od ? dout[(n * od + o) * (unsigned)HW + q] * d.dscale : 0.f;
         }
     };
     if (g < G) {
@@ -294,7 +310,7 @@
     }
     constexpr int KR = (NA + 3) / 4;
     __shared__ float red[KR * 512];
-    double* dst = acc + (size_t)(blockIdx.x % SCD_STAT_REPLICAS) * accsz;
+    double* dst = acc + (size_t)(bid % SCD_STAT_REPLICAS) * accsz;
 #pragma unroll
     for (int k0 = 0; k0 < NA; k0 += KR) {
         if (k0) __syncthreads();
@@ -325,6 +341,12 @@
     }
 }
 
+template <typename T, int U, int GD>
+__global__ __launch_bounds__(512) void heads_bwd_kernel(const T* hid, int N, int HW, HeadsDesc d, T* dhid,
+                                                        double* acc, int accsz, int PXB) {
+    heads_bwd_block<T, U, GD>(hid, N, HW, d, dhid, acc, accsz, PXB, blockIdx.x);
+}
+
 bool make_desc(HeadsDesc& d, int nh, int Hd, const int* od) {
     if (nh < 1 || nh > 4 || Hd % 8 != 0) return false;
     d.nh = nh; d.Hd = Hd; d.nout = 0;
@@ -335,7 +357,7 @@
         d.orow[h] = d.nout;
         d.nout += d.od[h];
         d.w1[h] = nullptr; d.b1[h] = nullptr; d.dout[h] = nullptr; d.out[h] = nullptr;
-        d.pk = nullptr;
+        d.pk = nullptr; d.dscale = 1.f;
     }
     return d.nout * Hd <= 8 * 512;
 }
@@ -385,75 +407,25 @@
     });
 }
 
-template <bool PK>
-static int launch_heads_bwd(int dtype, const void* hid, int N, int HW, int nh, int Hd, const int* od, int nd,
-                            const float* const* w1, const float* const* douts, float dscale, float* packed, void* dhid,
-                            double* acc, void* stream) {
-    HeadsDesc d;
-    if (!make_desc(d, nh, Hd, od) || (PK && !packed) || nd < 1 || nd > nh) return SCD_ERR_ARG;
-    d.nd = nd;
-    d.dstride = nd * Hd;
-    return scd_dispatch_dtype(dtype, [&](auto tag) {
-        using T = typename decltype(tag)::type;
-        constexpr int E = 16 / sizeof(T);
-        const int cpp = nd * Hd / E;
-        if (cpp > 256 || (Hd % E)) return SCD_ERR_ARG;
-        for (int h = 0; h < nh; ++h) { d.w1[h] = w1[h]; d.dout[h] = douts[h]; }
-        const int accsz = d.nout * Hd + d.nout + nh * Hd;
-        const long P = (long)N * HW;
-        if (P * nh * Hd >= (1L << 31)) return SCD_ERR_ARG;
-        hipStream_t st = (hipStream_t)stream;
-        if constexpr (PK) {
-            hipLaunchKernelGGL(heads_pack_kernel, dim3(ew_blocks(P)), dim3(256), 0, st, N, HW, d, dscale, packed);
-            hipError_t e = hipGetLastError();
-            if (e != hipSuccess) return (int)e;
-            d.pk = packed;
-        }
-        const int G = 512 / cpp;
-        const int threads = G * cpp;
-        const int PXB = 2048;
-        const int blocks = cdiv(P, PXB);
-        hipLaunchKernelGGL((heads_bwd_kernel<T, E, PK>), dim3(blocks), dim3(threads), 0, st, (const T*)hid, N, HW, d,
-                           (T*)dhid, acc, accsz, PXB);
-        SCD_RETURN_LAUNCH();
-    });
-}
-
-extern "C" int scd_heads_bwd(int dtype, const void* hid, int N, int HW, int nh, int Hd, const int* od,
-                             const float* const* w1, const float* const* douts, void* dhid, double* acc,
-                             void* stream) {
-    SCD_F16_FWD(scd_heads_bwd, hid, N, HW, nh, Hd, od, w1, douts, dhid, acc, stream);
-    return launch_heads_bwd<false>(dtype, hid, N, HW, nh, Hd, od, nh, w1, douts, 1.f, nullptr, dhid, acc, stream);
-}
-
-extern "C" int scd_heads_bwd_packed(int dtype, const void* hid, int N, int HW, int nh, int Hd, const int* od,
-                                    const float* const* w1, const float* const* douts, float dscale, float* packed,
-                                    void* dhid, double* acc, void* stream) {
-    SCD_F16_FWD(scd_heads_bwd_packed, hid, N, HW, nh, Hd, od, w1, douts, dscale, packed, dhid, acc, stream);
-    return scd_heads_bwd_packed_split(dtype, hid, N, HW, nh, Hd, od, nh, w1, douts, dscale, packed, dhid, acc, stream);
-}
-
-extern "C" int scd_heads_bwd_packed_split(int dtype, const void* hid, int N, int HW, int nh, int Hd, const int* od,
-                                          int nd, const float* const* w1, const float* const* douts, float dscale,
-                                          float* packed, void* dhid, double* acc, void* stream) {
-    SCD_F16_FWD(scd_heads_bwd_packed_split, hid, N, HW, nh, Hd, od, nd, w1, douts, dscale, packed, dhid, acc, stream);
-    return launch_heads_bwd<true>(dtype, hid, N, HW, nh, Hd, od, nd, w1, douts, dscale, packed, dhid, acc, stream);
-}
-
 namespace {
 SCD_KERNEL_NS_BEGIN
 constexpr int SP_SPB = 2;
 
+constexpr int SP_GROUPS = 2;
+
 template <typename T>
-__global__ __launch_bounds__(256) void heads_sparse_bwd_kernel(const T* hid, const T* feat, int N, int H, int W, int Cin,
-                                                               HeadsDesc d, float dscale, const long* inds, int K,
-                                                               T* dhid_s, T* xcol, double* acc, int accsz,
-                                                               int* slotmap, int* ownermap) {
+__device__ __forceinline__ void heads_sparse_block(const T* hid, const T* feat, int N, int H, int W, int Cin,
+                                                   const HeadsDesc& d, const long* inds, int K, T* dhid_s, T* xcol,
+                                                   double* acc, int accsz, int* slotmap, int* ownermap, int sb) {
     const int HW = H * W;
     const int Cs = (d.nh - d.nd) * d.Hd;
-    const int tid = threadIdx.x;
+    const int ngl = blockDim.x >> 8;
+    const int lg = threadIdx.x >> 8;
+    const bool live = lg < ngl;
+    const int grp = sb * ngl + lg;
+    const int tid = threadIdx.x & 255;
     const int c = tid;
-    const bool cok = c < Cs;
+    const bool cok = live && c < Cs;
     const int h = cok ? d.nd + c / d.Hd : d.nd;
     const int j = cok ? c - (h - d.nd) * d.Hd : 0;
     const int od = d.od[h];
@@ -462,12 +434,13 @@
     for (int o = 0; o < 4; ++o) w[o] = (cok && o < od) ? d.w1[h][o * d.Hd + j] : 0.f;
     float a_dw1[4] = {0.f, 0.f, 0.f, 0.f}, a_db1[4] = {0.f, 0.f, 0.f, 0.f}, a_db0 = 0.f;
     const int S = N * K;
-    const int s0 = blockIdx.x * SP_SPB;
-    const int ns = min(S, s0 + SP_SPB) - s0;
-    __shared__ int dup[SP_SPB];
-    if (tid < SP_SPB) dup[tid] = 0;
+    const int s0 = grp * SP_SPB;
+    const int ns = live ? max(0, min(S, s0 + SP_SPB) - s0) : 0;
+    __shared__ int dups[SP_GROUPS][SP_SPB];
+    int* dup = dups[live ? lg : 0];
+    if (live && tid < SP_SPB) dup[tid] = 0;
     __syncthreads();
-    for (int i = tid; i < ns * K; i += blockDim.x) {
+    for (int i = tid; i < ns * K; i += 256) {
         const int jj = i / K, k2 = i - (i / K) * K;
         const int s = s0 + jj, k = s - (s / K) * K;
         if (k2 < k && inds[s - k + k2] == inds[s]) dup[jj] = 1;
@@ -486,7 +459,7 @@
             const float hv = to_f<T>(hid[p * d.hstride + d.nd * d.Hd + c]);
             float g[4];
 #pragma unroll
-            for (int o = 0; o < 4; ++o) g[o] = o < od ? d.dout[h][((long)b * od + o) * HW + q0] * dscale : 0.f;
+            for (int o = 0; o < 4; ++o) g[o] = o < od ? d.dout[h][((long)b * od + o) * HW + q0] * d.dscale : 0.f;
             const float sacc = g[0] * w[0] + g[1] * w[1] + g[2] * w[2] + g[3] * w[3];
             r = hv > 0.f ? sacc : 0.f;
 #pragma unroll
@@ -500,7 +473,7 @@
             if ((unsigned)qy < (unsigned)H && (unsigned)qx < (unsigned)W)
                 atomicMin(ownermap + (long)b * HW + qy * W + qx, s * 9 + tid);
         }
-        for (int ci = tid; ci < Cin; ci += blockDim.x) {
+        for (int ci = tid; ci < Cin; ci += 256) {
             T v[9];
 #pragma unroll
             for (int t = 0; t < 9; ++t) {
@@ -512,8 +485,8 @@
             for (int t = 0; t < 9; ++t) xcol[(long)s * 9 * Cin + t * Cin + ci] = v[t];
         }
     }
-    if (cok) {
-        double* dst = acc + (size_t)(blockIdx.x % SCD_STAT_REPLICAS) * accsz;
+    if (cok && ns > 0) {
+        double* dst = acc + (size_t)(grp % SCD_STAT_REPLICAS) * accsz;
 #pragma unroll
         for (int o = 0; o < 4; ++o)
             if (o < od) atomic_add_f64(dst + (d.orow[h] + o) * d.Hd + j, (double)a_dw1[o]);
@@ -523,6 +496,26 @@
             for (int o = 0; o < 4; ++o)
                 if (o < od) atomic_add_f64(dst + d.nout * d.Hd + d.orow[h] + o, (double)a_db1[o]);
     }
+}
+
+template <typename T>
+__global__ __launch_bounds__(256) void heads_sparse_bwd_kernel(const T* hid, const T* feat, int N, int H, int W, int Cin,
+                                                               HeadsDesc d, const long* inds, int K, T* dhid_s, T* xcol,
+                                                               double* acc, int accsz, int* slotmap, int* ownermap) {
+    heads_sparse_block<T>(hid, feat, N, H, W, Cin, d, inds, K, dhid_s, xcol, acc, accsz, slotmap, ownermap, blockIdx.x);
+}
+
+template <typename T, int U, int GD>
+__global__ __launch_bounds__(512) void heads_bwd_dense_sparse_kernel(const T* hid, const T* feat, int N, int H, int W,
+                                                                     int Cin, HeadsDesc d, T* dhid, int PXB, int nbd,
+                                                                     const long* inds, int K, T* dhid_s, T* xcol,
+                                                                     double* acc, int accsz, int* slotmap,
+                                                                     int* ownermap) {
+    if ((int)blockIdx.x < nbd)
+        heads_bwd_block<T, U, GD>(hid, N, H * W, d, dhid, acc, accsz, PXB, blockIdx.x);
+    else
+        heads_sparse_block<T>(hid, feat, N, H, W, Cin, d, inds, K, dhid_s, xcol, acc, accsz, slotmap, ownermap,
+                              (int)blockIdx.x - nbd);
 }
 
 template <typename T>
@@ -598,6 +591,99 @@
 SCD_KERNEL_NS_END
 }
 
+struct SparseTail {
+    const void* feat;
+    int H, W, Cin;
+    const long* inds;
+    int K;
+    void *dhid_s, *xcol;
+    int *slotmap, *ownermap;
+};
+
+static bool sparse_tail_ok(int N, int H, int W, int nh, int Hd, int nd, int K) {
+    if (nd < 0 || nd >= nh || K < 1 || (nh - nd) * Hd > 256) return false;
+    return (long)N * K * 9 * 9 < (1L << 31) && (long)N * H * W * nh * Hd < (1L << 31);
+}
+
+template <bool PK>
+static int launch_heads_bwd(int dtype, const void* hid, int N, int HW, int nh, int Hd, const int* od, int nd,
+                            const float* const* w1, const float* const* douts, float dscale, float* packed, void* dhid,
+                            double* acc, void* stream, const SparseTail* sp = nullptr) {
+    HeadsDesc d;
+    if (!make_desc(d, nh, Hd, od) || (PK && !packed) || nd < 1 || nd > nh) return SCD_ERR_ARG;
+    if (sp && (sp->H * sp->W != HW || !sparse_tail_ok(N, sp->H, sp->W, nh, Hd, nd, sp->K))) return SCD_ERR_ARG;
+    d.nd = nd;
+    d.dstride = nd * Hd;
+    d.dscale = dscale;
+    return scd_dispatch_dtype(dtype, [&](auto tag) {
+        using T = typename decltype(tag)::type;
+        constexpr int E = 16 / sizeof(T);
+        const int cpp = nd * Hd / E;
+        if (cpp > 256 || (Hd % E)) return SCD_ERR_ARG;
+        for (int h = 0; h < nh; ++h) { d.w1[h] = w1[h]; d.dout[h] = douts[h]; }
+        const int accsz = d.nout * Hd + d.nout + nh * Hd;
+        const long P = (long)N * HW;
+        if (P * nh * Hd >= (1L << 31)) return SCD_ERR_ARG;
+        hipStream_t st = (hipStream_t)stream;
+        if constexpr (PK) {
+            hipLaunchKernelGGL(heads_pack_kernel, dim3(ew_blocks(P)), dim3(256), 0, st, N, HW, d, dscale, packed);
+            hipError_t e = hipGetLastError();
+            if (e != hipSuccess) return (int)e;
+            d.pk = packed;
+        }
+        const int G = 512 / cpp;
+        const int threads = G * cpp;
+        const int PXB = 2048;
+        const int blocks = cdiv(P, PXB);
+        bool one = !PK;
+        for (int h = 0; h < nd; ++h) one = one && od[h] == 1;
+        if (sp) {
+            if (!PK && !one) return SCD_ERR_ARG;
+            const int sblocks = cdiv((long)N * sp->K, SP_SPB * (threads / 256));
+            hipLaunchKernelGGL((heads_bwd_dense_sparse_kernel<T, E, PK ? GD_PACKED : GD_ONE>), dim3(blocks + sblocks),
+                               dim3(threads), 0, st, (const T*)hid, (const T*)sp->feat, N, sp->H, sp->W, sp->Cin, d,
+                               (T*)dhid, PXB, blocks, sp->inds, sp->K, (T*)sp->dhid_s, (T*)sp->xcol, acc, accsz,
+                               sp->slotmap, sp->ownermap);
+            SCD_RETURN_LAUNCH();
+        }
+        if (one)
+            hipLaunchKernelGGL((heads_bwd_kernel<T, E, GD_ONE>), dim3(blocks), dim3(threads), 0, st, (const T*)hid, N,
+                               HW, d, (T*)dhid, acc, accsz, PXB);
+        else
+            hipLaunchKernelGGL((heads_bwd_kernel<T, E, PK ? GD_PACKED : GD_NCHW>), dim3(blocks), dim3(threads), 0, st,
+                               (const T*)hid, N, HW, d, (T*)dhid, acc, accsz, PXB);
+        SCD_RETURN_LAUNCH();
+    });
+}
+
+extern "C" int scd_heads_bwd(int dtype, const void* hid, int N, int HW, int nh, int Hd, const int* od,
+                             const float* const* w1, const float* const* douts, void* dhid, double* acc,
+                             void* stream) {
+    SCD_F16_FWD(scd_heads_bwd, hid, N, HW, nh, Hd, od, w1, douts, dhid, acc, stream);
+    return launch_heads_bwd<false>(dtype, hid, N, HW, nh, Hd, od, nh, w1, douts, 1.f, nullptr, dhid, acc, stream);
+}
+
+extern "C" int scd_heads_bwd_split(int dtype, const void* hid, int N, int HW, int nh, int Hd, const int* od, int nd,
+                                   const float* const* w1, const float* const* douts, float dscale, void* dhid,
+                                   double* acc, void* stream) {
+    SCD_F16_FWD(scd_heads_bwd_split, hid, N, HW, nh, Hd, od, nd, w1, douts, dscale, dhid, acc, stream);
+    return launch_heads_bwd<false>(dtype, hid, N, HW, nh, Hd, od, nd, w1, douts, dscale, nullptr, dhid, acc, stream);
+}
+
+extern "C" int scd_heads_bwd_packed(int dtype, const void* hid, int N, int HW, int nh, int Hd, const int* od,
+                                    const float* const* w1, const float* const* douts, float dscale, float* packed,
+                                    void* dhid, double* acc, void* stream) {
+    SCD_F16_FWD(scd_heads_bwd_packed, hid, N, HW, nh, Hd, od, w1, douts, dscale, packed, dhid, acc, stream);
+    return scd_heads_bwd_packed_split(dtype, hid, N, HW, nh, Hd, od, nh, w1, douts, dscale, packed, dhid, acc, stream);
+}
+
+extern "C" int scd_heads_bwd_packed_split(int dtype, const void* hid, int N, int HW, int nh, int Hd, const int* od,
+                                          int nd, const float* const* w1, const float* const* douts, float dscale,
+                                          float* packed, void* dhid, double* acc, void* stream) {
+    SCD_F16_FWD(scd_heads_bwd_packed_split, hid, N, HW, nh, Hd, od, nd, w1, douts, dscale, packed, dhid, acc, stream);
+    return launch_heads_bwd<true>(dtype, hid, N, HW, nh, Hd, od, nd, w1, douts, dscale, packed, dhid, acc, stream);
+}
+
 extern "C" int scd_heads_sparse_bwd(int dtype, const void* hid, const void* feat, int N, int H, int W, int Cin, int nh,
                                     int Hd, const int* od, int nd, const float* const* w1, const float* const* douts,
                                     float dscale, const long* inds, int K, void* dhid_s, void* xcol, double* acc,
@@ -605,27 +691,40 @@
     SCD_F16_FWD(scd_heads_sparse_bwd, hid, feat, N, H, W, Cin, nh, Hd, od, nd, w1, douts, dscale, inds, K, dhid_s, xcol,
                 acc, slotmap, ownermap, stream);
     HeadsDesc d;
-    if (!make_desc(d, nh, Hd, od) || nd < 0 || nd >= nh || K < 1 || (nh - nd) * Hd > 256) return SCD_ERR_ARG;
-    if ((long)N * K * 9 * 9 >= (1L << 31) || (long)N * H * W * nh * Hd >= (1L << 31)) return SCD_ERR_ARG;
+    if (!make_desc(d, nh, Hd, od) || !sparse_tail_ok(N, H, W, nh, Hd, nd, K)) return SCD_ERR_ARG;
     d.nd = nd;
+    d.dscale = dscale;
     for (int h = 0; h < nh; ++h) { d.w1[h] = w1[h]; d.dout[h] = douts[h]; }
     const int accsz = d.nout * Hd + d.nout + nh * Hd;
     const int blocks = cdiv((long)N * K, SP_SPB);
     return scd_dispatch_dtype(dtype, [&](auto tag) {
         using T = typename decltype(tag)::type;
         hipLaunchKernelGGL(heads_sparse_bwd_kernel<T>, dim3(blocks), dim3(256), 0, (hipStream_t)stream, (const T*)hid,
-                           (const T*)feat, N, H, W, Cin, d, dscale, inds, K, (T*)dhid_s, (T*)xcol, acc, accsz, slotmap,
+                           (const T*)feat, N, H, W, Cin, d, inds, K, (T*)dhid_s, (T*)xcol, acc, accsz, slotmap,
                            ownermap);
         SCD_RETURN_LAUNCH();
     });
 }
 
-extern "C" int scd_heads_sparse_fixup(int dtype, void* dx, const void* cols, int N, int H, int W, int Cin,
-                                      const long* inds, int K, int* slotmap, int* ownermap, const void* bn_y,
-                                      const float* mean, const float* invstd, const float* relu_scale,
-                                      const float* relu_shift, double* bn_stats, void* stream) {
-    SCD_F16_FWD(scd_heads_sparse_fixup, dx, cols, N, H, W, Cin, inds, K, slotmap, ownermap, bn_y, mean, invstd,
-                relu_scale, relu_shift, bn_stats, stream);
+extern "C" int scd_heads_bwd_dense_sparse(int dtype, const void* hid, const void* feat, int N, int H, int W, int Cin,
+                                          int nh, int Hd, const int* od, int nd, const float* const* w1,
+                                          const float* const* douts, float dscale, float* packed, const long* inds,
+                                          int K, void* dhid, void* dhid_s, void* xcol, double* acc, int* slotmap,
+                                          int* ownermap, void* stream) {
+    SCD_F16_FWD(scd_heads_bwd_dense_sparse, hid, feat, N, H, W, Cin, nh, Hd, od, nd, w1, douts, dscale, packed, inds, K,
+                dhid, dhid_s, xcol, acc, slotmap, ownermap, stream);
+    const SparseTail sp = {feat, H, W, Cin, inds, K, dhid_s, xcol, slotmap, ownermap};
+    if (packed)
+        return launch_heads_bwd<true>(dtype, hid, N, H * W, nh, Hd, od, nd, w1, douts, dscale, packed, dhid, acc,
+                                      stream, &sp);
+    return launch_heads_bwd<false>(dtype, hid, N, H * W, nh, Hd, od, nd, w1, douts, dscale, nullptr, dhid, acc, stream,
+                                   &sp);
+}
+
+static int launch_sparse_fixup(int dtype, void* dx, const void* cols, int N, int H, int W, int Cin, const long* inds,
+                               int K, int* slotmap, int* ownermap, const void* bn_y, const float* mean,
+                               const float* invstd, const float* relu_scale, const float* relu_shift, double* bn_stats,
+                               bool reset, void* stream) {
     if (Cin < 1 || K < 1) return SCD_ERR_ARG;
     if (bn_y && !(mean && invstd && relu_scale && relu_shift && bn_stats)) return SCD_ERR_ARG;
     const int S = N * K;
@@ -635,6 +734,7 @@
         hipLaunchKernelGGL(heads_sparse_fixup_kernel<T>, dim3(S), dim3(256), 0, st, (T*)dx, (const T*)cols, N, H, W,
                            Cin, inds, K, slotmap, ownermap, (const T*)bn_y, mean, invstd, relu_scale, relu_shift,
                            bn_stats);
+        if (!reset) SCD_RETURN_LAUNCH();
         hipError_t e = hipGetLastError();
         if (e != hipSuccess) return (int)e;
         hipLaunchKernelGGL(heads_sparse_reset_kernel, dim3(cdiv(S, 256)), dim3(256), 0, st, inds, S, K, H * W, slotmap);
@@ -642,6 +742,26 @@
     });
 }
 
+extern "C" int scd_heads_sparse_fixup(int dtype, void* dx, const void* cols, int N, int H, int W, int Cin,
+                                      const long* inds, int K, int* slotmap, int* ownermap, const void* bn_y,
+                                      const float* mean, const float* invstd, const float* relu_scale,
+                                      const float* relu_shift, double* bn_stats, void* stream) {
+    SCD_F16_FWD(scd_heads_sparse_fixup, dx, cols, N, H, W, Cin, inds, K, slotmap, ownermap, bn_y, mean, invstd,
+                relu_scale, relu_shift, bn_stats, stream);
+    return launch_sparse_fixup(dtype, dx, cols, N, H, W, Cin, inds, K, slotmap, ownermap, bn_y, mean, invstd,
+                               relu_scale, relu_shift, bn_stats, true, stream);
+}
+
+extern "C" int scd_heads_sparse_fixup_keep(int dtype, void* dx, const void* cols, int N, int H, int W, int Cin,
+                                           const long* inds, int K, int* slotmap, int* ownermap, const void* bn_y,
+                                           const float* mean, const float* invstd, const float* relu_scale,
+                                           const float* relu_shift, double* bn_stats, void* stream) {
+    SCD_F16_FWD(scd_heads_sparse_fixup_keep, dx, cols, N, H, W, Cin, inds, K, slotmap, ownermap, bn_y, mean, invstd,
+                relu_scale, relu_shift, bn_stats, stream);
+    return launch_sparse_fixup(dtype, dx, cols, N, H, W, Cin, inds, K, slotmap, ownermap, bn_y, mean, invstd,
+                               relu_scale, relu_shift, bn_stats, false, stream);
+}
+
 #ifndef SCD_F16_BUILD
 namespace {
 
@@ -651,12 +771,16 @@
     float* db0[4];
 };
 
-__global__ void heads_bwd_weight_finalize_kernel(double* acc, int accsz, HeadsDesc d, HeadsGrad g, int accumulate,
-                                                 double alpha) {
+__global__ __launch_bounds__(256) void heads_bwd_weight_finalize_kernel(double* acc, int accsz, HeadsDesc d,
+                                                                        HeadsGrad g, int accumulate, double alpha) {
     for (int i = blockIdx.x * blockDim.x + threadIdx.x; i < accsz; i += gridDim.x * blockDim.x) {
+        double v[SCD_STAT_REPLICAS];
+#pragma unroll
+        for (int r = 0; r < SCD_STAT_REPLICAS; ++r) v[r] = acc[(long)r * accsz + i];
         double s = 0.0;
+#pragma unroll
         for (int r = 0; r < SCD_STAT_REPLICAS; ++r) {
-            s += acc[(long)r * accsz + i];
+            s += v[r];
             acc[(long)r * accsz + i] = 0.0;
         }
         float* dst;
@@ -771,6 +895,14 @@
     SCD_RETURN_LAUNCH();
 }
 
+extern "C" int scd_heads_sparse_reset(const long* inds, int N, int K, int HW, int* slotmap, void* stream) {
+    if (N < 1 || K < 1 || HW < 1 || !inds || !slotmap) return SCD_ERR_ARG;
+    const int S = N * K;
+    hipLaunchKernelGGL(heads_sparse_reset_kernel, dim3(cdiv(S, 256)), dim3(256), 0, (hipStream_t)stream, inds, S, K, HW,
+                       slotmap);
+    SCD_RETURN_LAUNCH();
+}
+
 extern "C" int scd_adam_step(float* p, const float* g, float* m, float* v, long n, float lr, float beta1, float beta2,
                              float eps, float bc1, float bc2, float gscale, void* stream) {
     hipLaunchKernelGGL(adam_kernel, dim3(ew_blocks(n)), dim3(256), 0, (hipStream_t)stream, p, g, m, v, n, lr, beta1,
diff --git a/scd-resnet_amd/csrc/loss_decode.hip b/scd-resnet_amd/csrc/loss_decode.hip
--- a/scd-resnet_amd/csrc/loss_decode.hip
+++ b/scd-resnet_amd/csrc/loss_decode.hip
@@ -96,12 +96,44 @@
     int C, toff;
 };
 
+constexpr int L1_CMAX0 = 4, L1_CMAX1 = 2;
+
+template <bool PRE>
 __global__ __launch_bounds__(1024) void centernet_loss_b_kernel(int N, int HW, const int64_t* inds, const uint8_t* mask,
                                                                const float* target, int K, int tstride, L1Term t0,
                                                                L1Term t1, double* facc, LossFin w, float* out,
                                                                float* factors) {
     float s[2] = {0.f, 0.f}, cnt = 0.f;
     for (int i = threadIdx.x; i < N * K; i += blockDim.x) {
+        if constexpr (PRE) {
+            const bool m = mask[i];
+            const long ind = inds[i];
+            if (!m) continue;
+            cnt += 1.f;
+            const int n = i / K;
+            const float* tg = target + (long)i * tstride;
+            const long f0 = (long)n * t0.C * HW + ind, f1 = (long)n * t1.C * HW + ind;
+            float d0[L1_CMAX0], d1[L1_CMAX1];
+#pragma unroll
+            for (int c = 0; c < L1_CMAX0; ++c) d0[c] = c < t0.C ? t0.feat[f0 + (long)c * HW] - tg[t0.toff + c] : 0.f;
+#pragma unroll
+            for (int c = 0; c < L1_CMAX1; ++c) d1[c] = c < t1.C ? t1.feat[f1 + (long)c * HW] - tg[t1.toff + c] : 0.f;
+#pragma unroll
+            for (int c = 0; c < L1_CMAX0; ++c) {
+                if (c >= t0.C) break;
+                s[0] += fabsf(d0[c]);
+                const float sg = d0[c] > 0.f ? 1.f : (d0[c] < 0.f ? -1.f : 0.f);
+                if (sg != 0.f) atomic_add_f32(t0.g + f0 + (long)c * HW, sg);
+            }
+#pragma unroll
+            for (int c = 0; c < L1_CMAX1; ++c) {
+                if (c >= t1.C) break;
+                s[1] += fabsf(d1[c]);
+                const float sg = d1[c] > 0.f ? 1.f : (d1[c] < 0.f ? -1.f : 0.f);
+                if (sg != 0.f) atomic_add_f32(t1.g + f1 + (long)c * HW, sg);
+            }
+            continue;
+        }
         if (!mask[i]) continue;
         cnt += 1.f;
         const int n = i / K;
@@ -482,8 +514,12 @@
     LossFin w;
     for (int i = 0; i < 8; ++i) w.l1w[i] = i < 2 ? l1_weights[i] : 0.f;
     L1Term t0{regr, g_regr, Cr, toff_r}, t1{off, g_off, Co, toff_o};
-    hipLaunchKernelGGL(centernet_loss_b_kernel, dim3(1), dim3(1024), 0, st, N, HW, inds, mask, target, K, tstride, t0, t1,
-                       focal_acc, w, out, factors);
+    if (Cr <= L1_CMAX0 && Co <= L1_CMAX1)
+        hipLaunchKernelGGL(centernet_loss_b_kernel<true>, dim3(1), dim3(1024), 0, st, N, HW, inds, mask, target, K,
+                           tstride, t0, t1, focal_acc, w, out, factors);
+    else
+        hipLaunchKernelGGL(centernet_loss_b_kernel<false>, dim3(1), dim3(1024), 0, st, N, HW, inds, mask, target, K,
+                           tstride, t0, t1, focal_acc, w, out, factors);
     SCD_RETURN_LAUNCH();
 }
 
diff --git a/scd-resnet_amd/csrc/scd_common.h b/scd-resnet_amd/csrc/scd_common.h
--- a/scd-resnet_amd/csrc/scd_common.h
+++ b/scd-resnet_amd/csrc/scd_common.h
@@ -32,6 +32,9 @@
     X(scd_heads_bwd_packed_split) \
     X(scd_heads_sparse_bwd) \
     X(scd_heads_sparse_fixup) \
+    X(scd_heads_bwd_split) \
+    X(scd_heads_bwd_dense_sparse) \
+    X(scd_heads_sparse_fixup_keep) \
     X(scd_stem_conv_fwd) \
     X(scd_stem_conv_wgrad) \
     X(scd_stem_bwd_fused) \
diff --git a/scd-resnet_amd/scdhip/blocks.py b/scd-resnet_amd/scdhip/blocks.py
--- a/scd-resnet_amd/scdhip/blocks.py
+++ b/scd-resnet_amd/scdhip/blocks.py
@@ -273,7 +273,7 @@
     def forward(ctx, feat, w0_first, heads):
         N, H, W, Cin = feat.shape
         w0s = [h[0].weight for h in heads]
-        b0 = torch.cat([h[0].bias for h in heads], 0)
+        b0 = ops.bias_concat([h[0].bias for h in heads], feat.dtype)
         hd = ops.HeadsDesc([h[2].weight for h in heads], [h[2].bias for h in heads])
         wp = ops.pack_concat(w0s, feat.dtype, 0)
         hint = ops.take_sparse_hint()
@@ -347,8 +347,7 @@
         inds = ops.sparse_grad_inds(douts[-1])
         Sl = N * inds.shape[1]
         Cs = (nh - nd) * Hd
-        dh_dense = ops.heads_bwd_packed(hid, hd, dptrs, S, nd)
-        dhid_s, xcol, slotmap, ownermap = ops.heads_sparse_bwd(hid, feat, hd, nd, dptrs, S, inds)
+        dh_dense, dhid_s, xcol, slotmap, ownermap = ops.heads_bwd_dense_sparse(hid, feat, hd, nd, dptrs, S, inds)
         ops.heads_bwd_weight_finalize(hd, [h[0].bias for h in heads], S)
         ld = (Cin * 9, 9, 1)
 
@@ -359,12 +358,13 @@
                 ops.conv_wgrad(dh_dense, feat, 3, 3, 1, 1, None, None, rows=rd)
                 ops.conv_wgrad(dhid_s.view(1, 1, Sl, Cs), xcol.view(1, 1, Sl, 9 * Cin), 1, 1, 1, 0, None, None,
                                rows=rs, red_taps=9)
+                ops.heads_slotmap_reset(inds, slotmap, N, H * W)
         fuse = ctx.prod is not None and dt in ops.HALF
         bn_args = ops.fused_bn_bwd_args(ctx.prod) if fuse else None
         dfeat = ops.conv_dgrad(dh_dense, ops.pack_concat(w0s[:nd], dt, 1), Cin, H, W, 3, 3, 1, 1, bn_bwd=bn_args)
         wt_s = ops.pack_concat(w0s[nd:], dt, 2)
         cols = ops.conv_fwd(dhid_s.view(1, 1, Sl, Cs), wt_s, 9 * Cin, 1, 1, 1, 0)
-        ops.heads_sparse_fixup(dfeat, cols, inds, slotmap, ownermap, bn_args)
+        ops.heads_sparse_fixup(dfeat, cols, inds, slotmap, ownermap, bn_args, reset=False)
         mods = [m for h in heads for m in h if isinstance(m, torch.nn.Module)]
         if fuse:
             ops.mark_bn_bwd_fused(ctx.prod[0], dfeat)
diff --git a/scd-resnet_amd/scdhip/lib.py b/scd-resnet_amd/scdhip/lib.py
--- a/scd-resnet_amd/scdhip/lib.py
+++ b/scd-resnet_amd/scdhip/lib.py
@@ -99,6 +99,10 @@
     "scd_heads_bwd_packed_split": (I, [I, P, I, I, I, I, IP, I, PP, PP, F, P, P, P, P]),
     "scd_heads_sparse_bwd": (I, [I, P, P, I, I, I, I, I, I, IP, I, PP, PP, F, P, I, P, P, P, P, P, P]),
     "scd_heads_sparse_fixup": (I, [I, P, P, I, I, I, I, P, I, P, P, P, P, P, P, P, P, P]),
+    "scd_heads_bwd_split": (I, [I, P, I, I, I, I, IP, I, PP, PP, F, P, P, P]),
+    "scd_heads_bwd_dense_sparse": (I, [I, P, P, I, I, I, I, I, I, IP, I, PP, PP, F, P, P, I, P, P, P, P, P, P, P]),
+    "scd_heads_sparse_fixup_keep": (I, [I, P, P, I, I, I, I, P, I, P, P, P, P, P, P, P, P, P]),
+    "scd_heads_sparse_reset": (I, [P, I, I, I, P, P]),
     "scd_focal_fwd": (I, [P, P, L, P, P, P]),
     "scd_l1_gather_fwd": (I, [P, I, I, I, P, P, P, I, I, I, P, P, P]),
     "scd_centernet_loss_finalize": (I, [P, I, P, I, P, P, P, P]),
diff --git a/scd-resnet_amd/scdhip/ops.py b/scd-resnet_amd/scdhip/ops.py
--- a/scd-resnet_amd/scdhip/ops.py
+++ b/scd-resnet_amd/scdhip/ops.py
@@ -342,6 +342,8 @@
 
 class PackPlan:
 
+    cache_biases = True
+
     def __init__(self):
         self.entries = {}
         self._sig = None
@@ -382,7 +384,7 @@
                 descs, start = [], 0
                 for out, parts, _, _ in es:
                     for (w, mode, ldp, row_off, a_off, a_tot) in parts:
-                        A, B, T = w.shape[0], w.shape[1], w.shape[2] * w.shape[3]
+                        A, B, T = (w.numel(), 1, 1) if mode == 4 else (w.shape[0], w.shape[1], w.shape[2] * w.shape[3])
                         d = L.PackDesc(w.data_ptr(), out.data_ptr(), start, A, B, T, mode, ldp, row_off, a_off, a_tot)
                         descs.append(d)
                         if mode == 0:
@@ -391,6 +393,8 @@
                             start += (4 * B * ldp + 4095) // 4096 * 4096
                         elif mode == 2:
                             start += (A * B * T + 4095) // 4096 * 4096
+                        elif mode == 4:
+                            start += (A + 4095) // 4096 * 4096
                         else:
                             bb = max(1, 64 // T)
                             start += ((A + 63) // 64) * ((B + bb - 1) // bb) * 4096
@@ -454,6 +458,23 @@
     return out
 
 
+def bias_concat(bs, dtype):
+    plan = _ACTIVE_PLAN
+    if plan is None or not PackPlan.cache_biases or not all(isinstance(b, torch.nn.Parameter) for b in bs):
+        return torch.cat(list(bs), 0)
+    key = (tuple(id(b) for b in bs), dtype, "bias")
+    hit = plan.lookup(key)
+    if hit is not None:
+        return hit
+    out = torch.cat(list(bs), 0)
+    parts, off = [], 0
+    for b in bs:
+        parts.append((b, 4, 0, 0, off, out.numel()))
+        off += b.numel()
+    plan.add(key, out, parts, dtype)
+    return out
+
+
 def pack_weight(w, dtype, mode, ldp=None, out=None, row_off=0, _cache=True):
     plan = _ACTIVE_PLAN
     if _cache and out is None and row_off == 0 and plan is not None and isinstance(w, torch.nn.Parameter):
@@ -847,6 +868,9 @@
         self.fused = self.Hd == 128 and self.nh <= 4 and max(self.od) <= 4
         self._acc = None
 
+    def pixel_major(self, n):
+        return all(o == 1 for o in self.od[:n])
+
     def acc(self):
         if self._acc is None:
             n = L.lib().scd_heads_bwd_accsize(self.nh, self.Hd, self.odarr) // 8
@@ -885,11 +909,30 @@
     N, H, W, _ = hid.shape
     n = hd.nh if nd is None else nd
     dhid = torch.empty(N, H, W, n * hd.Hd, device=hid.device, dtype=hid.dtype)
+    if hd.pixel_major(n):
+        L.call("scd_heads_bwd_split", dt(hid), ptr(hid), N, H * W, hd.nh, hd.Hd, hd.odarr, n, hd.w1s, dptrs, float(S),
+               ptr(dhid), ptr(hd.acc()), stream())
+        return dhid
     packed = torch.empty(N * H * W * n * 4, device=hid.device)
     name, split = ("scd_heads_bwd_packed", ()) if nd is None else ("scd_heads_bwd_packed_split", (nd,))
     L.call(name, dt(hid), ptr(hid), N, H * W, hd.nh, hd.Hd, hd.odarr, *split, hd.w1s, dptrs, float(S), ptr(packed),
            ptr(dhid), ptr(hd.acc()), stream())
     return dhid
+
+
+def heads_bwd_dense_sparse(hid, feat, hd, nd, dptrs, S, inds):
+    N, H, W, Cin = feat.shape
+    K = inds.shape[1]
+    dhid = torch.empty(N, H, W, nd * hd.Hd, device=hid.device, dtype=hid.dtype)
+    dhid_s = torch.empty(N * K, (hd.nh - nd) * hd.Hd, device=feat.device, dtype=feat.dtype)
+    xcol = torch.empty(N * K, Cin * 9, device=feat.device, dtype=feat.dtype)
+    packed = None if hd.pixel_major(nd) else torch.empty(N * H * W * nd * 4, device=hid.device)
+    slotmap, ownermap = sparse_maps(feat.device, N * H * W)
+    _await_slotmap_reset(slotmap)
+    L.call("scd_heads_bwd_dense_sparse", dt(hid), ptr(hid), ptr(feat), N, H, W, Cin, hd.nh, hd.Hd, hd.odarr, nd, hd.w1s,
+           dptrs, float(S), ptr(packed), ptr(inds), K, ptr(dhid), ptr(dhid_s), ptr(xcol), ptr(hd.acc()), ptr(slotmap),
+           ptr(ownermap), stream())
+    return dhid, dhid_s, xcol, slotmap, ownermap
 
 
 def heads_sparse_bwd(hid, feat, hd, nd, dptrs, S, inds):
@@ -898,19 +941,43 @@
     dhid_s = torch.empty(N * K, (hd.nh - nd) * hd.Hd, device=feat.device, dtype=feat.dtype)
     xcol = torch.empty(N * K, Cin * 9, device=feat.device, dtype=feat.dtype)
     slotmap, ownermap = sparse_maps(feat.device, N * H * W)
+    _await_slotmap_reset(slotmap)
     L.call("scd_heads_sparse_bwd", dt(hid), ptr(hid), ptr(feat), N, H, W, Cin, hd.nh, hd.Hd, hd.odarr, nd, hd.w1s,
            dptrs, float(S), ptr(inds), K, ptr(dhid_s), ptr(xcol), ptr(hd.acc()), ptr(slotmap), ptr(ownermap), stream())
     return dhid_s, xcol, slotmap, ownermap
 
 
-def heads_sparse_fixup(dfeat, cols, inds, slotmap, ownermap, bn_bwd=None):
+def heads_sparse_fixup(dfeat, cols, inds, slotmap, ownermap, bn_bwd=None, reset=True):
     N, H, W, Cin = dfeat.shape
     bn_ptrs = (None,) * 6
     if bn_bwd is not None:
         st, ybn, bstats = bn_bwd
         bn_ptrs = (ptr(ybn), ptr(st.mean), ptr(st.invstd), ptr(st.scale), ptr(st.shift), ptr(bstats))
-    L.call("scd_heads_sparse_fixup", dt(dfeat), ptr(dfeat), ptr(cols), N, H, W, Cin, ptr(inds), inds.shape[1],
-           ptr(slotmap), ptr(ownermap), *bn_ptrs, stream())
+    L.call("scd_heads_sparse_fixup" if reset else "scd_heads_sparse_fixup_keep", dt(dfeat), ptr(dfeat), ptr(cols), N, H,
+           W, Cin, ptr(inds), inds.shape[1], ptr(slotmap), ptr(ownermap), *bn_ptrs, stream())
+
+
+_SLOTMAP_RESET = {}
+
+
+def _await_slotmap_reset(slotmap):
+    e = _SLOTMAP_RESET.get(slotmap.data_ptr())
+    if e is not None and e[0] != -1 and e[0] == _graph_task():
+        e[0] = -1
+        torch.cuda.current_stream().wait_event(e[1])
+
+
+def heads_slotmap_reset(inds, slotmap, N, HW):
+    side = side_stream(slotmap.device)
+    with torch.cuda.stream(side) if side is not None else contextlib.nullcontext():
+        L.call("scd_heads_sparse_reset", ptr(inds), N, inds.shape[1], HW, ptr(slotmap), stream())
+        if side is not None:
+            e = _SLOTMAP_RESET.get(slotmap.data_ptr())
+            if e is None:
+                e = _SLOTMAP_RESET[slotmap.data_ptr()] = [-1, torch.cuda.Event()]
+            e[0] = _graph_task()
+            e[1].record(side)
+            inds.record_stream(side)
 
 
 def heads_bwd_weight_finalize(hd, b0s, S):
```

Measured after the change: 6186 images/s, median of 6. Within noise of the previous version (+0.4%).
